# prstrive/GenS

Hardware: AMD Instinct MI355X
Metric: SDF ray-samples/sec at 480x640, 5-view, 3-scale volumes (higher is better)
Workload: dtype f32; 1 GPU; BASELINE config[1]: 5-view 480x640, volume_dims=[256, 128, 64], inference of 307200 rays x 128 samples per scene (K1 volume build + hierarchical sampling + SDF/blend MLPs + compositing); one scene per GPU; samples_per_ray=128, views=5, ray_chunk=30720, ray_chunk_set_by=ImplicitSurface.validate (default), cnn=out of scope (synthetic feature pyramid and regularised volumes), parallelism=single GPU

## Files before the change

gens_amd/csrc/k6b_sdf_bf16x3.hip:

```cpp
#include "common.h"

typedef float f32x16 __attribute__((ext_vector_type(16)));
typedef float f32x2v __attribute__((ext_vector_type(2)));
typedef float f32x4v __attribute__((ext_vector_type(4)));
typedef __bf16 bf16x2 __attribute__((ext_vector_type(2)));
typedef __bf16 bf16x8 __attribute__((ext_vector_type(8)));
typedef uint32_t u32x4 __attribute__((ext_vector_type(4)));

#define GB_WAVES 4
#define GB_PIECE 1024
#define GB_TERMS 3
#define GB_CH 8
#define GB_RING 4
#define GB_GT 2
#define GB_LPW (GB_CH / GB_WAVES)
#define GB_W_BYTES (GB_RING * GB_CH * GB_PIECE)
#define GB_D_BYTES (2 * 16 * 64 * 16)
#define GB_LDS_BYTES (GB_W_BYTES + GB_WAVES * GB_D_BYTES)
#define GB_JL_OFF 16384
#define GB_LOCK_OFF (GB_JL_OFF + 32 * 256)
#define GB_SLOT_BYTES (GB_LOCK_OFF + 256)
#define GB_SLOTS 2048
#define GB_C 144.26950408889634f

struct Split3Block {
    u32x4 p[GB_TERMS];
};

struct Split3Word {
    uint32_t w[GB_TERMS];
};
__device__ __forceinline__ uint32_t pk_bf16(float a, float b) {
    return __builtin_bit_cast(uint32_t, __builtin_convertvector((f32x2v){a, b}, bf16x2));
}
__device__ __forceinline__ Split3Word split3_pair(float a, float b) {
    Split3Word s;
#pragma unroll
    for (int k = 0; k < GB_TERMS; ++k) {
        const uint32_t w = pk_bf16(a, b);
        s.w[k] = w;
        if (k + 1 < GB_TERMS) {
            a -= __builtin_bit_cast(float, w << 16);
            b -= __builtin_bit_cast(float, w & 0xffff0000u);
        }
    }
    return s;
}
#define GB_PUT(BLK_, W_, A_, B_)                                            \
    {                                                                       \
        const Split3Word sw__ = split3_pair((A_), (B_));                    \
        _Pragma("unroll") for (int k__ = 0; k__ < GB_TERMS; ++k__) (BLK_).p[k__][(W_)] = sw__.w[k__]; \
    }

__device__ __forceinline__ float4 sample_volume4b(const float4* __restrict__ v, int Xd, int Yd, int Zd, const float x[3], bool live, float4& jx,
                                                  float4& jy, float4& jz) {
    float w0[3], w1[3];
    int i0[3];
    bool in0[3], in1[3];
    const int sz[3] = {Xd, Yd, Zd};
#pragma unroll
    for (int a = 0; a < 3; ++a) {
        const float pos = (x[a] + 1.0f) / 2.0f * (float)(sz[a] - 1);
        const float f = fminf(fmaxf(floorf(pos), -2.0f), (float)sz[a] + 1.0f);
        i0[a] = (int)f;
        w0[a] = (f + 1.0f) - pos;
        w1[a] = pos - f;
        in0[a] = i0[a] >= 0 && i0[a] < sz[a];
        in1[a] = i0[a] + 1 >= 0 && i0[a] + 1 < sz[a];
    }
    float4 acc = f4_zero();
    jx = f4_zero(); jy = f4_zero(); jz = f4_zero();
#pragma unroll
    for (int c = 0; c < 8; ++c) {
        const int a = c >> 2, b = (c >> 1) & 1, d = c & 1;
        const bool ok = live && (a ? in1[0] : in0[0]) && (b ? in1[1] : in0[1]) && (d ? in1[2] : in0[2]);
        const int cx = min(max(i0[0] + a, 0), Xd - 1), cy = min(max(i0[1] + b, 0), Yd - 1), cz = min(max(i0[2] + d, 0), Zd - 1);
        float4 t = v[((int64_t)cx * Yd + cy) * Zd + cz];
        if (!ok) t = f4_zero();
        const float wx = a ? w1[0] : w0[0], wy = b ? w1[1] : w0[1], wz = d ? w1[2] : w0[2];
        acc = f4_madd(acc, t, wx * wy * wz);
        jx = f4_madd(jx, t, (a ? 1.0f : -1.0f) * wy * wz);
        jy = f4_madd(jy, t, wx * (b ? 1.0f : -1.0f) * wz);
        jz = f4_madd(jz, t, wx * wy * (d ? 1.0f : -1.0f));
    }
    const float sx = (float)(Xd - 1) / 2.0f, sy = (float)(Yd - 1) / 2.0f, sz_ = (float)(Zd - 1) / 2.0f;
    jx.x *= sx; jx.y *= sx; jx.z *= sx; jx.w *= sx;
    jy.x *= sy; jy.y *= sy; jy.z *= sy; jy.w *= sy;
    jz.x *= sz_; jz.y *= sz_; jz.z *= sz_; jz.w *= sz_;
    return acc;
}

template <int NLEV>
struct GradShapeB {
    static constexpr int CF = 4 * NLEV;
    static constexpr int NCH = CF / 2;
    static constexpr int NC = (5 * NCH + 1 + 7) / 8;
    static constexpr int TC = (5 * NCH + 15) / 16;
    static constexpr int BLK = 4 * GB_TERMS;
    static constexpr int fwd(int l) { return l == 0 ? 0 : BLK * (2 + (l - 1) * (NC + 8) + (l > 3 ? 2 : 0)); }
    static constexpr int FWD_PIECES = fwd(5) + BLK * (NC + 8);
    static constexpr int rev_tiles(int l) { return 4 + TC + (l == 3 ? 1 : 0); }
    static constexpr int rev_blocks(int l) { return l == 2 ? 7 : 8; }
    static constexpr int rev(int l) {
        int p = FWD_PIECES;
        for (int k = 5; k > l; --k) p += GB_TERMS * rev_tiles(k) * rev_blocks(k);
        return p;
    }
    static constexpr int PIECES = rev(0) + 8 * GB_TERMS;
    static constexpr int NCHUNK = (PIECES + GB_CH - 1) / GB_CH;
    static constexpr int NCHUNK_FWD = (FWD_PIECES + GB_CH - 1) / GB_CH;
};

template <int NLEV, bool GRAD>
__global__ __launch_bounds__(64 * GB_WAVES, 1) void sdf_bf16x3_k(LevelSet vols, const char* __restrict__ pieces, const float* w_out, float b_last,
                                                                 float scale, float inv_scale, const float* __restrict__ pts,
                                                                 const int64_t* __restrict__ index, int64_t n_max, const int32_t* __restrict__ n_dev,
                                                                 float* __restrict__ sdf_out, float* __restrict__ grad_out,
                                                                 char* __restrict__ stash_all) {
    typedef GradShapeB<NLEV> S;
    constexpr int NCH = S::NCH, NC = S::NC, TC = S::TC, MID = NLEV / 2;
    constexpr int NCHUNK = GRAD ? S::NCHUNK : S::NCHUNK_FWD;
    extern __shared__ __attribute__((aligned(16))) char lds[];
    const int tid = threadIdx.x, lane = tid & 63;
    const int wave = __builtin_amdgcn_readfirstlane(tid >> 6);
    const int n_pt = lane & 31, half = lane >> 5;
    const int64_t n = n_dev ? min(n_max, (int64_t)n_dev[0]) : n_max;
    const int64_t m0 = (int64_t)blockIdx.x * (32 * GB_WAVES);
    if (m0 >= n) return;
    float4* const DS = (float4*)(lds + GB_W_BYTES + wave * GB_D_BYTES);

    const __amdgpu_buffer_rsrc_t prs = __builtin_amdgcn_make_buffer_rsrc((void*)pieces, 0, NCHUNK * GB_CH * GB_PIECE, 0x00020000);
    const uint32_t lane16 = (uint32_t)lane * 16u;
    auto stage = [&](int c) {
        char* dst = lds + (c % GB_RING) * (GB_CH * GB_PIECE);
#pragma unroll
        for (int p = 0; p < GB_LPW; ++p) {
            const int piece = wave + GB_WAVES * p;
            __builtin_amdgcn_raw_ptr_buffer_load_lds(prs, (__attribute__((address_space(3))) void*)(dst + piece * GB_PIECE), 16, lane16,
                                                     (uint32_t)(c * (GB_CH * GB_PIECE) + piece * GB_PIECE), 0, 0);
        }
    };
#pragma unroll
    for (int c = 0; c < GB_RING - 1; ++c) stage(c);

    uint32_t* lock = nullptr;
    uint32_t lock_seen = 0u;
    __amdgpu_buffer_rsrc_t stash;
    if constexpr (GRAD) {
        uint32_t hw_id, xcc_id;
        asm volatile("s_getreg_b32 %0, hwreg(HW_REG_HW_ID)" : "=s"(hw_id));
        asm volatile("s_getreg_b32 %0, hwreg(HW_REG_XCC_ID)" : "=s"(xcc_id));
        const uint32_t slot = ((((xcc_id & 7u) << 2 | ((hw_id >> 13) & 3u)) << 4 | ((hw_id >> 8) & 15u)) << 2) | (uint32_t)wave;
        char* const stash_slot = stash_all + (size_t)slot * GB_SLOT_BYTES;
        lock = (uint32_t*)(stash_slot + GB_LOCK_OFF);
        lock_seen = lane == 0 ? atomicCAS(lock, 0u, 1u) : 0u;
        stash = __builtin_amdgcn_make_buffer_rsrc((void*)stash_slot, 0, GB_LOCK_OFF, 0x00020000);
    }
    const uint32_t stash_lane = (uint32_t)lane * 16u, jl_lane = GB_JL_OFF + (uint32_t)lane * 4u;

    const int64_t row = m0 + 32 * wave + n_pt;
    const bool live = row < n;
    const int64_t src = live ? (index ? index[row] : row) : 0;
    float x[3] = {0.f, 0.f, 0.f};
    if (live) { x[0] = pts[3 * src]; x[1] = pts[3 * src + 1]; x[2] = pts[3 * src + 2]; }
    float nan_sum = 0.0f;

    Split3Block P[2];
    {
        float q[16];
#pragma unroll
        for (int k = 0; k < 16; ++k) q[k] = 0.0f;
#pragma unroll
        for (int a = 0; a < 3; ++a) {
            const float v = x[a] * scale;
            float s0, c0, s1, c1;
            hw_sincos(v * (half ? 4.0f : 1.0f), s0, c0);
            hw_sincos(v * (half ? 8.0f : 2.0f), s1, c1);
            if (half == 0) {
                q[a] = v; q[3 + a] = s0; q[6 + a] = c0; q[9 + a] = s1; q[12 + a] = c1;
            } else {
                q[a] = s0; q[3 + a] = c0; q[6 + a] = s1; q[9 + a] = c1;
            }
            nan_sum += x[a];
        }
        if (half == 0) q[15] = 1.0f;
#pragma unroll
        for (int k = 0; k < 16; k += 2) GB_PUT(P[k >> 3], (k & 7) >> 1, q[k], q[k + 1])
    }

    Split3Block C[NC];
    const float* wo = w_out + half * (64 + 16 * TC);
    float s_cond = 0.0f;
    float f[NCH];
    {
        float jl[3 * NCH];
#pragma unroll
        for (int j = 0; j <= MID; ++j) {
            const int l = j < MID ? (half ? MID + 1 + j : j) : MID;
            float4 jx, jy, jz;
            const float4 t = sample_volume4b((const float4*)vols.data[l], vols.dx[l], vols.dy[l], vols.dz[l], x, live, jx, jy, jz);
            float tv[4] = {t.x, t.y, t.z, t.w}, ax[4] = {jx.x, jx.y, jx.z, jx.w}, ay[4] = {jy.x, jy.y, jy.z, jy.w}, az[4] = {jz.x, jz.y, jz.z, jz.w};
            if (j == MID && half) {
                tv[0] = tv[2]; tv[1] = tv[3]; ax[0] = ax[2]; ax[1] = ax[3]; ay[0] = ay[2]; ay[1] = ay[3]; az[0] = az[2]; az[1] = az[3];
            }
#pragma unroll
            for (int c = 0; c < (j < MID ? 4 : 2); ++c) {
                const int ch = 4 * j + c;
                f[ch] = tv[c];
                jl[3 * ch] = ax[c]; jl[3 * ch + 1] = ay[c]; jl[3 * ch + 2] = az[c];
            }
        }
        if constexpr (GRAD) {
            if (lane == 0) gens_lock_slot(lock, lock_seen);
#pragma unroll
            for (int k = 0; k < 3 * NCH; ++k) __builtin_amdgcn_raw_buffer_store_b32(__builtin_bit_cast(uint32_t, jl[k]), stash, jl_lane + (uint32_t)k * 256u, 0, 0);
        }
        float e[8 * NC];
#pragma unroll
        for (int k = 5 * NCH; k < 8 * NC; ++k) e[k] = (k == 5 * NCH && half == 0) ? 1.0f : 0.0f;
#pragma unroll
        for (int j = 0; j < NCH; ++j) {
            e[5 * j] = f[j];
            hw_sincos(f[j], e[5 * j + 1], e[5 * j + 2]);
            hw_sincos(2.0f * f[j], e[5 * j + 3], e[5 * j + 4]);
            nan_sum += f[j];
#pragma unroll
            for (int q = 0; q < 5; ++q) s_cond = __builtin_fmaf(e[5 * j + q], wo[64 + 5 * j + q], s_cond);
        }
#pragma unroll
        for (int k = 0; k < 8 * NC; k += 2) GB_PUT(C[k >> 3], (k & 7) >> 1, e[k], e[k + 1])
    }

    f32x16 acc[4];
    Split3Block H[8];
    f32x16 D3[4], D4[4];
    f32x16 gc[TC], gp;
    u32x4 abuf[2][GB_TERMS * GB_GT];
    int par = 0;
    int dirty = GRAD ? 1 : 0;

#define GB_BOUNDARY(C_)                                                                                  \
    {                                                                                                    \
        const int c__ = (C_);                                                                            \
        const int later__ = (c__ + GB_RING - 2 < NCHUNK - 1 ? c__ + GB_RING - 2 : NCHUNK - 1) - c__;     \
        if (dirty || later__ <= 0) asm volatile("s_waitcnt vmcnt(0)" ::: "memory");                      \
        else if (later__ == 1) asm volatile("s_waitcnt vmcnt(%0)" ::"n"(GB_LPW) : "memory");             \
        else asm volatile("s_waitcnt vmcnt(%0)" ::"n"(2 * GB_LPW) : "memory");                           \
        dirty = 0;                                                                                       \
        __builtin_amdgcn_s_barrier();                                                                    \
        asm volatile("" ::: "memory");                                                                   \
        if (c__ + GB_RING - 1 < NCHUNK) stage(c__ + GB_RING - 1);                                        \
    }
#define GB_LOAD(SET_, P0_, CNT_)                                                                         \
    _Pragma("unroll") for (int j_ = 0; j_ < GB_TERMS * GB_GT; ++j_) if (j_ < (CNT_)) {                    \
        const int p_ = (P0_) + j_;                                                                       \
        if (p_ % GB_CH == 0) GB_BOUNDARY(p_ / GB_CH)                                                     \
        abuf[SET_][j_] = *((const u32x4*)(lds + ((p_ / GB_CH) % GB_RING) * (GB_CH * GB_PIECE) + (p_ % GB_CH) * GB_PIECE) + lane); \
    }
#define GB_MFMA(ACC_, A_, B_) ACC_ = __builtin_amdgcn_mfma_f32_32x32x16_bf16(__builtin_bit_cast(bf16x8, (A_)), __builtin_bit_cast(bf16x8, (B_)), ACC_, 0, 0, 0)
#define GB_RACC(T_) (*((T_) < 4 ? &acc[(T_) < 4 ? (T_) : 0] : (T_) < 4 + TC ? &gc[(T_) < 4 + TC && (T_) >= 4 ? (T_) - 4 : 0] : &gp))
#define GB_TERM(WA_, WB_, REV_, B_)                                                                      \
    _Pragma("unroll") for (int t_ = 0; t_ < GB_GT; ++t_) if (t_ < nt_) {                                 \
        if (REV_) GB_MFMA(GB_RACC(t0_ + t_), abuf[par][GB_TERMS * t_ + (WA_)], (B_)[i_].p[(WB_)]);       \
        else GB_MFMA(acc[(t0_ + t_) & 3], abuf[par][GB_TERMS * t_ + (WA_)], (B_)[i_].p[(WB_)]);          \
    }
#define GB_SEGMENT(P0_, CNT_, NT_, B_, REV_)                                                             \
    {                                                                                                    \
        constexpr int ng__ = ((NT_) + GB_GT - 1) / GB_GT;       \
        GB_LOAD(par, (P0_), GB_TERMS * ((NT_) < GB_GT ? (NT_) : GB_GT))                                  \
        _Pragma("unroll") for (int q_ = 0; q_ < (CNT_) * ng__; ++q_) {                                   \
            const int i_ = q_ / ng__, t0_ = (q_ % ng__) * GB_GT, nt_ = (NT_) - t0_ < GB_GT ? (NT_) - t0_ : GB_GT; \
            if (q_ + 1 < (CNT_) * ng__) {                                                                \
                const int i2_ = (q_ + 1) / ng__, t2_ = ((q_ + 1) % ng__) * GB_GT, n2_ = (NT_) - t2_ < GB_GT ? (NT_) - t2_ : GB_GT; \
                GB_LOAD(par ^ 1, (P0_) + GB_TERMS * ((NT_) * i2_ + t2_), GB_TERMS * n2_)                  \
            }                                                                                            \
            __builtin_amdgcn_sched_barrier(0);                                                           \
            GB_TERM(2, 0, REV_, B_) GB_TERM(1, 1, REV_, B_) GB_TERM(0, 2, REV_, B_)                      \
            GB_TERM(1, 0, REV_, B_) GB_TERM(0, 1, REV_, B_) GB_TERM(0, 0, REV_, B_)                      \
            __builtin_amdgcn_sched_barrier(0);                                                           \
            par ^= 1;                                                                                    \
        }                                                                                                \
    }
#define GB_ZERO()                                             \
    _Pragma("unroll") for (int t_ = 0; t_ < 4; ++t_)          \
        _Pragma("unroll") for (int r_ = 0; r_ < 16; ++r_) acc[t_][r_] = 0.0f;
#define GB_SOFTPLUS_TILE(T_, HT_, DT_)                                                                     \
    {                                                                                                      \
        f32x16 e__, u__, r__;                                                                              \
        _Pragma("unroll") for (int r_ = 0; r_ < 16; ++r_) e__[r_] = __builtin_amdgcn_exp2f(__builtin_amdgcn_fmed3f((T_)[r_], 126.0f, -3.0e38f)); \
        _Pragma("unroll") for (int r_ = 0; r_ < 16; ++r_) u__[r_] = 1.0f + e__[r_];                        \
        if (GRAD) { _Pragma("unroll") for (int r_ = 0; r_ < 16; ++r_) r__[r_] = __builtin_amdgcn_rcpf(u__[r_]); } \
        _Pragma("unroll") for (int r_ = 0; r_ < 16; ++r_) u__[r_] = __builtin_amdgcn_logf(u__[r_]);        \
        if (GRAD) { _Pragma("unroll") for (int r_ = 0; r_ < 16; ++r_) (DT_)[r_] = e__[r_] * r__[r_]; }     \
        _Pragma("unroll") for (int r_ = 0; r_ < 16; ++r_) (HT_)[r_] = __builtin_amdgcn_fmed3f((T_)[r_], u__[r_], 3.0e38f); \
    }
#define GB_SPLIT_TILE(T_, V_)                                                                              \
    _Pragma("unroll") for (int r_ = 0; r_ < 16; r_ += 2) GB_PUT(H[2 * (T_) + (r_ >> 3)], (r_ & 7) >> 1, (V_)[r_], (V_)[r_ + 1])

    float s_val = s_cond;
    GB_ZERO();
    GB_SEGMENT(S::fwd(0), 2, 4, P, false);
#pragma unroll
    for (int l = 0; l < 6; ++l) {
        if (l > 0) {
            GB_ZERO();
            GB_SEGMENT(S::fwd(l), NC, 4, C, false);
            if (l == 3) GB_SEGMENT(S::fwd(3) + S::BLK * NC, 2, 4, P, false);
            GB_SEGMENT(S::fwd(l) + S::BLK * (NC + (l == 3 ? 2 : 0)), 8, 4, H, false);
        }
#pragma unroll
        for (int t = 0; t < 4; ++t) {
            f32x16 h, d;
            if (l == 3) {
                GB_SOFTPLUS_TILE(acc[t], h, D3[t]);
            } else if (l == 4) {
                GB_SOFTPLUS_TILE(acc[t], h, D4[t]);
            } else {
                GB_SOFTPLUS_TILE(acc[t], h, d);
            }
            if constexpr (GRAD) {
                if (l < 2) {
#pragma unroll
                    for (int q = 0; q < 4; ++q) DS[(l * 16 + 4 * t + q) * 64 + lane] = make_float4(d[4 * q], d[4 * q + 1], d[4 * q + 2], d[4 * q + 3]);
                }
                if (l == 2) {
#pragma unroll
                    for (int q = 0; q < 4; ++q)
                        __builtin_amdgcn_raw_buffer_store_b128(__builtin_bit_cast(u32x4, (f32x4v){d[4 * q], d[4 * q + 1], d[4 * q + 2], d[4 * q + 3]}), stash,
                                                               stash_lane + (uint32_t)(4 * t + q) * 1024u, 0, 0);
                    dirty = 1;
                }
            }
            if (l < 5) {
                GB_SPLIT_TILE(t, h);
            } else {
                f32x16 g;
#pragma unroll
                for (int r = 0; r < 16; ++r) {
                    const float w = wo[16 * t + r];
                    s_val = __builtin_fmaf(h[r], w, s_val);
                    if (GRAD) g[r] = (w * GB_C) * d[r];
                }
                if constexpr (GRAD) GB_SPLIT_TILE(t, g);
            }
        }
    }
    s_val += 0.0f * nan_sum;
    s_val += __shfl_xor(s_val, 32, 64);

    if constexpr (!GRAD) {
        if (half == 0 && live) sdf_out[src] = (s_val + b_last) * inv_scale;
    } else {
#pragma unroll
        for (int c = 0; c < TC; ++c)
#pragma unroll
            for (int r = 0; r < 16; ++r) gc[c][r] = (16 * c + r < 5 * NCH) ? wo[64 + 16 * c + r] : 0.0f;
#pragma unroll
        for (int r = 0; r < 16; ++r) gp[r] = 0.0f;
#pragma unroll
        for (int l = 5; l >= 1; --l) {
            GB_ZERO();
            if (l == 3) {
#pragma unroll
                for (int t = 0; t < 4; ++t)
#pragma unroll
                    for (int q = 0; q < 4; ++q) {
                        const f32x4v v = __builtin_bit_cast(f32x4v, __builtin_amdgcn_raw_buffer_load_b128(stash, stash_lane + (uint32_t)(4 * t + q) * 1024u, 0, 0));
                        D4[t][4 * q] = v[0]; D4[t][4 * q + 1] = v[1]; D4[t][4 * q + 2] = v[2]; D4[t][4 * q + 3] = v[3];
                    }
            }
            if (l == 3) {
                GB_SEGMENT(S::rev(3), 8, 4 + TC + 1, H, true);
            } else if (l == 2) {
                GB_SEGMENT(S::rev(2), 7, 4 + TC, H, true);
            } else {
                GB_SEGMENT(S::rev(l), 8, 4 + TC, H, true);
            }
#pragma unroll
            for (int t = 0; t < 4; ++t) {
                f32x16 g;
#pragma unroll
                for (int q = 0; q < 4; ++q) {
                    float4 d;
                    if (l == 5) d = make_float4(D4[t][4 * q], D4[t][4 * q + 1], D4[t][4 * q + 2], D4[t][4 * q + 3]);
                    if (l == 4) d = make_float4(D3[t][4 * q], D3[t][4 * q + 1], D3[t][4 * q + 2], D3[t][4 * q + 3]);
                    if (l == 3) d = make_float4(D4[t][4 * q], D4[t][4 * q + 1], D4[t][4 * q + 2], D4[t][4 * q + 3]);
                    if (l == 2) d = DS[(16 + 4 * t + q) * 64 + lane];
                    if (l == 1) d = DS[(4 * t + q) * 64 + lane];
                    g[4 * q] = acc[t][4 * q] * d.x;
                    g[4 * q + 1] = acc[t][4 * q + 1] * d.y;
                    g[4 * q + 2] = acc[t][4 * q + 2] * d.z;
                    g[4 * q + 3] = acc[t][4 * q + 3] * d.w;
                }
                GB_SPLIT_TILE(t, g);
            }
        }
        {
            GB_ZERO();
            GB_LOAD(par, S::rev(0), GB_TERMS)
#pragma unroll
            for (int i = 0; i < 8; ++i) {
                if (i + 1 < 8) { GB_LOAD(par ^ 1, S::rev(0) + GB_TERMS * (i + 1), GB_TERMS) }
                __builtin_amdgcn_sched_barrier(0);
                GB_MFMA(acc[0], abuf[par][2], H[i].p[0]);
                GB_MFMA(acc[1], abuf[par][1], H[i].p[1]);
                GB_MFMA(acc[2], abuf[par][1], H[i].p[0]);
                GB_MFMA(acc[0], abuf[par][0], H[i].p[2]);
                GB_MFMA(acc[3], abuf[par][0], H[i].p[1]);
                GB_MFMA(gp, abuf[par][0], H[i].p[0]);
                __builtin_amdgcn_sched_barrier(0);
                par ^= 1;
            }
#pragma unroll
            for (int r = 0; r < 16; ++r) gp[r] += (acc[0][r] + acc[1][r]) + (acc[2][r] + acc[3][r]);
        }

        {
            float g[3];
#pragma unroll
            for (int a = 0; a < 3; ++a) asm volatile("" : "+v"(x[a]));
#pragma unroll
            for (int j = 0; j < NCH; ++j) asm volatile("" : "+v"(f[j]));
#pragma unroll
            for (int a = 0; a < 3; ++a) {
                const float v = x[a] * scale;
                float s0, c0, s1, c1;
                hw_sincos(v * (half ? 4.0f : 1.0f), s0, c0);
                hw_sincos(v * (half ? 8.0f : 2.0f), s1, c1);
                g[a] = half ? 4.0f * (gp[a] * c0 - gp[3 + a] * s0) + 8.0f * (gp[6 + a] * c1 - gp[9 + a] * s1)
                            : gp[a] + (gp[3 + a] * c0 - gp[6 + a] * s0) + 2.0f * (gp[9 + a] * c1 - gp[12 + a] * s1);
                g[a] *= scale;
            }
            {
                float acc_in = x[0] + x[1] + x[2];
#pragma unroll
                for (int j = 0; j < NCH; ++j) acc_in += f[j];
#pragma unroll
                for (int a = 0; a < 3; ++a) g[a] += 0.0f * acc_in;
            }
#pragma unroll
            for (int j = 0; j < NCH; ++j) {
                const int q = 5 * j;
                float s1, c1, s2, c2;
                hw_sincos(f[j], s1, c1);
                hw_sincos(2.0f * f[j], s2, c2);
                const float df = gc[q >> 4][q & 15] + gc[(q + 1) >> 4][(q + 1) & 15] * c1 - gc[(q + 2) >> 4][(q + 2) & 15] * s1 +
                                 2.0f * (gc[(q + 3) >> 4][(q + 3) & 15] * c2 - gc[(q + 4) >> 4][(q + 4) & 15] * s2);
#pragma unroll
                for (int a = 0; a < 3; ++a) {
                    const float jl = __builtin_bit_cast(float, __builtin_amdgcn_raw_buffer_load_b32(stash, jl_lane + (uint32_t)(3 * j + a) * 256u, 0, 0));
                    g[a] = __builtin_fmaf(df, jl, g[a]);
                }
            }
#pragma unroll
            for (int a = 0; a < 3; ++a) g[a] += __shfl_xor(g[a], 32, 64);
            if (half == 0 && live) {
                sdf_out[src] = (s_val + b_last) * inv_scale;
                grad_out[3 * src] = g[0] * inv_scale;
                grad_out[3 * src + 1] = g[1] * inv_scale;
                grad_out[3 * src + 2] = g[2] * inv_scale;
            }
        }
        if (lane == 0) atomicExch(lock, 0u);
    }
#undef GB_BOUNDARY
#undef GB_LOAD
#undef GB_MFMA
#undef GB_RACC
#undef GB_TERM
#undef GB_SEGMENT
#undef GB_ZERO
#undef GB_SOFTPLUS_TILE
#undef GB_SPLIT_TILE
}

int gens_fill_levels(const char* who, LevelSet* ls, const float* const* data, const int* dims, int n_levels);

extern "C" int gens_sdf_bf16x3_pieces(int n_levels) {
    return n_levels == 3 ? GradShapeB<3>::NCHUNK * GB_CH : n_levels == 5 ? GradShapeB<5>::NCHUNK * GB_CH : 0;
}

extern "C" int64_t gens_sdf_grad_f16_stash_bytes(void);

static int check_bf16x3_args(const char* who, int n_levels, const void* pieces, const float* w_out, float scale, const float* pts, int64_t n,
                             const float* sdf_out) {
    GENS_CHECK_ARG(n_levels == 3 || n_levels == 5, GENS_ELIMIT, "%s: built for 3 or 5 volume levels, got %d", who, n_levels);
    GENS_CHECK_ARG(pieces && w_out, GENS_EINVAL, "%s: null weight stream", who);
    GENS_CHECK_ARG(((uintptr_t)pieces & 15) == 0, GENS_EINVAL, "%s: the weight stream must be 16-byte aligned", who);
    GENS_CHECK_ARG(n >= 0 && (n == 0 || (pts && sdf_out)), GENS_EINVAL, "%s: null pts / output", who);
    GENS_CHECK_ARG(scale != 0.0f, GENS_EINVAL, "%s: scale must be non-zero", who);
    return 0;
}

extern "C" int gens_sdf_value_bf16x3(const float* const* vols_packed, const int* dims, int n_levels, const void* pieces, const float* w_out,
                                     float b_last, float scale, const float* pts, const int64_t* index, int64_t n, const int32_t* n_device,
                                     float* sdf_out, void* stream) {
    LevelSet vs;
    if (int e = gens_fill_levels("gens_sdf_value_bf16x3", &vs, vols_packed, dims, n_levels)) return e;
    if (int e = check_bf16x3_args("gens_sdf_value_bf16x3", n_levels, pieces, w_out, scale, pts, n, sdf_out)) return e;
    if (n == 0) return 0;
    const unsigned grid = gens_blocks(n, 32 * GB_WAVES);
    if (n_levels == 3)
        sdf_bf16x3_k<3, false><<<grid, 64 * GB_WAVES, GB_W_BYTES, (hipStream_t)stream>>>(vs, (const char*)pieces, w_out, b_last, scale, 1.0f / scale, pts,
                                                                                          index, n, n_device, sdf_out, nullptr, nullptr);
    else
        sdf_bf16x3_k<5, false><<<grid, 64 * GB_WAVES, GB_W_BYTES, (hipStream_t)stream>>>(vs, (const char*)pieces, w_out, b_last, scale, 1.0f / scale, pts,
                                                                                          index, n, n_device, sdf_out, nullptr, nullptr);
    return gens_launch_status("gens_sdf_value_bf16x3");
}

extern "C" int gens_sdf_grad_bf16x3(const float* const* vols_packed, const int* dims, int n_levels, const void* pieces, const float* w_out,
                                    float b_last, float scale, const float* pts, const int64_t* index, int64_t n, const int32_t* n_device,
                                    float* sdf_out, float* grad_out, void* stash, void* stream) {
    LevelSet vs;
    if (int e = gens_fill_levels("gens_sdf_grad_bf16x3", &vs, vols_packed, dims, n_levels)) return e;
    if (int e = check_bf16x3_args("gens_sdf_grad_bf16x3", n_levels, pieces, w_out, scale, pts, n, sdf_out)) return e;
    GENS_CHECK_ARG(n == 0 || grad_out, GENS_EINVAL, "gens_sdf_grad_bf16x3: null gradient output");
    GENS_CHECK_ARG(stash && ((uintptr_t)stash & 15) == 0, GENS_EINVAL,
                   "gens_sdf_grad_bf16x3: null or misaligned stash (gens_sdf_grad_f16_stash_bytes() bytes, zeroed once)");
    GENS_CHECK_ARG(gens_sdf_grad_f16_stash_bytes() == (int64_t)GB_SLOTS * GB_SLOT_BYTES, GENS_EINVAL, "gens_sdf_grad_bf16x3: stash layout differs from k6gh's");
    if (n == 0) return 0;
    static GensLdsOptIn lds3, lds5;
    if (int e = n_levels == 3 ? gens_lds_opt_in(lds3, (const void*)sdf_bf16x3_k<3, true>, GB_LDS_BYTES, "gens_sdf_grad_bf16x3")
                              : gens_lds_opt_in(lds5, (const void*)sdf_bf16x3_k<5, true>, GB_LDS_BYTES, "gens_sdf_grad_bf16x3"))
        return e;
    const unsigned grid = gens_blocks(n, 32 * GB_WAVES);
    if (n_levels == 3)
        sdf_bf16x3_k<3, true><<<grid, 64 * GB_WAVES, GB_LDS_BYTES, (hipStream_t)stream>>>(vs, (const char*)pieces, w_out, b_last, scale, 1.0f / scale, pts,
                                                                                           index, n, n_device, sdf_out, grad_out, (char*)stash);
    else
        sdf_bf16x3_k<5, true><<<grid, 64 * GB_WAVES, GB_LDS_BYTES, (hipStream_t)stream>>>(vs, (const char*)pieces, w_out, b_last, scale, 1.0f / scale, pts,
                                                                                           index, n, n_device, sdf_out, grad_out, (char*)stash);
    return gens_launch_status("gens_sdf_grad_bf16x3");
}
```

gens_amd/csrc/k7t_blend.hip:

```cpp
#include "k4_common.h"

typedef float f32x4 __attribute__((ext_vector_type(4)));

#define KT_NT 4
#define KT_XS 29

struct BlendTWeights {
    const float4* stream;
    const float* tab;
    float v2_last_b, u2_b, r3_b, s_abs;
    const float* sdev;
};
enum { KT_RD1_B = 0, KT_RD2_B, KT_B2_B, KT_V1_B, KT_V2_B, KT_U1_B, KT_R2_B, KT_V2_LAST, KT_U2, KT_R3, KT_TAB_ENTRIES };

__device__ __forceinline__ float elu1t(float x) { return __builtin_amdgcn_fmed3f(x, hw_exp(x) - 1.0f, 0.0f); }
template <int G>
__device__ __forceinline__ float group_sum(float v) {
    v += dpp_move<0xB1, 0xF>(v, v);
    if (G == 4) v += dpp_move<0x4E, 0xF>(v, v);
    return v;
}
template <int G>
__device__ __forceinline__ float group_min(float v) {
    v = fminf(v, dpp_move<0xB1, 0xF>(v, v));
    if (G == 4) v = fminf(v, dpp_move<0x4E, 0xF>(v, v));
    return v;
}
template <int G>
__device__ __forceinline__ float group_max(float v) {
    v = fmaxf(v, dpp_move<0xB1, 0xF>(v, v));
    if (G == 4) v = fmaxf(v, dpp_move<0x4E, 0xF>(v, v));
    return v;
}
__device__ __forceinline__ float lanes_q_sum(float v) {
    v += __shfl_xor(v, 16, 64);
    v += __shfl_xor(v, 32, 64);
    return v;
}

template <int NLEV, int S>
__global__ __launch_bounds__(64, 2) void blend_t_k(BlendTWeights W, MapSet fs, const float4* __restrict__ imgs, const float* __restrict__ w2c,
                                                   const float* __restrict__ intr, const float* __restrict__ c2w, const float* __restrict__ pts,
                                                   const int64_t* __restrict__ index, int64_t n_max, const int32_t* __restrict__ n_dev,
                                                   float* __restrict__ rgb_out, uint8_t* __restrict__ vis_out) {
    constexpr int F = 3 + 4 * NLEV;
    constexpr int XQ = NLEV + 1;
    constexpr int XT = (XQ + 3) / 4;
    constexpr int G = S == 2 ? 2 : 4;
    constexpr int PPT = 16 / G;
    constexpr int PPW = 64 / G;
    constexpr int NPT = PPW / 16;
    static_assert(S >= 2 && S <= 4, "two to four source views");
    static_assert(4 * XQ <= KT_XS, "feature tile too narrow");
    __shared__ float X[64 * KT_XS];
    __shared__ float RD[64 * 5];
    __shared__ float R[64];
    const int lane = threadIdx.x;
    const int np = lane & 15, q = lane >> 4;
    const int64_t n = n_dev ? min(n_max, (int64_t)n_dev[0]) : n_max;
    const int64_t first = (int64_t)blockIdx.x * PPW;
    if (first >= n) return;
    if (W.sdev) { W.v2_last_b = W.sdev[0]; W.u2_b = W.sdev[1]; W.r3_b = W.sdev[2]; W.s_abs = W.sdev[3]; }

    const float4* wp = W.stream;
    float4 wb[3];
    int par = 0;
    wb[0] = wp[lane];
    wb[1] = wp[lane + 64];
    wp += 128;

    {
        const int pl = lane / G, sv = (lane % G) + 1;
        const bool live = first + pl < n && sv <= S;
        const int64_t src = live ? (index ? index[first + pl] : first + pl) : 0;
        float x = 0.f, y = 0.f, z = 0.f;
        if (live) { x = pts[3 * src]; y = pts[3 * src + 1]; z = pts[3 * src + 2]; }
        bool inside = true;
        float* xr = X + lane * KT_XS;
        const int svc = sv <= S ? sv : S;
        const SrcBase pb = project_src_base(w2c + 16 * svc, intr + 16 * svc, x, y, z);
#pragma unroll
        for (int l = 0; l < NLEV; ++l) {
            const int h = fs.h[l], w = fs.w[l];
            const SrcProj p = project_src_level(pb, exp2f(-(float)l), h, w, fs.cw[l], fs.ch[l], fs.rcw[l], fs.rch[l]);
            inside = inside && p.inside;
            float4 f = f4_zero(), c = f4_zero();
            if (live) {
                const Taps2 t = bilinear_taps(p.ix, p.iy, h, w);
                f = sample_texel(fs.data[l] + (int64_t)svc * h * w, h, w, 1, 0, t);
                if (l == 0) c = sample_texel(imgs + (int64_t)svc * h * w, h, w, 1, 0, t);
            }
            xr[3 + 4 * l] = f.x; xr[4 + 4 * l] = f.y; xr[5 + 4 * l] = f.z; xr[6 + 4 * l] = f.w;
            if (l == 0) { xr[0] = c.x; xr[1] = c.y; xr[2] = c.z; }
        }
        xr[F] = 1.0f;
        float acc_in = x + y + z;
#pragma unroll
        for (int k = 0; k < F; ++k) acc_in += xr[k];
        R[lane] = ((live && inside) ? 1.0f : 0.0f) + 0.0f * acc_in;
        if (live && vis_out) vis_out[src * S + (sv - 1)] = inside ? 1 : 0;
        float rx = c2w[3] - x, ry = c2w[7] - y, rz = c2w[11] - z;
        const float rn = hw_rcp(__builtin_amdgcn_sqrtf(rx * rx + ry * ry + rz * rz) + 1e-6f);
        rx *= rn; ry *= rn; rz *= rn;
        const float* cs = c2w + 16 * svc;
        float sx = cs[3] - x, sy = cs[7] - y, sz = cs[11] - z;
        const float sn = hw_rcp(__builtin_amdgcn_sqrtf(sx * sx + sy * sy + sz * sz) + 1e-6f);
        sx *= sn; sy *= sn; sz *= sn;
        const float dx = rx - sx, dy = ry - sy, dz = rz - sz;
        const float dn = hw_rcp(fmaxf(__builtin_amdgcn_sqrtf(dx * dx + dy * dy + dz * dz), 1e-6f));
        float* rd = RD + lane * 5;
        rd[0] = live ? dx * dn : 0.0f;
        rd[1] = live ? dy * dn : 0.0f;
        rd[2] = live ? dz * dn : 0.0f;
        rd[3] = live ? rx * sx + ry * sy + rz * sz : 0.0f;
    }
    __syncthreads();

    float xq[KT_NT][XQ];
    float rgbc[KT_NT];
    float rdq[KT_NT], dotv[KT_NT], mask[KT_NT], rd3one[KT_NT], rdsh[KT_NT];
#pragma unroll
    for (int j = 0; j < KT_NT; ++j) {
        const int row = 16 * j + np;
#pragma unroll
        for (int kq = 0; kq < XQ; ++kq) xq[j][kq] = X[row * KT_XS + 4 * kq + q];
        rgbc[j] = xq[j][0];
        rdq[j] = RD[row * 5 + q];
        dotv[j] = RD[row * 5 + 3];
        mask[j] = R[row];
        rdsh[j] = q ? RD[row * 5 + q - 1] : 0.0f;
        rd3one[j] = q == 0 ? dotv[j] : (q == 1 ? 1.0f : 0.0f);
    }
    const float* tab = W.tab + q * 8;
#define KT_TAB(E, K) tab[(E) * 32 + (K)]

#define KT_GROUP(NT_, NQ_, ACC_, C0_, B_, Q0_)                                                           \
    {                                                                                                    \
        const float4 a_ = wb[par];                                                                       \
        wb[(par + 2) % 3] = wp[lane];                                                                    \
        wp += 64;                                                                                        \
        par = (par + 1) % 3;                                                                             \
        _Pragma("unroll") for (int j_ = 0; j_ < (NT_); ++j_) ACC_(j_) = __builtin_amdgcn_mfma_f32_16x16x4f32(a_.x, B_(j_, (Q0_)), C0_(j_), 0, 0, 0); \
        if ((NQ_) > 1) { _Pragma("unroll") for (int j_ = 0; j_ < (NT_); ++j_) ACC_(j_) = __builtin_amdgcn_mfma_f32_16x16x4f32(a_.y, B_(j_, (Q0_) + 1), ACC_(j_), 0, 0, 0); } \
        if ((NQ_) > 2) { _Pragma("unroll") for (int j_ = 0; j_ < (NT_); ++j_) ACC_(j_) = __builtin_amdgcn_mfma_f32_16x16x4f32(a_.z, B_(j_, (Q0_) + 2), ACC_(j_), 0, 0, 0); } \
        if ((NQ_) > 3) { _Pragma("unroll") for (int j_ = 0; j_ < (NT_); ++j_) ACC_(j_) = __builtin_amdgcn_mfma_f32_16x16x4f32(a_.w, B_(j_, (Q0_) + 3), ACC_(j_), 0, 0, 0); } \
    }
#define KT_PRODUCT(NT_, MT_, NQ_, ACC2_, B_)                                                             \
    _Pragma("unroll") for (int T_ = 0; T_ < (MT_); ++T_)                                                 \
        _Pragma("unroll") for (int g_ = 0; g_ < ((NQ_) + 3) / 4; ++g_) {                                 \
            if (g_ == 0) KT_GROUP(NT_, ((NQ_) < 4 ? (NQ_) : 4), ACC_T_, INIT_T_, B_, 0)                  \
            else KT_GROUP(NT_, ((NQ_) - 4 * g_ < 4 ? (NQ_) - 4 * g_ : 4), ACC_T_, ACC_T_, B_, 4 * g_)   \
        }

    f32x4 D[KT_NT];
    {
        const f32x4 b = {KT_TAB(KT_RD1_B, 0), KT_TAB(KT_RD1_B, 1), KT_TAB(KT_RD1_B, 2), KT_TAB(KT_RD1_B, 3)};
#define ACC_T_(j) D[j]
#define INIT_T_(j) b
#define B_RD(j, k) rdq[j]
        KT_GROUP(KT_NT, 1, ACC_T_, INIT_T_, B_RD, 0)
#undef ACC_T_
#undef INIT_T_
#pragma unroll
        for (int j = 0; j < KT_NT; ++j)
#pragma unroll
            for (int i = 0; i < 4; ++i) D[j][i] = elu1t(D[j][i]);
    }
    {
        f32x4 E[XT][KT_NT], bias[XT];
#pragma unroll
        for (int T = 0; T < XT; ++T)
            bias[T] = (f32x4){KT_TAB(KT_RD2_B, 4 * T), KT_TAB(KT_RD2_B, 4 * T + 1), KT_TAB(KT_RD2_B, 4 * T + 2), KT_TAB(KT_RD2_B, 4 * T + 3)};
#define ACC_T_(j) E[T_][j]
#define INIT_T_(j) bias[T_]
#define B_D(j, k) D[j][k]
        KT_PRODUCT(KT_NT, XT, 4, E, B_D)
#undef ACC_T_
#undef INIT_T_
#pragma unroll
        for (int j = 0; j < KT_NT; ++j)
#pragma unroll
            for (int kq = 0; kq < XQ; ++kq) xq[j][kq] += elu1t(E[kq >> 2][j][kq & 3]);
    }

    float wn[KT_NT];
    float pm[NPT][XQ], pv[NPT][XQ];
    const bool dead = S == 3 && (np & 3) == 3;
    {
        const int src = (G * (np % PPT) + 16 * q) * 4;
#pragma unroll
        for (int t = 0; t < NPT; ++t)
#pragma unroll
            for (int kq = 0; kq < XQ; ++kq) { pm[t][kq] = 0.0f; pv[t][kq] = 0.0f; }
#pragma unroll
        for (int j = 0; j < KT_NT; ++j) {
            const float e = hw_exp(W.s_abs * (dotv[j] - 1.0f));
            const float mn = group_min<G>(dead ? __builtin_inff() : e);
            const float wr = dead ? 0.0f : (e - mn) * mask[j];
            wn[j] = wr / (group_sum<G>(wr) + 1e-8f);
#pragma unroll
            for (int kq = 0; kq < XQ; ++kq) {
                const float mean = group_sum<G>(wn[j] * xq[j][kq]);
                const float d = xq[j][kq] - mean;
                const float var = group_sum<G>(wn[j] * (d * d));
                const float tm = __builtin_bit_cast(float, __builtin_amdgcn_ds_bpermute(src, __builtin_bit_cast(int, mean)));
                const float tv = __builtin_bit_cast(float, __builtin_amdgcn_ds_bpermute(src, __builtin_bit_cast(int, var)));
#pragma unroll
                for (int t = 0; t < NPT; ++t) {
                    const bool sel = (16 * t + np) / PPT == j;
                    pm[t][kq] = sel ? tm : pm[t][kq];
                    pv[t][kq] = sel ? tv : pv[t][kq];
                }
            }
        }
    }

    f32x4 H1[4][KT_NT];
    {
        f32x4 P[NPT][4];
        const f32x4 zero4 = {0.f, 0.f, 0.f, 0.f};
#define INIT_T_(j) zero4
#define ACC_T_(j) P[j][T_]
#define B_PM(j, k) ((k) < XQ ? pm[j][(k) < XQ ? (k) : 0] : pv[j][(k) < XQ ? 0 : (k) - XQ])
        KT_PRODUCT(NPT, 4, 2 * XQ, P, B_PM)
#undef ACC_T_
#undef INIT_T_
#pragma unroll
        for (int j = 0; j < KT_NT; ++j) {
            const int src = (((PPT * j) & 15) + np / G + 16 * q) * 4;
#pragma unroll
            for (int T = 0; T < 4; ++T)
#pragma unroll
                for (int i = 0; i < 4; ++i) {
                    float v = P[(PPT * j) >> 4][T][i];
                    asm volatile("" : "+v"(v));
                    H1[T][j][i] = __builtin_bit_cast(float, __builtin_amdgcn_ds_bpermute(src, __builtin_bit_cast(int, v)));
                }
        }
#define ACC_T_(j) H1[T_][j]
#define INIT_T_(j) H1[T_][j]
#define B_X(j, k) xq[j][k]
        KT_PRODUCT(KT_NT, 4, XQ, H1, B_X)
#undef ACC_T_
#undef INIT_T_
#pragma unroll
        for (int T = 0; T < 4; ++T)
#pragma unroll
            for (int j = 0; j < KT_NT; ++j)
#pragma unroll
                for (int i = 0; i < 4; ++i) H1[T][j][i] = elu1t(H1[T][j][i]);
    }
    f32x4 XH[2][KT_NT];
    {
        f32x4 bias[2];
#pragma unroll
        for (int T = 0; T < 2; ++T)
            bias[T] = (f32x4){KT_TAB(KT_B2_B, 4 * T), KT_TAB(KT_B2_B, 4 * T + 1), KT_TAB(KT_B2_B, 4 * T + 2), KT_TAB(KT_B2_B, 4 * T + 3)};
#define ACC_T_(j) XH[T_][j]
#define INIT_T_(j) bias[T_]
#define B_H1(j, k) H1[(k) >> 2][j][(k) & 3]
        KT_PRODUCT(KT_NT, 2, 16, XH, B_H1)
#undef ACC_T_
#undef INIT_T_
#pragma unroll
        for (int T = 0; T < 2; ++T)
#pragma unroll
            for (int j = 0; j < KT_NT; ++j)
#pragma unroll
                for (int i = 0; i < 4; ++i) XH[T][j][i] = elu1t(XH[T][j][i]);
    }

    f32x4 G1[2][KT_NT];
#define B_XS(j, k) xs[j][k]
#define KT_LAYER32(ENTRY, SCALE)                                                                                      \
    {                                                                                                                 \
        float xs[KT_NT][8];                                                                                           \
        _Pragma("unroll") for (int j = 0; j < KT_NT; ++j)                                                             \
            _Pragma("unroll") for (int k = 0; k < 8; ++k) xs[j][k] = XH[k >> 2][j][k & 3] * SCALE[j];                 \
        f32x4 bias[2];                                                                                                \
        _Pragma("unroll") for (int T = 0; T < 2; ++T)                                                                 \
            bias[T] = (f32x4){KT_TAB(ENTRY, 4 * T), KT_TAB(ENTRY, 4 * T + 1), KT_TAB(ENTRY, 4 * T + 2), KT_TAB(ENTRY, 4 * T + 3)}; \
        KT_PRODUCT(KT_NT, 2, 8, G1, B_XS)                                                                             \
        _Pragma("unroll") for (int T = 0; T < 2; ++T)                                                                 \
            _Pragma("unroll") for (int j = 0; j < KT_NT; ++j)                                                         \
                _Pragma("unroll") for (int i = 0; i < 4; ++i) G1[T][j][i] = elu1t(G1[T][j][i]);                       \
    }
#define KT_DOT32(ENTRY, OUT)                                                                                          \
    _Pragma("unroll") for (int j = 0; j < KT_NT; ++j) {                                                               \
        float s_ = 0.0f;                                                                                              \
        _Pragma("unroll") for (int k = 0; k < 8; ++k) s_ = __builtin_fmaf(G1[k >> 2][j][k & 3], KT_TAB(ENTRY, k), s_); \
        OUT[j] = lanes_q_sum(s_);                                                                                     \
    }

    float vis[KT_NT];
#define ACC_T_(j) G1[T_][j]
#define INIT_T_(j) bias[T_]
    KT_LAYER32(KT_V1_B, wn)
    KT_DOT32(KT_V2_LAST, vis)
#undef ACC_T_
#undef INIT_T_
    {
        f32x4 V2[2][KT_NT], bias[2];
#pragma unroll
        for (int T = 0; T < 2; ++T)
            bias[T] = (f32x4){KT_TAB(KT_V2_B, 4 * T), KT_TAB(KT_V2_B, 4 * T + 1), KT_TAB(KT_V2_B, 4 * T + 2), KT_TAB(KT_V2_B, 4 * T + 3)};
#define ACC_T_(j) V2[T_][j]
#define INIT_T_(j) bias[T_]
#define B_G1(j, k) G1[(k) >> 2][j][(k) & 3]
        KT_PRODUCT(KT_NT, 2, 8, V2, B_G1)
#undef ACC_T_
#undef INIT_T_
#pragma unroll
        for (int T = 0; T < 2; ++T)
#pragma unroll
            for (int j = 0; j < KT_NT; ++j)
#pragma unroll
                for (int i = 0; i < 4; ++i) XH[T][j][i] += elu1t(V2[T][j][i]);
    }
#pragma unroll
    for (int j = 0; j < KT_NT; ++j) vis[j] = hw_sigmoid(elu1t(vis[j] + W.v2_last_b)) * mask[j];

    float vis2[KT_NT];
#define ACC_T_(j) G1[T_][j]
#define INIT_T_(j) bias[T_]
    KT_LAYER32(KT_U1_B, vis)
    KT_DOT32(KT_U2, vis2)
#undef ACC_T_
#undef INIT_T_
#pragma unroll
    for (int j = 0; j < KT_NT; ++j) vis2[j] = hw_sigmoid(vis2[j] + W.u2_b) * mask[j];

    float score[KT_NT];
    {
        f32x4 C1[KT_NT];
        const f32x4 zero4 = {0.f, 0.f, 0.f, 0.f};
#define INIT_T_(j) zero4
#define ACC_T_(j) C1[j]
#define B_R1(j, k) ((k) < 8 ? XH[((k) < 8 ? (k) : 0) >> 2][j][(k) & 3] : (k) == 8 ? (q == 0 ? vis2[j] : rdsh[j]) : rd3one[j])
        KT_PRODUCT(KT_NT, 1, 10, C1, B_R1)
#undef ACC_T_
#undef INIT_T_
#pragma unroll
        for (int j = 0; j < KT_NT; ++j)
#pragma unroll
            for (int i = 0; i < 4; ++i) C1[j][i] = elu1t(C1[j][i]);
        f32x4 C2[KT_NT];
        const f32x4 b2 = {KT_TAB(KT_R2_B, 0), KT_TAB(KT_R2_B, 1), KT_TAB(KT_R2_B, 2), KT_TAB(KT_R2_B, 3)};
#define ACC_T_(j) C2[j]
#define INIT_T_(j) b2
#define B_C1(j, k) C1[j][k]
        KT_PRODUCT(KT_NT, 1, 4, C2, B_C1)
#undef ACC_T_
#undef INIT_T_
#pragma unroll
        for (int j = 0; j < KT_NT; ++j) {
            const float s = elu1t(C2[j][0]) * KT_TAB(KT_R3, 0) + elu1t(C2[j][1]) * KT_TAB(KT_R3, 1);
            score[j] = (mask[j] == 0.0f ? -1e9f : lanes_q_sum(s) + W.r3_b) + 0.0f * mask[j];
            if (dead) score[j] = -__builtin_inff();
        }
    }

#pragma unroll
    for (int j = 0; j < KT_NT; ++j) {
        const float mx = group_max<G>(score[j]);
        const float e = hw_exp(score[j] - mx);
        const float den = group_sum<G>(e);
        const float col = group_sum<G>(rgbc[j] * e) / den;
        const int64_t pt = first + PPT * j + np / G;
        if ((np % G) == 0 && q < 3 && pt < n) {
            const int64_t dst = index ? index[pt] : pt;
            rgb_out[3 * dst + q] = col;
        }
    }
#undef KT_TAB
#undef KT_GROUP
#undef KT_PRODUCT
#undef KT_LAYER32
#undef KT_DOT32
}

int gens_fill_maps(const char* who, MapSet* ms, const float* const* feats, const int* hw, int n_levels);

extern "C" int gens_blend_views_t_groups(int n_levels) {
    if (n_levels < 1 || n_levels > 5) return 0;
    const int xq = n_levels + 1, xt = (xq + 3) / 4;
    return 1 + xt + 4 * ((2 * xq + 3) / 4) + 4 * ((xq + 3) / 4) + 2 * 4 + 2 * 2 + 2 * 2 + 2 * 2 + 3 + 1;
}
extern "C" int gens_blend_views4_groups(int n_levels) { return gens_blend_views_t_groups(n_levels); }

struct BlendTWeights;
static int blend_t_run(int n_levels, int nv, const BlendTWeights& W, const MapSet& fs, const float* imgs, const float* w2c, const float* intr,
                       const float* c2w, const float* pts, const int64_t* index, int64_t n, const int32_t* n_device, float* rgb_out,
                       uint8_t* vis_out, void* stream);

template <int S>
static void blend_t_launch(int n_levels, unsigned grid, hipStream_t st, const BlendTWeights& W, const MapSet& fs, const float* imgs, const float* w2c,
                           const float* intr, const float* c2w, const float* pts, const int64_t* index, int64_t n, const int32_t* n_device,
                           float* rgb_out, uint8_t* vis_out) {
#define BLEND_LAUNCH(NL) blend_t_k<NL, S><<<grid, 64, 0, st>>>(W, fs, (const float4*)imgs, w2c, intr, c2w, pts, index, n, n_device, rgb_out, vis_out)
    switch (n_levels) {
        case 1: BLEND_LAUNCH(1); break;
        case 2: BLEND_LAUNCH(2); break;
        case 3: BLEND_LAUNCH(3); break;
        case 4: BLEND_LAUNCH(4); break;
        default: BLEND_LAUNCH(5); break;
    }
#undef BLEND_LAUNCH
}

extern "C" int gens_blend_views_t(const float* const* feats, const int* hw, int n_levels, const float* imgs, const float* w2c, const float* intr,
                                  const float* c2w, int nv, const float* wstream, const float* tab, const float* scalars, const float* pts,
                                  const int64_t* index, int64_t n, const int32_t* n_device, float* rgb_out, uint8_t* vis_out, void* stream) {
    MapSet fs;
    GENS_CHECK_ARG(feats && wstream && tab && scalars, GENS_EINVAL, "gens_blend_views_t: null table");
    if (int e = gens_fill_maps("gens_blend_views_t", &fs, feats, hw, n_levels)) return e;
    GENS_CHECK_ARG(n_levels <= 5, GENS_ELIMIT, "gens_blend_views_t: at most 5 feature levels (d_feature <= 20), got %d", n_levels);
    GENS_CHECK_ARG(nv >= 3 && nv <= 5, GENS_ELIMIT, "gens_blend_views_t: built for two to four source views (nv = 3..5), got nv=%d (use gens_blend_views)", nv);
    GENS_CHECK_ARG(imgs && w2c && intr && c2w, GENS_EINVAL, "gens_blend_views_t: null camera / image pointer");
    GENS_CHECK_ARG(((uintptr_t)wstream & 15) == 0, GENS_EINVAL, "gens_blend_views_t: the weight stream must be 16-byte aligned");
    GENS_CHECK_ARG(n >= 0 && (n == 0 || (pts && rgb_out)), GENS_EINVAL, "gens_blend_views_t: null pts / output");
    if (n == 0) return 0;
    BlendTWeights W;
    W.stream = (const float4*)wstream;
    W.tab = tab;
    W.v2_last_b = scalars[0]; W.u2_b = scalars[1]; W.r3_b = scalars[2]; W.s_abs = scalars[3];
    W.sdev = nullptr;
    return blend_t_run(n_levels, nv, W, fs, imgs, w2c, intr, c2w, pts, index, n, n_device, rgb_out, vis_out, stream);
}

static int blend_t_run(int n_levels, int nv, const BlendTWeights& W, const MapSet& fs, const float* imgs, const float* w2c, const float* intr,
                       const float* c2w, const float* pts, const int64_t* index, int64_t n, const int32_t* n_device, float* rgb_out,
                       uint8_t* vis_out, void* stream) {
    hipStream_t st = (hipStream_t)stream;
    if (nv == 3) blend_t_launch<2>(n_levels, gens_blocks(n, 32), st, W, fs, imgs, w2c, intr, c2w, pts, index, n, n_device, rgb_out, vis_out);
    else if (nv == 4) blend_t_launch<3>(n_levels, gens_blocks(n, 16), st, W, fs, imgs, w2c, intr, c2w, pts, index, n, n_device, rgb_out, vis_out);
    else blend_t_launch<4>(n_levels, gens_blocks(n, 16), st, W, fs, imgs, w2c, intr, c2w, pts, index, n, n_device, rgb_out, vis_out);
    return gens_launch_status("gens_blend_views_t");
}

extern "C" int gens_blend_views4(const float* const* feats, const int* hw, int n_levels, const float* imgs, const float* w2c, const float* intr,
                                 const float* c2w, int nv, const float* wstream, const float* tab, const float* scalars, const float* pts,
                                 const int64_t* index, int64_t n, const int32_t* n_device, float* rgb_out, uint8_t* vis_out, void* stream) {
    GENS_CHECK_ARG(nv == 5, GENS_ELIMIT, "gens_blend_views4: built for four source views (nv = 5), got nv=%d (use gens_blend_views_t / gens_blend_views)", nv);
    return gens_blend_views_t(feats, hw, n_levels, imgs, w2c, intr, c2w, nv, wstream, tab, scalars, pts, index, n, n_device, rgb_out, vis_out, stream);
}

struct BlendPackT {
    const float* p[23];
    int f;
    float4* stream;
    float* tab;
    float* scalars;
    int n_groups;
};

__device__ __forceinline__ float bpt_entry(const BlendPackT& A, int prod, int row, int slot, int xq) {
    const int f = A.f;
    int wi, O, I, col;
    bool has_bias = false;
    switch (prod) {
        case 0: wi = 0; O = 16; I = 4; col = slot < 4 ? slot : -2; break;
        case 1: wi = 2; O = f; I = 16; col = slot < 16 ? slot : -2; break;
        case 2: wi = 4; O = 64; I = 3 * f;
            col = slot < 4 * xq ? (slot < f ? slot : -2) : (slot - 4 * xq < f ? f + slot - 4 * xq : -2); break;
        case 3: wi = 4; O = 64; I = 3 * f; has_bias = true; col = slot < f ? 2 * f + slot : (slot == f ? -1 : -2); break;
        case 4: wi = 6; O = 32; I = 64; col = slot < 64 ? slot : -2; break;
        case 5: wi = 8; O = 32; I = 32; col = slot < 32 ? slot : -2; break;
        case 6: wi = 10; O = 32; I = 32; col = slot < 32 ? slot : -2; break;
        case 7: wi = 12; O = 32; I = 32; col = slot < 32 ? slot : -2; break;
        case 8: wi = 16; O = 16; I = 37; has_bias = true; col = slot < 37 ? slot : (slot == 37 ? -1 : -2); break;
        default: wi = 18; O = 8; I = 16; col = slot < 16 ? slot : -2; break;
    }
    if (row >= O || col == -2) return 0.0f;
    if (col == -1) return has_bias ? A.p[wi + 1][row] : 0.0f;
    return A.p[wi][(int64_t)row * I + col];
}

__global__ __launch_bounds__(256) void blend_pack_t_k(BlendPackT A) {
    const int f = A.f, xq = (f + 1) / 4, xt = (xq + 3) / 4;
    const int nq[10] = {1, 4, 2 * xq, xq, 16, 8, 8, 8, 10, 4};
    const int mt[10] = {1, xt, 4, 4, 2, 2, 2, 2, 1, 1};
    const int gid = blockIdx.x * 256 + threadIdx.x;
    const int n_stream = (A.n_groups + 2) * 64;
    if (gid < n_stream) {
        const int grp = gid >> 6, lane = gid & 63;
        float4 v = f4_zero();
        if (grp < A.n_groups) {
            int prod = 0, g0 = 0;
            for (; prod < 10; ++prod) {
                const int gp = mt[prod] * ((nq[prod] + 3) / 4);
                if (grp < g0 + gp) break;
                g0 += gp;
            }
            const int gq = (nq[prod] + 3) / 4, t = (grp - g0) / gq, g = (grp - g0) % gq;
            const int m = lane & 15, qk = lane >> 4;
            const int row = 16 * t + 4 * (m & 3) + (m >> 2);
            float e[4];
#pragma unroll
            for (int j = 0; j < 4; ++j) {
                const int kq = 4 * g + j;
                e[j] = kq < nq[prod] ? bpt_entry(A, prod, row, 4 * kq + qk, xq) : 0.0f;
            }
            v = make_float4(e[0], e[1], e[2], e[3]);
        }
        A.stream[gid] = v;
        return;
    }
    const int k = gid - n_stream;
    if (k < 10 * 32) {
        const int entry = k >> 5, q = (k >> 3) & 3, c = k & 7;
        float v = 0.0f;
        if (entry < 7) {
            const int bi[7] = {1, 3, 7, 9, 11, 13, 19}, len[7] = {16, f, 32, 32, 32, 32, 8}, tiles[7] = {1, xt, 2, 2, 2, 2, 1};
            const int T = c >> 2, i = c & 3, src = 16 * T + 4 * i + q;
            if (T < tiles[entry] && src < len[entry]) v = A.p[bi[entry]][src];
        } else {
            const int src = 4 * c + q;
            if (entry == 7) v = A.p[10][32 * 32 + src];
            else if (entry == 8) v = A.p[14][src];
            else v = src < 8 ? A.p[20][src] : 0.0f;
        }
        A.tab[k] = v;
    } else if (k == 10 * 32) {
        A.scalars[0] = A.p[11][32];
        A.scalars[1] = A.p[15][0];
        A.scalars[2] = A.p[21][0];
        A.scalars[3] = fabsf(A.p[22][0]);
    }
}

extern "C" int gens_blend_pack_t(const float* const* weights, int n_levels, float* wstream, float* tab, float* scalars_dev, void* stream) {
    GENS_CHECK_ARG(weights && wstream && tab && scalars_dev, GENS_EINVAL, "gens_blend_pack_t: null pointer");
    GENS_CHECK_ARG(n_levels >= 1 && n_levels <= 5, GENS_ELIMIT, "gens_blend_pack_t: 1..5 feature levels, got %d", n_levels);
    GENS_CHECK_ARG(((uintptr_t)wstream & 15) == 0, GENS_EINVAL, "gens_blend_pack_t: the weight stream must be 16-byte aligned");
    BlendPackT A;
    for (int k = 0; k < 23; ++k) {
        GENS_CHECK_ARG(weights[k], GENS_EINVAL, "gens_blend_pack_t: weight %d is null", k);
        A.p[k] = weights[k];
    }
    A.f = 3 + 4 * n_levels;
    A.stream = (float4*)wstream;
    A.tab = tab;
    A.scalars = scalars_dev;
    A.n_groups = gens_blend_views_t_groups(n_levels);
    const int work = (A.n_groups + 2) * 64 + 10 * 32 + 1;
    blend_pack_t_k<<<gens_blocks(work, 256), 256, 0, (hipStream_t)stream>>>(A);
    return gens_launch_status("gens_blend_pack_t");
}

extern "C" int gens_blend_views_t_dev(const float* const* feats, const int* hw, int n_levels, const float* imgs, const float* w2c, const float* intr,
                                      const float* c2w, int nv, const float* wstream, const float* tab, const float* scalars_dev, const float* pts,
                                      const int64_t* index, int64_t n, const int32_t* n_device, float* rgb_out, uint8_t* vis_out, void* stream) {
    MapSet fs;
    GENS_CHECK_ARG(feats && wstream && tab && scalars_dev, GENS_EINVAL, "gens_blend_views_t_dev: null table");
    if (int e = gens_fill_maps("gens_blend_views_t_dev", &fs, feats, hw, n_levels)) return e;
    GENS_CHECK_ARG(n_levels <= 5, GENS_ELIMIT, "gens_blend_views_t_dev: at most 5 feature levels (d_feature <= 20), got %d", n_levels);
    GENS_CHECK_ARG(nv >= 3 && nv <= 5, GENS_ELIMIT, "gens_blend_views_t_dev: built for two to four source views (nv = 3..5), got nv=%d", nv);
    GENS_CHECK_ARG(imgs && w2c && intr && c2w, GENS_EINVAL, "gens_blend_views_t_dev: null camera / image pointer");
    GENS_CHECK_ARG(((uintptr_t)wstream & 15) == 0, GENS_EINVAL, "gens_blend_views_t_dev: the weight stream must be 16-byte aligned");
    GENS_CHECK_ARG(n >= 0 && (n == 0 || (pts && rgb_out)), GENS_EINVAL, "gens_blend_views_t_dev: null pts / output");
    if (n == 0) return 0;
    BlendTWeights W;
    W.stream = (const float4*)wstream;
    W.tab = tab;
    W.v2_last_b = W.u2_b = W.r3_b = W.s_abs = 0.0f;
    W.sdev = scalars_dev;
    return blend_t_run(n_levels, nv, W, fs, imgs, w2c, intr, c2w, pts, index, n, n_device, rgb_out, vis_out, stream);
}
```

gens_amd/lib.py:

```python
import ctypes as C
import os

import torch

_HERE = os.path.dirname(os.path.abspath(__file__))
LIB_PATH = os.environ.get("GENS_HIP_LIB", os.path.join(_HERE, "csrc", "libgens_hip.so"))

MAX_LEVELS = 8
MAX_VIEWS = 16
LAYOUT_PLANAR = 0
LAYOUT_PACKED = 1

_p = C.c_void_p
_i = C.c_int
_l = C.c_int64
_f = C.c_float
_d = C.c_double
_pp = C.POINTER(C.c_void_p)
_ip = C.POINTER(C.c_int)
_fp = C.POINTER(C.c_float)


class CompositeIn(C.Structure):
    _fields_ = [(n, _p) for n in ("rays_o", "rays_d", "z", "sdf", "grad", "color", "smooth", "voxel_mask", "src_vis", "inv_s", "z_max")] + [
        ("n_rays", _l), ("n", _i), ("n_src", _i), ("sample_dist", _f), ("cos_anneal", _f), ("rot", _f * 9), ("rot_dev", _p), ("cos_anneal_dev", _p)]


class LossArgs(C.Structure):
    _fields_ = [("color", _p), ("target", _p), ("valid", _p), ("b", _l), ("sparse", _p), ("n_sparse", _l), ("sparse_scale", _f), ("pseudo", _p),
                ("n_pseudo", _l), ("ncc", _p), ("mid_in", _p), ("depth", _p), ("pseudo_depth_t", _p), ("depth_t", _p), ("ge", _p), ("se", _p), ("tv", _p)] + [
        (n, _f) for n in ("w_color", "w_igr", "w_sparse", "w_mfc", "w_smooth", "w_tv", "w_pseudo_sdf", "w_pseudo_depth")] + [
        (n, _p) for n in ("out", "g", "g_color", "g_sparse", "g_pseudo", "g_ncc", "g_depth", "g_scalars")]


class CompositeOut(C.Structure):
    _fields_ = [(n, _p) for n in ("color", "normal", "depth", "wsum", "wmax", "mid_in", "sdf_depth", "z_cross", "eik_num", "eik_den",
                                  "smooth_vec", "valid", "cross_idx", "weights", "inside", "pts_cross")]


class CompositeGrad(C.Structure):
    _fields_ = [(n, _p) for n in ("g_color", "g_normal", "g_depth", "g_weights", "g_wsum", "g_eik_num", "g_smooth_vec", "g_z_cross",
                                  "weights", "cross_idx", "smooth_vec", "g_sdf", "g_grad", "g_col", "g_smooth", "g_inv_s", "g_gradient_error",
                                  "g_smooth_error", "finish")]


class MeshGridArgs(C.Structure):
    _fields_ = [(n, _p) for n in ("vertices", "triangles", "cell_start", "cell_faces")] + [("n_faces", _l)] + [
        (n, _f) for n in ("lo_x", "lo_y", "lo_z", "cell")] + [(n, _i) for n in ("nx", "ny", "nz")]


class PointGridArgs(C.Structure):
    _fields_ = [(n, _p) for n in ("points", "sorted", "cell_start", "cell_points")] + [("n", _l)] + [
        (n, _d) for n in ("lo_x", "lo_y", "lo_z", "cell")] + [(n, _i) for n in ("nx", "ny", "nz")]


SIGNATURES = {
    "gens_pack_nchw": [_p, _p, _i, _i, _i, _i, _p],
    "gens_unpack_nhwc": [_p, _p, _i, _i, _i, _i, _p],
    "gens_pack_volume": [_p, _p, _i, _i, _i, _p],
    "gens_volume_build_fwd": [_p, _p, _p, _f, _i, _i, _i, _i, _i, _p, _p, _p],
    "gens_volume_build_bwd": [_p, _p, _p, _f, _i, _i, _i, _i, _p, _p, _p],
    "gens_selftest_division": [_p, _p],
    "gens_volume_build_levels": [_pp, _ip, _ip, _i, _p, _pp, _i, _i, _pp, _pp, _pp, _p],
    "gens_volume_build_levels_bits": [_pp, _ip, _ip, _i, _p, _pp, _i, _i, _pp, _pp, _pp, _pp, _p],
    "gens_volume_build_bwd_levels": [_pp, _ip, _ip, _i, _p, _pp, _i, _pp, _pp, _pp, _pp, _p, _l, _p],
    "gens_gemm_tn_slabs": [_l, _i, _i],
    "gens_gemm_tn": [_p, _p, _l, _i, _i, _p, _p, _p],
    "gens_conv3d_gather": [_p, _p, _p, _i, _i, _ip, _i, _p, _p],
    "gens_conv3d_scatter2": [_p, _p, _i, _i, _ip, _p, _p],
    "gens_conv3d_wgrad_parts": [_i, _i, _ip],
    "gens_conv3d_wgrad_parts_strided": [_i, _i, _ip, _i],
    "gens_conv3d_wgrad": [_p, _p, _i, _i, _ip, _i, _p, _p],
    "gens_instnorm_blocks": [_i, _l],
    "gens_instnorm_stats": [_p, _i, _l, _p, _p],
    "gens_instnorm_finish": [_p, _i, _l, C.c_double, _i, _p, _p],
    "gens_instnorm_relu_fwd": [_p, _p, _i, _l, _p, _p],
    "gens_instnorm_relu_add_fwd": [_p, _p, _p, _i, _l, _p, _p],
    "gens_instnorm_relu_bwd_stats": [_p, _p, _p, _i, _l, _p, _p],
    "gens_instnorm_relu_bwd": [_p, _p, _p, _p, _i, _l, _p, _p],
    "gens_lookup_volume_fwd": [_pp, _ip, _i, _i, _p, _l, _p, _p],
    "gens_lookup_volume_bwd": [_pp, _ip, _i, _i, _p, _p, _l, _pp, _p, _p],
    "gens_lookup_volume_bwd_bricks": [_pp, _ip, _i, _i, _p, _p, _l, _pp, _p, _p, _l, _p],
    "gens_lookup_volume_bwd2": [_pp, _ip, _i, _i, _p, _p, _p, _pp, _l, _p, _pp, _p, _p],
    "gens_lookup_volume_bwd2_bricks": [_pp, _ip, _i, _i, _p, _p, _p, _pp, _l, _p, _pp, _p, _p, _l, _p],
    "gens_lookup_mask_nearest": [_pp, _ip, _i, _p, _l, _p, _p, _p],
    "gens_ray_points": [_p, _p, _p, _l, _i, _i, _f, _pp, _ip, _i, _i, _p, _p, _p],
    "gens_pack_mask_bits": [_p, _l, _p, _p],
    "gens_lookup_feature_fwd": [_pp, _ip, _i, _p, _p, _p, _p, _i, _p, _l, _p, _p, _p, _p],
    "gens_lookup_feature_bwd": [_ip, _i, _p, _p, _i, _p, _p, _l, _pp, _p, _p],
    "gens_upsample": [_p, _p, _p, _p, _l, _i, _i, _f, _pp, _ip, _i, _i, _p, _p, _p, _p, _p],
    "gens_merge_samples": [_p, _p, _p, _p, _p, _p, _l, _i, _i, _p, _p, _p, _p],
    "gens_merge_upsample": [_p, _p, _p, _p, _p, _p, _p, _p, _l, _i, _i, _i, _f, _f, _pp, _ip, _i, _i, _i, _p, _p, _p, _p, _p, _p, _p],
    "gens_composite_fwd": [C.POINTER(CompositeIn), C.POINTER(CompositeOut), _p],
    "gens_composite_bwd": [C.POINTER(CompositeIn), C.POINTER(CompositeGrad), _p],
    "gens_patch_sample_fwd": [_p, _i, _i, _i, _p, _l, _p, _p],
    "gens_patch_sample_bwd": [_p, _i, _i, _i, _p, _p, _l, _p, _p],
    "gens_upsample2d_into": [_p, _i, _i, _i, _i, _p, _i, _i, _i, _i, _p],
    "gens_upsample2d_cat": [_pp, _ip, _i, _i, _p, _i, _i, _i, _p],
    "gens_select_views": [_pp, _pp, _ip, _ip, _i, _p, _i, _p],
    "gens_tv_fwd": [_p, _p, _i, _i, _i, _p, _p],
    "gens_tv_bwd": [_p, _p, _i, _i, _i, _f, _p, _p],
    "gens_tv_bwd_scaled": [_p, _p, _i, _i, _i, _f, _p, _p, _p],
    "gens_lattice_points": [_fp, _fp, _i, _l, _l, _p, _p],
    "gens_blend_views": [_pp, _ip, _i, _p, _p, _p, _p, _i, _pp, _fp, _p, _p, _l, _p, _p, _p, _p],
    "gens_blend_views4": [_pp, _ip, _i, _p, _p, _p, _p, _i, _p, _p, _fp, _p, _p, _l, _p, _p, _p, _p],
    "gens_blend_views4_groups": [_i],
    "gens_blend_views_t": [_pp, _ip, _i, _p, _p, _p, _p, _i, _p, _p, _fp, _p, _p, _l, _p, _p, _p, _p],
    "gens_blend_views_t_groups": [_i],
    "gens_blend_pack_t": [_pp, _i, _p, _p, _p, _p],
    "gens_blend_views_t_dev": [_pp, _ip, _i, _p, _p, _p, _p, _i, _p, _p, _p, _p, _p, _l, _p, _p, _p, _p],
    "gens_compact_valid": [_p, _l, _p, _p, _p, _p],
    "gens_sdf_value": [_pp, _ip, _i, _p, _p, _f, _f, _p, _p, _l, _p, _p, _p],
    "gens_sdf_value_groups": [_i],
    "gens_sdf_grad": [_pp, _ip, _i, _p, _p, _f, _f, _p, _p, _l, _p, _p, _p, _p, _p],
    "gens_sdf_grad_groups": [_i],
    "gens_sdf_grad_f16": [_pp, _ip, _i, _p, _p, _f, _f, _f, _p, _p, _l, _p, _p, _p, _p, _p, _p],
    "gens_sdf_grad_f16_pieces": [_i],
    "gens_sdf_value_f16": [_pp, _ip, _i, _p, _p, _f, _f, _p, _p, _l, _p, _p, _p, _p],
    "gens_sdf_value_f16_units": [_i],
    "gens_sdf_value_bf16x3": [_pp, _ip, _i, _p, _p, _f, _f, _p, _p, _l, _p, _p, _p],
    "gens_sdf_grad_bf16x3": [_pp, _ip, _i, _p, _p, _f, _f, _p, _p, _l, _p, _p, _p, _p, _p],
    "gens_sdf_bf16x3_pieces": [_i],
    "gens_lncc_fwd": [_p, _p, _l, _i, _i, _i, _p, _p, _p],
    "gens_lncc_bwd": [_p, _p, _p, _p, _l, _i, _i, _i, _p, _p, _p],
    "gens_mc_classify": [_p, _i, _i, _i, _f, _p, _p, _p, _p, _p, _p],
    "gens_mc_emit": [_p, _i, _i, _i, _f, _p, _i, _p, _p, _p, _p, _p, _p, _p, _p],
    "gens_sdf_mlp": [_pp, _ip, _i, _pp, _pp, _p, _p, _f, _f, _p, _p, _l, _p, _p, _p, _p],
    "gens_sdf_mlp_dev": [_pp, _ip, _i, _pp, _pp, _p, _p, _f, _p, _p, _l, _p, _p, _p, _p],
    "gens_blend_train_fwd": [_pp, _ip, _i, _p, _p, _p, _p, _i, _pp, _p, _p, _l, _p, _p, _p, _p],
    "gens_blend_train_bwd": [_pp, _ip, _i, _p, _p, _p, _p, _i, _pp, _p, _p, _l, _p, _p, _pp, _pp, _p, _p, _p],
    "gens_blend_train_bwd_acc": [_pp, _ip, _i, _p, _p, _p, _p, _i, _pp, _p, _p, _l, _p, _p, _p, _p, _p, _p, _p],
    "gens_blend_train_bwd_t": [_pp, _ip, _i, _p, _p, _p, _p, _i, _pp, _p, _p, _l, _p, _p, _p, _p, _p, _p, _p],
    "gens_blend_train_bwd_t_dump": [_pp, _ip, _i, _p, _p, _p, _p, _i, _pp, _p, _p, _l, _p, _p, _p, _p, _p, _p, _pp, _pp, _p],
    "gens_lookup_feature_bwd_idx": [_ip, _i, _p, _p, _i, _p, _p, _p, _l, _p, _pp, _p, _p],
    "gens_gemm_tn_batch_live": [_i, _pp, _ip, _pp, _ip, _ip, _ip, _l, _p, _i, _i, _p, _p, _p],
    "gens_sdf_train_pack": [_pp, _pp, _i, _pp, _pp, _p],
    "gens_sdf_train_pack_wn": [_pp, _pp, _pp, _i, _pp, _pp, _pp, _p, _p, _p],
    "gens_sdf_train_wgrad": [_pp, _pp, _i, _p, _p, _pp, _pp, _pp, _p],
    "gens_sdf_train_fwd": [_pp, _ip, _i, _pp, _pp, _p, _p, _p, _p, _l, _p, _p, _p, _p, _p, _p],
    "gens_sdf_train_bwd": [_pp, _ip, _i, _pp, _pp, _p, _p, _p, _l, _p, _p, _p, _p, _p, _p, _p, _p, _p, _p, _p, _p, _p, _p],
    "gens_gemm_tn_batch": [_i, _pp, _ip, _pp, _ip, _ip, _ip, _l, _p, _p, _p],
    "gens_sdf_train_scatter": [_ip, _i, _p, _p, _p, _p, _p, _p, _p, _l, _p, _pp, _p],
    "gens_scene_setup": [_p, _p, _i, _p, _p],
    "gens_coarse_z": [_p, _p, _i, _p, _p, _l, _i, _p, _p],
    "gens_sdf_grad_stash_reset": [_p, _p],
    "gens_depthwise_conv2d_fwd": [_p, _p, _i, _i, _i, _i, _i, _i, _p, _p],
    "gens_depthwise_conv2d_dgrad": [_p, _p, _i, _i, _i, _i, _i, _i, _p, _p],
    "gens_depthwise_conv2d_wgrad_parts": [_i, _i, _i, _i, _i, _i],
    "gens_depthwise_conv2d_wgrad": [_p, _p, _i, _i, _i, _i, _i, _i, _p, _p],
    "gens_batchnorm2d_train_fwd": [_p, _p, _p, _i, _i, _i, _f, _f, _i, _p, _p, _p, _p, _p, _p, _p],
    "gens_batchnorm2d_train_bwd": [_p, _p, _p, _p, _p, _i, _i, _i, _i, _p, _p, _p, _p, _p],
    "gens_grid_sample_fwd": [_p, _p, _i, _i, _i, _ip, _l, _i, _i, _p, _p],
    "gens_grid_sample_bwd": [_p, _p, _p, _i, _i, _i, _ip, _l, _i, _i, _p, _p, _p],
    "gens_grid_sample_bwd2": [_p, _p, _p, _p, _p, _i, _i, _i, _ip, _l, _i, _i, _p, _p, _p, _p],
    "gens_sdf_grad_f16_stash_reset": [_p, _p],
    "gens_blend_train_wgrad": [_p, _p, _i, _p, _i, _pp, _p],
    "gens_loss_fwd": [_p, _p],
    "gens_loss_bwd": [_p, _p],
    "gens_composite_finish_fwd": [_p, _p, _p, _l, _p, _p],
    "gens_composite_finish_bwd": [_p, _l, _p, _p, _p, _p, _p, _l, _l, _p],
    "gens_patch_warp_fwd": [_p, _p, _p, _p, _l, _p, _p, _p, _i, _p, _i, _i, _i, _i, _p, _p, _p],
    "gens_patch_warp_bwd": [_p, _p, _p, _p, _l, _p, _p, _p, _i, _p, _i, _i, _i, _i, _p, _p, _p],
    "gens_pack_maps": [_pp, _pp, _ip, _i, _p],
    "gens_unpack_maps": [_pp, _pp, _ip, _i, _p],
    "gens_compact_points": [_p, _l, _l, _l, _p, _p, _p, _p, _p, _p, _p, _i, _p, _l, _p, _p, _p, _p],
    "gens_tv_levels_blocks": [_ip, _i],
    "gens_tv_levels_fwd": [_pp, _pp, _ip, _i, _p, _p, _p],
    "gens_tv_levels_bwd": [_pp, _pp, _ip, _i, _p, _p, _pp, _p],
    "gens_mesh_grid_count": [C.POINTER(MeshGridArgs), _p, _p],
    "gens_mesh_grid_fill": [C.POINTER(MeshGridArgs), _p, _p],
    "gens_ray_first_hit": [C.POINTER(MeshGridArgs), _p, _p, _l, _p, _p, _p],
    "gens_view_rays_hit_faces": [C.POINTER(MeshGridArgs), _p, _p, _i, _i, _i, _i, _i, _f, _p, _p, _p],
    "gens_face_cc_hook": [_p, _l, _p, _l, _p],
    "gens_face_cc_compress": [_p, _l, _p, _p],
    "gens_mesh_sample_count": [_p, _l, _p, _l, _d, _p, _p],
    "gens_mesh_sample_emit": [_p, _l, _p, _l, _d, _p, _l, _p, _p],
    "gens_point_grid_count": [C.POINTER(PointGridArgs), _p, _p],
    "gens_point_grid_fill": [C.POINTER(PointGridArgs), _p, _p],
    "gens_radius_downsample_round": [C.POINTER(PointGridArgs), _p, _d, _p, _p, _p, _p],
    "gens_nearest_point": [C.POINTER(PointGridArgs), _p, _l, _d, _p, _p, _p],
    "gens_dilate_u8": [_p, _p, _i, _i, _i, _i, _i, _i, _i, _ip, _p],
    "gens_vertex_mask_votes": [_p, _l, _p, _p, _i, _i, _i, _p, _p],
    "gens_view_rays_hit_counts": [C.POINTER(MeshGridArgs), _p, _p, _i, _i, _i, _f, _p, _p, _p],
    "gens_filter_masks": [_p, _f, _pp, _pp, _pp, _ip, _i, _p, _p, _p],
    "gens_filter_band": [_p, _f, _i, _p, _p, _p],
    "gens_filter_levels": [_pp, _pp, _pp, _ip, _i, _p, _p, _p],
    "gens_components_scratch_bytes": [_i, _i, _i],
    "gens_largest_component": [_p, _i, _i, _i, _i, _p, _p, _p, _p],
    "gens_unpack_mask_bits": [_p, _l, _p, _p],
    "gens_sparse_coarse_points": [_fp, _fp, _i, _i, _l, _l, _p, _p],
    "gens_sparse_classify": [_p, _i, _i, _f, _f, _p, _p],
    "gens_sparse_brick_points": [_fp, _fp, _i, _i, _p, _l, _l, _l, _p, _p],
    "gens_sparse_fill": [_p, _i, _i, _p, _p],
    "gens_sparse_scatter": [_p, _i, _i, _p, _l, _l, _l, _p, _p],
    "gens_sparse_leaks": [_p, _i, _i, _p, _f, _p, _p],
}

_lib = None


def load():
    global _lib
    if _lib is not None:
        return _lib
    if not os.path.exists(LIB_PATH):
        raise RuntimeError(f"{LIB_PATH} is missing: build it with `make -C gens_amd/csrc` (or __graft_entry__.build()); "
                           "gens_amd has no CPU / PyTorch fallback for the hot path")
    lib = C.CDLL(LIB_PATH)
    lib.gens_last_error.restype = C.c_char_p
    lib.gens_last_error.argtypes = []
    lib.gens_abi_version.restype = _i
    lib.gens_abi_version.argtypes = []
    lib.gens_tv_blocks.restype = _i
    lib.gens_tv_blocks.argtypes = [_l]
    lib.gens_volume_build_bwd_levels_scratch_bytes.restype = _l
    lib.gens_volume_build_bwd_levels_scratch_bytes.argtypes = [_ip, _ip, _i, _i]
    lib.gens_sdf_train_stash_bytes.restype = _l
    lib.gens_sdf_grad_stash_bytes.restype = _l
    lib.gens_sdf_grad_stash_bytes.argtypes = []
    lib.gens_sdf_grad_f16_stash_bytes.restype = _l
    lib.gens_sdf_grad_f16_stash_bytes.argtypes = []
    lib.gens_sdf_train_stash_bytes.argtypes = [_l, _i]
    lib.gens_blend_train_rows.restype = _l
    lib.gens_blend_train_rows.argtypes = [_l, _i]
    lib.gens_blend_train_acc_parts.restype = _i
    lib.gens_blend_train_acc_parts.argtypes = [_l, _i]
    lib.gens_blend_train_acc_floats.restype = _i
    lib.gens_blend_train_acc_floats.argtypes = [_i]
    lib.gens_blend_train_t_parts.restype = _i
    lib.gens_blend_train_t_parts.argtypes = [_l, _i]
    lib.gens_lookup_scatter_bricks_scratch_bytes.restype = _l
    lib.gens_lookup_scatter_bricks_scratch_bytes.argtypes = [_l]
    lib.gens_gemm_tn_batch_workspace.restype = _l
    lib.gens_gemm_tn_batch_workspace.argtypes = [_i, _ip, _ip, _l]
    lib.gens_scene_cams_floats.restype = _l
    lib.gens_scene_cams_floats.argtypes = [_i]
    lib.gens_batchnorm2d_scratch_doubles.restype = _l
    lib.gens_batchnorm2d_scratch_doubles.argtypes = [_i, _i, _i]
    lib.gens_compact_points_scratch.restype = _l
    lib.gens_compact_points_scratch.argtypes = [_l]
    for name, args in SIGNATURES.items():
        fn = getattr(lib, name)
        fn.restype = _i
        fn.argtypes = args
    lib.gens_components_scratch_bytes.restype = _l
    _lib = lib
    return lib


_profile = None


_profile_only = None


def profile_begin(only=None):
    global _profile, _profile_only
    _profile = []
    _profile_only = set(only) if only else None


def profile_end(raw=False, per_launch=False):
    global _profile
    rec, _profile = _profile or [], None
    torch.cuda.synchronize()
    if raw:
        return [(name, s.elapsed_time(e), nbytes, flops) for name, s, e, nbytes, flops, _live in rec]
    out, each = {}, {}
    for name, s, e, nbytes, flops, live in rec:
        d = out.setdefault(name, {"launches": 0, "ms": 0.0, "bytes": 0, "flops": 0})
        frac = 1.0
        if live is not None:
            frac = min(1.0, float(live[0].item()) / max(1, live[1]))
        ms = s.elapsed_time(e)
        d["launches"] += 1
        d["ms"] += ms
        d["bytes"] += int(nbytes * frac)
        d["flops"] += int(flops * frac)
        each.setdefault(name, []).append(ms)
    return (out, each) if per_launch else out


def call(name, *args, nbytes=0, flops=0, live=None, label=None):
    lib = load()
    key = label or name
    if _profile is not None and (_profile_only is None or key in _profile_only):
        s, e = torch.cuda.Event(enable_timing=True), torch.cuda.Event(enable_timing=True)
        s.record()
        rc = getattr(lib, name)(*args)
        e.record()
        _profile.append((key, s, e, int(nbytes), int(flops), (live[0].clone(), live[1]) if live is not None else None))
    else:
        rc = getattr(lib, name)(*args)
    if rc != 0:
        raise RuntimeError(f"{name} failed (rc={rc}): {lib.gens_last_error().decode()}")


def stream():
    return C.c_void_p(torch.cuda.current_stream().cuda_stream)


def ptr(t, dtype=torch.float32, align=None):
    if t is None:
        return None
    if not t.is_cuda:
        raise RuntimeError("gens_amd kernels need device tensors (no CPU path)")
    if t.dtype != dtype:
        raise RuntimeError(f"expected {dtype}, got {t.dtype}")
    if not t.is_contiguous():
        raise RuntimeError("tensor must be contiguous")
    if align and t.data_ptr() % align != 0 and t.numel() > 0:
        raise RuntimeError(f"tensor storage is not {align}-byte aligned (offset view, data_ptr % {align} = {t.data_ptr() % align}): pass a .clone()")
    return C.c_void_p(t.data_ptr())


def ptr_table(tensors, dtype=torch.float32, align=None):
    if tensors is None:
        return None
    arr = (C.c_void_p * len(tensors))()
    for k, t in enumerate(tensors):
        arr[k] = None if t is None else ptr(t, dtype, align).value
    return C.cast(arr, _pp)


def int_table(values):
    flat = [int(v) for v in values]
    return (C.c_int * len(flat))(*flat)
```

gens_amd/ops/base.py:

```python
import ctypes as C
import os
import math

import torch

from .. import lib as L

_f32 = torch.float32


class KernelChoice:

    def __init__(self, env=os.environ):
        f32_mfma = "transposed" if env.get("GENS_SDF_F32_MFMA") else "bf16x3"
        self.sdf_value = "rowmajor" if env.get("GENS_SDF_VALUE_ROWMAJOR") else f32_mfma
        self.sdf_grad = "rowmajor" if env.get("GENS_SDF_GRAD_ROWMAJOR") else f32_mfma
        self.sdf_grad_f16 = not env.get("GENS_SDF_GRAD_F32_ONLY")
        self.blend = "rowmajor" if env.get("GENS_BLEND_ROWMAJOR") else "transposed"
        self.blend_train_fwd = "rowmajor" if env.get("GENS_BLEND_TRAIN_ROWMAJOR") else "transposed"
        self.blend_train_wgrad = "rows" if env.get("GENS_K18_OPERAND_ROWS") else "inside"
        self.blend_train_bwd = "rowmajor" if env.get("GENS_BLEND_TRAIN_BWD_ROWMAJOR") or env.get("GENS_K18_OPERAND_ROWS") else "transposed"
        self.k1_bwd = "window" if env.get("GENS_K1_BWD_WINDOW") else "auto"
        self.tex_cache = not env.get("GENS_NO_TEX_CACHE")
        self.select_views = not env.get("GENS_NO_SELECT_VIEWS")
        self.k2_bricks_min = int(env.get("GENS_K2_BRICKS_MIN", "196608"))


kernels = KernelChoice()


def _c(t):
    return t if t.is_contiguous() else t.contiguous()


_SDF_GRAD_STASH = {}


def sdf_grad_stash(device):
    key = torch.device(device).index if torch.device(device).index is not None else torch.cuda.current_device()
    buf = _SDF_GRAD_STASH.get(key)
    if buf is None:
        buf = _SDF_GRAD_STASH[key] = torch.zeros(L.load().gens_sdf_grad_stash_bytes(), device=torch.device("cuda", key), dtype=torch.uint8)
    return buf


def reset_sdf_grad_stashes():
    for key, buf in _SDF_GRAD_STASH.items():
        with torch.cuda.device(key):
            L.call("gens_sdf_grad_stash_reset", L.ptr(buf, torch.uint8), L.stream())
    for key, buf in _SDF_GRAD_F16_STASH.items():
        with torch.cuda.device(key):
            L.call("gens_sdf_grad_f16_stash_reset", L.ptr(buf, torch.uint8), L.stream())


_SDF_GRAD_F16_STASH = {}


def sdf_grad_f16_stash(device):
    key = torch.device(device).index if torch.device(device).index is not None else torch.cuda.current_device()
    buf = _SDF_GRAD_F16_STASH.get(key)
    if buf is None:
        buf = _SDF_GRAD_F16_STASH[key] = torch.zeros(L.load().gens_sdf_grad_f16_stash_bytes(), device=torch.device("cuda", key), dtype=torch.uint8)
    return buf


def aligned16(t):
    t = _c(t)
    return t if t.data_ptr() % 16 == 0 else t.clone()


def _dev_f32(t, device):
    return _c(t.to(device=device, dtype=_f32))


def inv(a):
    return torch.linalg.inv_ex(a).inverse


class _PackNCHW(torch.autograd.Function):
    @staticmethod
    def forward(ctx, x):
        n, c, h, w = x.shape
        ctx.shape = (n, c, h, w)
        out = torch.empty(n, h, w, 4 * ((c + 3) // 4), device=x.device, dtype=_f32)
        L.call("gens_pack_nchw", L.ptr(_c(x)), L.ptr(out), n, c, h, w, L.stream())
        return out

    @staticmethod
    def backward(ctx, g):
        n, c, h, w = ctx.shape
        out = torch.empty(n, c, h, w, device=g.device, dtype=_f32)
        L.call("gens_unpack_nhwc", L.ptr(_c(g)), L.ptr(out), n, c, h, w, L.stream())
        return out


def pack_nchw(x):
    return _PackNCHW.apply(x)


class _PackMaps(torch.autograd.Function):

    @staticmethod
    def forward(ctx, *xs):
        xs = [_c(x) for x in xs]
        outs = [torch.empty(x.shape[0], x.shape[2], x.shape[3], 4 * ((x.shape[1] + 3) // 4), device=x.device, dtype=_f32) for x in xs]
        nchw = [d for x in xs for d in x.shape]
        L.call("gens_pack_maps", L.ptr_table(xs), L.ptr_table(outs, align=16), L.int_table(nchw), len(xs), L.stream())
        ctx.shapes = [tuple(x.shape) for x in xs]
        ctx.set_materialize_grads(False)
        ctx.mark_non_differentiable(*[o for k, o in enumerate(outs) if not ctx.needs_input_grad[k]])
        return tuple(outs)

    @staticmethod
    def backward(ctx, *gs):
        live = [k for k, g in enumerate(gs) if g is not None and ctx.needs_input_grad[k]]
        res = [None] * len(gs)
        if live:
            srcs = [aligned16(gs[k]) for k in live]
            dsts = [torch.empty(ctx.shapes[k], device=srcs[0].device, dtype=_f32) for k in live]
            nchw = [d for k in live for d in ctx.shapes[k]]
            L.call("gens_unpack_maps", L.ptr_table(srcs, align=16), L.ptr_table(dsts), L.int_table(nchw), len(live), L.stream())
            for k, d in zip(live, dsts):
                res[k] = d
        return tuple(res)


def pack_maps(maps):
    maps = [m if m.dtype == _f32 else m.to(_f32) for m in maps]
    out, todo = [None] * len(maps), []
    grad_mode = torch.is_grad_enabled()
    for k, m in enumerate(maps):
        hit = getattr(m, "_gens_tex", None) if kernels.tex_cache else None
        if hit is not None and hit[0] == m._version and hit[1] == (grad_mode and m.requires_grad) and hit[2].device == m.device:
            out[k] = hit[2]
        else:
            todo.append(k)
    for s in range(0, len(todo), 8):
        part = todo[s:s + 8]
        texs = _PackMaps.apply(*[maps[k] for k in part])
        for k, t in zip(part, texs):
            out[k] = t
            try:
                maps[k]._gens_tex = (maps[k]._version, grad_mode and maps[k].requires_grad, t)
            except (AttributeError, RuntimeError):
                pass
    return out


class SceneCams:
    _last = None

    def __init__(self, intrs, c2ws):
        dev = c2ws.device
        self.nv = int(c2ws.shape[0])
        self.c2w, self.intr = _dev_f32(c2ws.detach(), dev), _dev_f32(intrs.detach(), dev)
        self.buf = torch.empty(L.load().gens_scene_cams_floats(self.nv), device=dev, dtype=_f32)
        L.call("gens_scene_setup", L.ptr(self.c2w), L.ptr(self.intr), self.nv, L.ptr(self.buf), L.stream())
        nv, o = self.nv, self.nv * 16
        self.w2c = self.buf[:o].view(nv, 4, 4)
        self.ks = [self.buf[o + l * nv * 16:o + (l + 1) * nv * 16].view(nv, 4, 4) for l in range(L.MAX_LEVELS)]
        o += L.MAX_LEVELS * nv * 16
        self.rot_inv = self.buf[o:o + 9]
        self.kinv_ref = self.buf[o + 12:o + 21].view(3, 3)
        self.status = self.buf[o + 24:o + 25].view(torch.int32)

    @staticmethod
    def of(intrs, c2ws):
        key = (intrs, c2ws, intrs._version, c2ws._version)
        last = SceneCams._last
        if last is not None and last[0][0] is intrs and last[0][1] is c2ws and last[0][2:] == key[2:]:
            return last[1]
        cams = SceneCams(intrs, c2ws)
        SceneCams._last = (key, cams)
        return cams

    def check(self):
        if int(self.status.item()) != 0:
            raise RuntimeError("linalg.inv: a camera pose or intrinsics matrix of the scene is singular (gens_scene_setup)")


def pack_volume(v):
    v = v.detach()
    if v.dim() == 5:
        v = v[0]
    assert v.shape[0] == 4, "only 4-channel volume levels are supported"
    _, x, y, z = v.shape
    out = torch.empty(x, y, z, 4, device=v.device, dtype=_f32)
    L.call("gens_pack_volume", L.ptr(_c(v)), L.ptr(out), x, y, z, L.stream())
    return out


class VolumeSet:

    def __init__(self, tensors, layout):
        self.layout = layout
        self.tensors = [aligned16(t) if layout == L.LAYOUT_PACKED else _c(t) for t in tensors]
        if layout == L.LAYOUT_PACKED:
            dims = [tuple(t.shape[:3]) for t in self.tensors]
        else:
            for t in self.tensors:
                assert t.shape[-4] == 4, "only 4-channel volume levels are supported (confs/gens.conf:63-67)"
            dims = [tuple(t.shape[-3:]) for t in self.tensors]
        self.dims = dims
        self.n = len(self.tensors)
        assert 1 <= self.n <= L.MAX_LEVELS
        self.table = L.ptr_table(self.tensors)
        self.dim_table = L.int_table([d for dd in dims for d in dd])

    @staticmethod
    def packed(volumes):
        return VolumeSet([pack_volume(v) for v in volumes], L.LAYOUT_PACKED)

    @staticmethod
    def masks(mask_volumes):
        vs = VolumeSet.__new__(VolumeSet)
        vs.layout = L.LAYOUT_PLANAR
        vs.tensors = [_c(m.detach().reshape(m.shape[-3:])) for m in mask_volumes]
        vs.sources = list(mask_volumes)
        vs.dims = [tuple(t.shape) for t in vs.tensors]
        vs.n = len(vs.tensors)
        vs.table = L.ptr_table(vs.tensors)
        vs.dim_table = L.int_table([d for dd in vs.dims for d in dd])
        vs._bits = None
        return vs

    def bit_table(self):
        if getattr(self, "_bits", None) is None:
            words = []
            for t, src in zip(self.tensors, getattr(self, "sources", self.tensors)):
                hit = getattr(src, "_gens_bits", None)
                if hit is not None and hit[0] == src._version and hit[1].device == t.device:
                    words.append(hit[1])
                    continue
                n = t.numel()
                w = torch.empty((n + 31) // 32, device=t.device, dtype=torch.int32)
                L.call("gens_pack_mask_bits", L.ptr(t), n, L.ptr(w, torch.int32), L.stream())
                words.append(w)
                try:
                    src._gens_bits = (src._version, w)
                except (AttributeError, RuntimeError):
                    pass
            self._bits = (words, L.ptr_table(words, torch.int32))
        return self._bits[1]


__all__ = [n_ for n_ in dir() if not n_.startswith("__")]
```

gens_amd/ops/blend.py:

```python
from .base import *
from .sdf import _pack_b16, _pack_b_groups, _poison

def _pad32(b):
    out = torch.zeros(32 * ((b.numel() + 31) // 32), device=b.device, dtype=_f32)
    out[:b.numel()] = b.reshape(-1)
    return out


def _pack_blend_t(layers, n_feat):
    f = n_feat
    xq = (f + 1) // 4
    dev = layers["rd1"][0].device
    lane = torch.arange(64, device=dev)
    m, qk = lane & 15, lane >> 4
    row_in_tile = 4 * (m & 3) + (m >> 2)

    def product(w, slots, m_tiles, bias=None):
        o = w.shape[0]
        aug = torch.cat([w, (bias if bias is not None else torch.zeros(o, device=dev))[:, None], torch.zeros(o, 1, device=dev)], 1)
        aug = torch.cat([aug, torch.zeros(16 * m_tiles - o, aug.shape[1], device=dev)], 0) if 16 * m_tiles > o else aug
        cols = torch.tensor([c if c >= 0 else (w.shape[1] if c == -1 else w.shape[1] + 1) for c in slots], device=dev)
        nq = (len(slots) + 3) // 4
        cols = torch.cat([cols, torch.full((4 * nq - len(slots),), w.shape[1] + 1, device=dev)])
        groups = []
        for t in range(m_tiles):
            rows = 16 * t + row_in_tile
            for g in range((nq + 3) // 4):
                frag = torch.zeros(64, 4, device=dev, dtype=_f32)
                for j in range(4):
                    kq = 4 * g + j
                    if kq < nq:
                        frag[:, j] = aug[rows, cols[4 * kq + qk]]
                groups.append(frag)
        return groups

    rd1, rd2, b1, b2, v1, v2, u1, u2, r1, r2, r3 = (layers[k] for k in ("rd1", "rd2", "b1", "b2", "v1", "v2", "u1", "u2", "r1", "r2", "r3"))
    xt = (xq + 3) // 4
    g = []
    g += product(rd1[0], [0, 1, 2, 3], 1)
    g += product(rd2[0], list(range(16)), xt)
    pad = [-2] * (4 * xq - f)
    g += product(b1[0], list(range(f)) + pad + list(range(f, 2 * f)) + pad, 4)
    g += product(b1[0], list(range(2 * f, 3 * f)) + [-1], 4, b1[1])
    g += product(b2[0], list(range(64)), 2)
    g += product(v1[0], list(range(32)), 2)
    g += product(v2[0][:32], list(range(32)), 2)
    g += product(u1[0], list(range(32)), 2)
    g += product(r1[0], list(range(36)) + [36, -1, -2, -2], 1, r1[1])
    g += product(r2[0], list(range(16)), 1)
    stream = torch.stack(g + [torch.zeros(64, 4, device=dev, dtype=_f32)] * 2).contiguous()

    def acc_bias(b, m_tiles):
        full = torch.zeros(32, device=dev, dtype=_f32)
        full[:min(b.shape[0], 16 * m_tiles)] = b[:16 * m_tiles]
        out = torch.zeros(4, 8, device=dev, dtype=_f32)
        for q in range(4):
            for t in range(m_tiles):
                for i in range(4):
                    out[q, 4 * t + i] = full[16 * t + 4 * i + q]
        return out

    def dot_row(w):
        full = torch.zeros(32, device=dev, dtype=_f32)
        full[:w.shape[0]] = w
        return full.reshape(8, 4).t().contiguous()

    tab = torch.stack([acc_bias(rd1[1], 1), acc_bias(rd2[1], xt), acc_bias(b2[1], 2), acc_bias(v1[1], 2), acc_bias(v2[1][:32], 2),
                       acc_bias(u1[1], 2), acc_bias(r2[1], 1), dot_row(v2[0][32]), dot_row(u2[0][0]), dot_row(r3[0][0])]).contiguous()
    return stream, tab


class BlendPlan:

    @staticmethod
    def supported(net):
        return bool(getattr(net, "anti_alias_pooling", False)) and net.base_fc[0].weight.shape[0] == 64 and net.rgb_fc[0].weight.shape[1] == 37

    @staticmethod
    def version(net):
        return tuple(p._version for p in net.parameters()) + tuple(p.data_ptr() for p in net.parameters())

    def __init__(self, net):
        assert BlendPlan.supported(net)
        g = lambda m: (m.weight.detach().to(_f32), m.bias.detach().to(_f32))
        with torch.no_grad():
            rd1, rd2 = g(net.ray_dir_fc[0]), g(net.ray_dir_fc[2])
            b1, b2 = g(net.base_fc[0]), g(net.base_fc[2])
            v1, v2 = g(net.vis_fc[0]), g(net.vis_fc[2])
            u1, u2 = g(net.vis_fc2[0]), g(net.vis_fc2[2])
            r1, r2, r3 = g(net.rgb_fc[0]), g(net.rgb_fc[2]), g(net.rgb_fc[4])
            self.n_feat = rd2[0].shape[0]
            P = _pack_b_groups
            N = _pack_b16
            self.tensors = [N(rd1[0], [(0, 2)]), _pad32(rd1[1]), P(rd2[0]), _pad32(rd2[1]), P(b1[0]), _pad32(b1[1]), P(b2[0]), _pad32(b2[1]),
                            P(v1[0]), _pad32(v1[1]), P(v2[0][:32]), _pad32(v2[1][:32]), _c(v2[0][32].clone()),
                            P(u1[0]), _pad32(u1[1]), _c(u2[0][0].clone()),
                            N(r1[0], [(0, 4), (16, 4), (32, 2)]), _pad32(r1[1]), N(r2[0], [(0, 4)]), _pad32(r2[1]), _c(r3[0][0].clone())]
            self.scalars = (C.c_float * 4)(float(v2[1][32]), float(u2[1][0]), float(r3[1][0]), float(net.s.detach().abs()))
            self.finite = bool(torch.stack([torch.isfinite(p.detach()).all() for p in net.parameters()]).all())
            self.t_stream, self.t_tab = _pack_blend_t(dict(rd1=rd1, rd2=rd2, b1=b1, b2=b2, v1=v1, v2=v2, u1=u1, u2=u2, r1=r1, r2=r2, r3=r3),
                                                      self.n_feat)
            assert self.t_stream.shape[0] == L.load().gens_blend_views_t_groups((self.n_feat - 3) // 4) + 2
        self.table = L.ptr_table(self.tensors)
        self.key = BlendPlan.version(net)


def blend_views(plan, views, pts, index=None, rgb_out=None, vis_out=None, count=None):
    pts = _c(pts.detach().reshape(-1, 3).to(_f32))
    n = pts.shape[0] if index is None else index.shape[0]
    s = views.nv - 1
    nl = len(views.feat_tex)
    assert plan.n_feat == 3 + 4 * nl, "colour network width does not match the feature pyramid"
    if rgb_out is None:
        rgb_out = torch.zeros(pts.shape[0], 3, device=pts.device, dtype=_f32)
    if vis_out is None:
        vis_out = torch.zeros(pts.shape[0], s, device=pts.device, dtype=torch.uint8)
    idx = None if index is None else _c(index.to(torch.int64))
    hw = [d for f in views.feat_tex for d in f.shape[1:3]]
    feats = [aligned16(f.detach()) for f in views.feat_tex]
    f = plan.n_feat
    flops = 2 * s * (4 * 16 + 16 * f + 3 * f * 64 + 64 * 32 + 32 * 32 + 32 * 33 + 32 * 32 + 32 + 37 * 16 + 16 * 8 + 8)
    nbytes = n * (12 + 12 + s + (8 if idx is not None else 0))
    if 2 <= s <= 4 and kernels.blend == "transposed":
        L.call("gens_blend_views_t", L.ptr_table(feats, align=16), L.int_table(hw), nl, L.ptr(aligned16(views.imgs_tex.detach()), align=16),
               L.ptr(views.w2c), L.ptr(views.intr), L.ptr(views.c2w), views.nv, L.ptr(plan.t_stream), L.ptr(plan.t_tab), plan.scalars, L.ptr(pts),
               L.ptr(idx, torch.int64), n, L.ptr(count, torch.int32), L.ptr(rgb_out), L.ptr(vis_out, torch.uint8), L.stream(),
               live=None if count is None else (count, n), nbytes=nbytes, flops=n * flops, label="gens_blend_views")
        if not plan.finite:
            _poison(idx, count, rgb_out)
        return rgb_out, vis_out
    L.call("gens_blend_views", L.ptr_table(feats, align=16), L.int_table(hw), nl, L.ptr(aligned16(views.imgs_tex.detach()), align=16), L.ptr(views.w2c), L.ptr(views.intr),
           L.ptr(views.c2w), views.nv, plan.table, plan.scalars, L.ptr(pts), L.ptr(idx, torch.int64), n, L.ptr(count, torch.int32),
           L.ptr(rgb_out), L.ptr(vis_out, torch.uint8), L.stream(), live=None if count is None else (count, n), nbytes=nbytes, flops=n * flops)
    if not plan.finite:
        _poison(idx, count, rgb_out)
    return rgb_out, vis_out


def blend_params(net):
    mods = [net.ray_dir_fc[0], net.ray_dir_fc[2], net.base_fc[0], net.base_fc[2], net.vis_fc[0], net.vis_fc[2], net.vis_fc2[0], net.vis_fc2[2],
            net.rgb_fc[0], net.rgb_fc[2], net.rgb_fc[4]]
    out = []
    for m in mods:
        out += [m.weight, m.bias]
    return out + [net.s]


class _BlendTrain(torch.autograd.Function):

    @staticmethod
    def forward(ctx, pts, views, sel, *tensors):
        params, imgs_tex, feat_tex = tensors[:23], tensors[23], tensors[24:]
        n, s, nl = (pts.shape[0] if sel is None else sel.n_ray), views.nv - 1, len(feat_tex)
        dev = pts.device
        idx, cnt = (None, None) if sel is None else (sel.idx, sel.counts[1:2])
        w = [_c(p.detach().to(_f32)).reshape(-1) if p.dim() == 0 else _c(p.detach().to(_f32)) for p in params]
        feats = [aligned16(f.detach()) for f in feat_tex]
        imgs = aligned16(imgs_tex.detach())
        hw = [d for f in feats for d in f.shape[1:3]]
        if sel is None:
            rgb = torch.empty(n, 3, device=dev, dtype=_f32)
            vis = torch.empty(n, s, device=dev, dtype=torch.uint8)
        else:
            rgb, vis = sel.rgb, sel.vis
        f = 3 + 4 * nl
        flops = 2 * s * (4 * 16 + 16 * f + 3 * f * 64 + 64 * 32 + 32 * 32 + 32 * 33 + 32 * 32 + 32 + 37 * 16 + 16 * 8 + 8)
        ctx.args = (L.ptr_table(feats, align=16), L.int_table(hw), nl, L.ptr(imgs, align=16), L.ptr(views.w2c), L.ptr(views.intr), L.ptr(views.c2w),
                    views.nv, L.ptr_table(w), L.ptr(pts), L.ptr(idx, torch.int64), n, L.ptr(cnt, torch.int32))
        ctx.keep = (feats, imgs, w, views, pts, hw, idx, cnt)
        ctx.meta = (n, s, nl, f, flops, [p.shape for p in params], [t.shape for t in feat_tex], imgs_tex.shape)
        ctx.live = None if cnt is None else (cnt, n)
        if 2 <= s <= 4 and kernels.blend_train_fwd == "transposed":
            groups = L.load().gens_blend_views_t_groups(nl)
            wstream = torch.empty((groups + 2) * 64 * 4, device=dev, dtype=_f32)
            tab, sc = torch.empty(320, device=dev, dtype=_f32), torch.empty(4, device=dev, dtype=_f32)
            L.call("gens_blend_pack_t", L.ptr_table(w), nl, L.ptr(wstream, align=16), L.ptr(tab), L.ptr(sc), L.stream())
            L.call("gens_blend_views_t_dev", ctx.args[0], ctx.args[1], nl, ctx.args[3], ctx.args[4], ctx.args[5], ctx.args[6], views.nv, L.ptr(wstream),
                   L.ptr(tab), L.ptr(sc), L.ptr(pts), L.ptr(idx, torch.int64), n, L.ptr(cnt, torch.int32), L.ptr(rgb), L.ptr(vis, torch.uint8), L.stream(),
                   nbytes=n * (24 + s), flops=n * flops, live=ctx.live, label="gens_blend_train_fwd")
        else:
            L.call("gens_blend_train_fwd", *ctx.args, L.ptr(rgb), L.ptr(vis, torch.uint8), L.stream(), nbytes=n * (24 + s), flops=n * flops, live=ctx.live)
        ctx.mark_non_differentiable(vis)
        return rgb, vis

    @staticmethod
    @torch.autograd.function.once_differentiable
    def backward(ctx, g_rgb, _g_vis):
        n, s, nl, f, flops, pshapes, fshapes, ishape = ctx.meta
        feats, imgs, w, views, pts, hw, idx, cnt = ctx.keep
        dev = pts.device
        rows = L.load().gens_blend_train_rows(n, views.nv)
        ins = [4, 16, 3 * f, 64, 32, 32, 32, 32, 37, 16, 8]
        outs = [16, f, 64, 32, 32, 33, 32, 1, 16, 8, 1]
        e = lambda *shape: torch.empty(*shape, device=dev, dtype=_f32)
        ev = lambda x: (x + 1) // 2 * 2
        want_maps = any(ctx.needs_input_grad[3 + 23:])
        g_feat = e(n, s, f) if want_maps else None
        true_flops = (2 * flops + 2 * s * sum(m * (k + 1) for m, k in zip(outs, ins))) * n
        kernels.blend_bwd_round5_count_ratio = (3 * flops + 2 * s * sum(m * (k + 1) for m, k in zip(outs, ins))) * n / max(true_flops, 1)
        if 2 <= s <= 4 and kernels.blend_train_bwd == "transposed" and kernels.blend_train_wgrad == "inside" and n > 0:
            lib = L.load()
            csz = lib.gens_blend_train_acc_floats(nl)
            n_parts = lib.gens_blend_train_t_parts(n, views.nv)
            parts, cc, s_part = e(n_parts, csz), e(csz), e(n_parts)
            L.call("gens_blend_train_bwd_t", *ctx.args, L.ptr(_c(g_rgb.to(_f32))), L.ptr(g_feat), L.ptr(s_part), L.ptr(parts), L.ptr(cc), L.stream(),
                   nbytes=4 * n * (3 + s * f), flops=true_flops, live=ctx.live, label="gens_blend_train_bwd")
            return _BlendTrain._finish(ctx, cc, s_part, g_feat, w, f, nl, pshapes, fshapes, ishape, want_maps, views, pts, hw, idx, cnt, n, dev)
        s_part = e(rows // 32) if n else torch.zeros(rows // 32, device=dev, dtype=_f32)
        if kernels.blend_train_wgrad == "inside":
            lib = L.load()
            csz = lib.gens_blend_train_acc_floats(nl)
            assert csz == sum(ev(m) * ev(k + 1) for m, k in zip(outs, ins))
            parts = e(lib.gens_blend_train_acc_parts(n, views.nv), csz)
            cc = torch.zeros(csz, device=dev, dtype=_f32) if n == 0 else e(csz)
            L.call("gens_blend_train_bwd_acc", *ctx.args, L.ptr(_c(g_rgb.to(_f32))), L.ptr(g_feat), L.ptr(s_part), L.ptr(parts), L.ptr(cc), L.stream(),
                   nbytes=4 * n * (3 + s * f), flops=true_flops, live=ctx.live, label="gens_blend_train_bwd")
            return _BlendTrain._finish(ctx, cc, s_part, g_feat, w, f, nl, pshapes, fshapes, ishape, want_maps, views, pts, hw, idx, cnt, n, dev)
        r_ops = [e(rows, ev(k + 1)) for k in ins]
        l_ops = [e(rows, ev(m)) for m in outs]
        L.call("gens_blend_train_bwd", *ctx.args, L.ptr(_c(g_rgb.to(_f32))), L.ptr_table(r_ops), L.ptr_table(l_ops), L.ptr(g_feat), L.ptr(s_part),
               L.stream(), nbytes=4 * rows * (sum(ins) + 11 + sum(outs)), flops=2 * n * flops, live=ctx.live)
        ms, ns = [ev(m) for m in outs], [ev(k + 1) for k in ins]
        mi, ni = L.int_table(ms), L.int_table(ns)
        ws = e(L.load().gens_gemm_tn_batch_workspace(11, mi, ni, rows))
        cc = e(sum(m * k for m, k in zip(ms, ns)))
        if cnt is None:
            L.call("gens_gemm_tn_batch", 11, L.ptr_table(l_ops), mi, L.ptr_table(r_ops), ni, mi, ni, rows, L.ptr(ws), L.ptr(cc), L.stream(),
                   nbytes=4 * rows * (sum(ms) + sum(ns)), flops=2 * rows * sum(m * k for m, k in zip(ms, ns)))
        else:
            L.call("gens_gemm_tn_batch_live", 11, L.ptr_table(l_ops), mi, L.ptr_table(r_ops), ni, mi, ni, rows, L.ptr(cnt, torch.int32), 32 // s, 32,
                   L.ptr(ws), L.ptr(cc), L.stream(), nbytes=4 * rows * (sum(ms) + sum(ns)), flops=2 * rows * sum(m * k for m, k in zip(ms, ns)),
                   live=ctx.live, label="gens_gemm_tn_batch")
        return _BlendTrain._finish(ctx, cc, s_part, g_feat, w, f, nl, pshapes, fshapes, ishape, want_maps, views, pts, hw, idx, cnt, n, dev)

    @staticmethod
    def _finish(ctx, cc, s_part, g_feat, w, f, nl, pshapes, fshapes, ishape, want_maps, views, pts, hw, idx, cnt, n, dev):
        e = lambda *shape: torch.empty(*shape, device=dev, dtype=_f32)
        sizes = [math.prod(sh) if len(sh) else 1 for sh in pshapes]
        flat = e(sum(sizes))
        grads, off = [], 0
        for sh, sz in zip(pshapes, sizes):
            grads.append(flat[off:off + sz].view(sh))
            off += sz
        L.call("gens_blend_train_wgrad", L.ptr(cc), L.ptr(s_part), s_part.numel(), L.ptr(w[22]), f, L.ptr_table([g_.reshape(-1) for g_ in grads]), L.stream())
        g_imgs, g_feats = None, [None] * nl
        if want_maps:
            want_img = ctx.needs_input_grad[3 + 23]
            want_feat = any(ctx.needs_input_grad[3 + 24:])
            g_feats_t = [torch.zeros(sh, device=dev, dtype=_f32) for sh in fshapes] if want_feat else None
            g_imgs = torch.zeros(ishape, device=dev, dtype=_f32) if want_img else None
            L.call("gens_lookup_feature_bwd_idx", L.int_table(hw), nl, L.ptr(views.w2c), L.ptr(views.intr), views.nv, L.ptr(pts), L.ptr(g_feat),
                   L.ptr(idx, torch.int64), n, L.ptr(cnt, torch.int32), L.ptr_table(g_feats_t), L.ptr(g_imgs), L.stream(), label="gens_lookup_feature_bwd")
            if want_feat:
                g_feats = g_feats_t
        return (None, None, None, *grads, g_imgs, *g_feats)


def blend_train(net, views, pts, sel=None):
    pts = _c(pts.detach().reshape(-1, 3).to(_f32))
    rgb, vis = _BlendTrain.apply(pts, views, sel, *blend_params(net), views.imgs_tex, *views.feat_tex)
    return rgb, (vis if sel is not None else vis.bool())


class StepPoints:

    def __init__(self, pts_all, valid_all, n_ray, n_always, n_src, z=None, variance=None):
        dev = pts_all.device
        self.pts = pts_all
        self.n, self.n_ray, self.n_always = int(pts_all.shape[0]), int(n_ray), int(n_always)
        n = self.n
        self.idx = torch.empty(n, device=dev, dtype=torch.int64)
        self.counts = torch.empty(3, device=dev, dtype=torch.int32)
        self.y, self.g, self.s = (torch.empty(n, k, device=dev, dtype=_f32) for k in (1, 3, 3))
        self.rgb = torch.empty(self.n_ray, 3, device=dev, dtype=_f32)
        self.vis = torch.empty(self.n_ray, n_src, device=dev, dtype=torch.uint8)
        self.scalars = torch.empty(4, device=dev, dtype=_f32)
        zc = None if z is None else _c(z.detach())
        scratch = torch.empty(L.load().gens_compact_points_scratch(n), device=dev, dtype=torch.int32)
        L.call("gens_compact_points", L.ptr(_c(valid_all), torch.uint8), self.n_ray, self.n_always, n, L.ptr(self.idx, torch.int64),
               L.ptr(self.counts, torch.int32), L.ptr(self.y), L.ptr(self.g), L.ptr(self.s), L.ptr(self.rgb), L.ptr(self.vis, torch.uint8), n_src,
               L.ptr(zc), 0 if zc is None else zc.numel(), L.ptr(None if variance is None else _c(variance.detach().reshape(1))), L.ptr(self.scalars),
               L.ptr(scratch, torch.int32), L.stream(), nbytes=n * 9)


__all__ = [n_ for n_ in dir() if not n_.startswith("__")]
```

include/gens_hip.h:

```cpp
#ifndef GENS_HIP_H
#define GENS_HIP_H

#include <stdint.h>

#ifdef __cplusplus
extern "C" {
#endif

#define GENS_MAX_LEVELS 8
#define GENS_MAX_VIEWS 16

#define GENS_EINVAL (-1)
#define GENS_ELIMIT (-2)

#define GENS_LAYOUT_PLANAR 0
#define GENS_LAYOUT_PACKED 1

const char* gens_last_error(void);
int gens_abi_version(void);


int gens_pack_nchw(const float* src, float* dst, int n, int c, int h, int w, void* stream);
int gens_unpack_nhwc(const float* src, float* dst, int n, int c, int h, int w, void* stream);
int gens_pack_volume(const float* src, float* dst, int x, int y, int z, void* stream);

int gens_volume_build_fwd(const float* feat, const float* w2c, const float* intr, float intr_scale, int nv, int h,
                          int w, int d, int min_vis_view, float* volume, float* mask, void* stream);
int gens_volume_build_bwd(const float* feat, const float* w2c, const float* intr, float intr_scale, int nv, int h,
                          int w, int d, const float* g_volume, float* g_feat, void* stream);
int gens_volume_build_levels(const float* const* feat, const int* hw, const int* dims, int n_levels, const float* w2c,
                             const float* const* intr, int nv, int min_vis_view, float* const* volumes, float* const* masks,
                             uint8_t* const* counts, void* stream);
int gens_volume_build_levels_bits(const float* const* feat, const int* hw, const int* dims, int n_levels, const float* w2c,
                                  const float* const* intr, int nv, int min_vis_view, float* const* volumes, float* const* masks,
                                  uint8_t* const* counts, uint32_t* const* mask_bits, void* stream);
int64_t gens_volume_build_bwd_levels_scratch_bytes(const int* hw, const int* dims, int n_levels, int nv);
int gens_volume_build_bwd_levels(const float* const* feat, const int* hw, const int* dims, int n_levels, const float* w2c,
                                 const float* const* intr, int nv, const float* const* volumes, const uint8_t* const* counts,
                                 const float* const* g_volumes, float* const* g_feat, void* scratch, int64_t scratch_bytes, void* stream);
int gens_selftest_division(unsigned long long* counts, void* stream);

int gens_lookup_volume_fwd(const float* const* vols, const int* dims, int n_levels, int layout, const float* pts,
                           int64_t n, float* out, void* stream);
int gens_lookup_volume_bwd(const float* const* vols, const int* dims, int n_levels, int layout, const float* pts,
                           const float* g_out, int64_t n, float* const* g_vols, float* g_pts, void* stream);
int gens_lookup_volume_bwd2(const float* const* vols, const int* dims, int n_levels, int layout, const float* pts,
                            const float* g_out, const float* gg_pts, const float* const* gg_vols, int64_t n,
                            float* gg_out, float* const* g_vols2, float* g_pts2, void* stream);
int64_t gens_lookup_scatter_bricks_scratch_bytes(int64_t n);
int gens_lookup_volume_bwd_bricks(const float* const* vols, const int* dims, int n_levels, int layout, const float* pts,
                                  const float* g_out, int64_t n, float* const* g_vols, float* g_pts, void* scratch,
                                  int64_t scratch_bytes, void* stream);
int gens_lookup_volume_bwd2_bricks(const float* const* vols, const int* dims, int n_levels, int layout, const float* pts,
                                   const float* g_out, const float* gg_pts, const float* const* gg_vols, int64_t n,
                                   float* gg_out, float* const* g_vols2, float* g_pts2, void* scratch, int64_t scratch_bytes,
                                   void* stream);

int gens_lookup_mask_nearest(const float* const* masks, const int* dims, int n_levels, const float* pts, int64_t n,
                             uint8_t* valid, float* vals, void* stream);
int gens_ray_points(const float* rays_o, const float* rays_d, const float* z, int64_t n_rays, int n_samples, int mid,
                    float sample_dist, const float* const* masks, const int* dims, int n_levels, int mask_bits,
                    float* pts, uint8_t* valid, void* stream);
int gens_pack_mask_bits(const float* mask, int64_t n, uint32_t* bits, void* stream);

int gens_compact_valid(const uint8_t* valid, int64_t n, int64_t* idx, int32_t* count, int32_t* scratch, void* stream);

int gens_lookup_feature_fwd(const float* const* feats, const int* hw, int n_levels, const float* imgs,
                            const float* w2c, const float* intr, const float* c2w, int nv, const float* pts,
                            int64_t n, float* out, float* ray_diff, uint8_t* vis, void* stream);
int gens_lookup_feature_bwd(const int* hw, int n_levels, const float* w2c, const float* intr, int nv,
                            const float* pts, const float* g_out, int64_t n, float* const* g_feats, float* g_imgs,
                            void* stream);
int gens_lookup_feature_bwd_idx(const int* hw, int n_levels, const float* w2c, const float* intr, int nv,
                                const float* pts, const float* g_out, const int64_t* index, int64_t n, const int32_t* n_device,
                                float* const* g_feats, float* g_imgs, void* stream);

int gens_upsample(const float* rays_o, const float* rays_d, const float* z, const float* sdf, int64_t n_rays, int n,
                  int n_new, float inv_s, const float* const* masks, const int* dims, int n_levels, int mask_bits,
                  const uint8_t* valid_in, float* z_new, float* pts_new, uint8_t* valid_new, void* stream);
int gens_merge_samples(const float* z, const float* sdf, const float* z_new, const float* sdf_new, const uint8_t* valid,
                       const uint8_t* valid_new, int64_t n_rays, int n, int n_new, float* z_out, float* sdf_out,
                       uint8_t* valid_out, void* stream);
int gens_merge_upsample(const float* rays_o, const float* rays_d, const float* z, const float* sdf, const uint8_t* valid,
                        const float* z_add, const float* sdf_add, const uint8_t* valid_add, int64_t n_rays, int n, int n_add, int n_new,
                        float inv_s, float sample_dist, const float* const* masks, const int* dims, int n_levels, int mask_bits, int mode,
                        float* z_out, float* sdf_out, uint8_t* valid_out, float* z_new, float* pts_out, uint8_t* valid_new, void* stream);

typedef struct {
    const float *rays_o, *rays_d, *z, *sdf, *grad, *color, *smooth;
    const uint8_t *voxel_mask, *src_vis;
    const float *inv_s, *z_max;
    int64_t n_rays;
    int n, n_src;
    float sample_dist, cos_anneal;
    float rot[9];
    const float* rot_dev;
    const float* cos_anneal_dev;
} gens_composite_in;

typedef struct {
    float *color, *normal, *depth, *wsum, *wmax, *mid_in, *sdf_depth, *z_cross, *eik_num, *eik_den, *smooth_vec;
    uint8_t* valid;
    int32_t* cross_idx;
    float *weights, *inside;
    float* pts_cross;
} gens_composite_out;

typedef struct {
    const float *g_color, *g_normal, *g_depth, *g_weights, *g_wsum, *g_eik_num, *g_smooth_vec, *g_z_cross;
    const float* weights;
    const int32_t* cross_idx;
    const float* smooth_vec;
    float *g_sdf, *g_grad, *g_col, *g_smooth, *g_inv_s;
    const float *g_gradient_error, *g_smooth_error, *finish;
} gens_composite_grad;

int gens_composite_fwd(const gens_composite_in* in, const gens_composite_out* out, void* stream);
int gens_composite_bwd(const gens_composite_in* in, const gens_composite_grad* g, void* stream);
int gens_composite_finish_fwd(const float* eik_num, const float* eik_den, const float* smooth_vec, int64_t n_rays, float* finish, void* stream);
int gens_composite_finish_bwd(const float* g_inv_s, int64_t n_rays, const float* scalars, float* g_variance, float* g_sdf, float* g_grad,
                              float* g_smooth, int64_t n_ray_pts, int64_t n_all, void* stream);

int gens_sdf_mlp(const float* const* vols_packed, const int* dims, int n_levels, const float* const* wf,
                 const float* const* wb, const float* w_last, const float* w_last_scaled, float b_last, float scale,
                 const float* pts, const int64_t* index, int64_t n, const int32_t* n_device, float* sdf_out, float* grad_out,
                 void* stream);

int gens_sdf_mlp_dev(const float* const* vols_packed, const int* dims, int n_levels, const float* const* wf,
                     const float* const* wb, const float* w_last, const float* b_last_dev, float scale,
                     const float* pts, const int64_t* index, int64_t n, const int32_t* n_device, float* sdf_out, float* grad_out,
                     void* stream);

int gens_sdf_value(const float* const* vols_packed, const int* dims, int n_levels, const float* wstream, const float* w_out,
                   float b_last, float scale, const float* pts, const int64_t* index, int64_t n, const int32_t* n_device,
                   float* sdf_out, void* stream);
int gens_sdf_value_groups(int n_levels);

int gens_sdf_grad(const float* const* vols_packed, const int* dims, int n_levels, const float* wstream, const float* w_out,
                  float b_last, float scale, const float* pts, const int64_t* index, int64_t n, const int32_t* n_device,
                  float* sdf_out, float* grad_out, void* stash, void* stream);
int64_t gens_sdf_grad_stash_bytes(void);
int gens_sdf_grad_stash_reset(void* stash, void* stream);
int gens_sdf_grad_groups(int n_levels);

int gens_sdf_value_f16(const float* const* vols_packed, const int* dims, int n_levels, const void* units, const float* w_out,
                       float b_last, float scale, const float* pts, const int64_t* index, int64_t n, const int32_t* n_device,
                       float* sdf_out, int* overflow_flag, void* stream);
int gens_sdf_value_f16_units(int n_levels);

int gens_sdf_grad_f16(const float* const* vols_packed, const int* dims, int n_levels, const void* pieces, const float* w_out,
                      float b_last, float scale, float g_scale, const float* pts, const int64_t* index, int64_t n,
                      const int32_t* n_device, float* sdf_out, float* grad_out, void* stash, int* overflow_flag, void* stream);
int64_t gens_sdf_grad_f16_stash_bytes(void);
int gens_sdf_grad_f16_stash_reset(void* stash, void* stream);
int gens_sdf_grad_f16_pieces(int n_levels);

int gens_sdf_value_bf16x3(const float* const* vols_packed, const int* dims, int n_levels, const void* pieces, const float* w_out,
                          float b_last, float scale, const float* pts, const int64_t* index, int64_t n, const int32_t* n_device,
                          float* sdf_out, void* stream);
int gens_sdf_grad_bf16x3(const float* const* vols_packed, const int* dims, int n_levels, const void* pieces, const float* w_out,
                         float b_last, float scale, const float* pts, const int64_t* index, int64_t n, const int32_t* n_device,
                         float* sdf_out, float* grad_out, void* stash, void* stream);
int gens_sdf_bf16x3_pieces(int n_levels);

int gens_depthwise_conv2d_fwd(const float* in, const float* weight, int n, int c, int h, int w, int k, int stride, float* out, void* stream);
int gens_depthwise_conv2d_dgrad(const float* grad_out, const float* weight, int n, int c, int h, int w, int k, int stride, float* grad_in,
                                void* stream);
int gens_depthwise_conv2d_wgrad_parts(int n, int c, int h, int w, int k, int stride);
int gens_depthwise_conv2d_wgrad(const float* in, const float* grad_out, int n, int c, int h, int w, int k, int stride, float* partial,
                                void* stream);

int64_t gens_batchnorm2d_scratch_doubles(int n, int c, int hw);
int gens_batchnorm2d_train_fwd(const float* x, const float* gamma, const float* beta, int n, int c, int hw, float eps, float momentum, int relu,
                               float* y, float* mean_rstd, float* running_mean, float* running_var, int64_t* num_batches_tracked,
                               double* scratch, void* stream);
int gens_batchnorm2d_train_bwd(const float* x, const float* grad_y, const float* mean_rstd, const float* gamma, const float* beta, int n, int c,
                               int hw, int relu, float* grad_x, float* grad_gamma, float* grad_beta, double* scratch, void* stream);

int gens_grid_sample_fwd(const float* input, const float* grid, int ndim, int n, int c, const int* in_size, int64_t n_out,
                         int padding_mode, int align_corners, float* out, void* stream);
int gens_grid_sample_bwd(const float* grad_out, const float* input, const float* grid, int ndim, int n, int c, const int* in_size,
                         int64_t n_out, int padding_mode, int align_corners, float* grad_input, float* grad_grid, void* stream);
int gens_grid_sample_bwd2(const float* gg_input, const float* gg_grid, const float* grad_out, const float* input, const float* grid,
                          int ndim, int n, int c, const int* in_size, int64_t n_out, int padding_mode, int align_corners,
                          float* gg_out, float* grad_input, float* grad_grid, void* stream);

int gens_sdf_train_pack_wn(const float* const* v, const float* const* g, const float* const* b, int n_levels, float* const* scale,
                           float* const* wf, float* const* wb, float* w_last, float* b_last, void* stream);
int gens_sdf_train_wgrad(const float* const* v, const float* const* g, int n_levels, const float* cc, const float* w6_sum,
                         float* const* dv, float* const* dg, float* const* db, void* stream);
int64_t gens_sdf_train_stash_bytes(int64_t n, int backward);
int gens_sdf_train_pack(const float* const* w, const float* const* b, int n_levels, float* const* wf, float* const* wb, void* stream);
int gens_sdf_train_fwd(const float* const* vols_packed, const int* dims, int n_levels, const float* const* wf,
                       const float* const* wb, const float* w_last, const float* b_last, const float* pts, const int64_t* index,
                       int64_t n, const int32_t* n_device, void* stash, float* y_out, float* g_out, float* s_out, void* stream);
int gens_sdf_train_bwd(const float* const* vols_packed, const int* dims, int n_levels, const float* const* wf,
                       const float* const* wb, const float* w_last, const float* pts, const int64_t* index, int64_t n,
                       const int32_t* n_device, const float* y_bar, const float* g_bar, const float* s_bar, void* stash, float* lop,
                       float* rh, float* re, float* r0, float* f_hat, float* mu_f, float* lam_f, float* w6_part, void* stream);
int gens_sdf_train_scatter(const int* dims, int n_levels, const float* pts, const float* g_bar, const float* s_bar,
                           const float* f_hat, const float* mu_f, const float* lam_f, const int64_t* index, int64_t n,
                           const int32_t* n_device, float* const* g_vols, void* stream);

int gens_blend_views(const float* const* feats, const int* hw, int n_levels, const float* imgs, const float* w2c,
                     const float* intr, const float* c2w, int nv, const float* const* weights, const float* scalars,
                     const float* pts, const int64_t* index, int64_t n, const int32_t* n_device, float* rgb_out, uint8_t* vis_out,
                     void* stream);

int gens_blend_views_t(const float* const* feats, const int* hw, int n_levels, const float* imgs, const float* w2c, const float* intr,
                       const float* c2w, int nv, const float* wstream, const float* tab, const float* scalars, const float* pts,
                       const int64_t* index, int64_t n, const int32_t* n_device, float* rgb_out, uint8_t* vis_out, void* stream);
int gens_blend_views_t_groups(int n_levels);
int gens_blend_pack_t(const float* const* weights, int n_levels, float* wstream, float* tab, float* scalars_dev, void* stream);
int gens_blend_views_t_dev(const float* const* feats, const int* hw, int n_levels, const float* imgs, const float* w2c, const float* intr,
                           const float* c2w, int nv, const float* wstream, const float* tab, const float* scalars_dev, const float* pts,
                           const int64_t* index, int64_t n, const int32_t* n_device, float* rgb_out, uint8_t* vis_out, void* stream);
int gens_blend_views4(const float* const* feats, const int* hw, int n_levels, const float* imgs, const float* w2c, const float* intr,
                      const float* c2w, int nv, const float* wstream, const float* tab, const float* scalars, const float* pts,
                      const int64_t* index, int64_t n, const int32_t* n_device, float* rgb_out, uint8_t* vis_out, void* stream);
int gens_blend_views4_groups(int n_levels);

int64_t gens_blend_train_rows(int64_t n, int nv);
int gens_blend_train_fwd(const float* const* feats, const int* hw, int n_levels, const float* imgs, const float* w2c, const float* intr,
                         const float* c2w, int nv, const float* const* weights, const float* pts, const int64_t* index, int64_t n,
                         const int32_t* n_device, float* rgb_out, uint8_t* vis_out, void* stream);
int gens_blend_train_bwd(const float* const* feats, const int* hw, int n_levels, const float* imgs, const float* w2c, const float* intr,
                         const float* c2w, int nv, const float* const* weights, const float* pts, const int64_t* index, int64_t n,
                         const int32_t* n_device, const float* g_rgb, float* const* r_ops, float* const* l_ops, float* g_feat,
                         float* s_part, void* stream);
int gens_blend_train_acc_parts(int64_t n, int nv);
int gens_blend_train_acc_floats(int n_levels);
int gens_blend_train_bwd_acc(const float* const* feats, const int* hw, int n_levels, const float* imgs, const float* w2c, const float* intr,
                             const float* c2w, int nv, const float* const* weights, const float* pts, const int64_t* index, int64_t n,
                             const int32_t* n_device, const float* g_rgb, float* g_feat, float* s_part, float* parts, float* cc, void* stream);
int gens_blend_train_t_parts(int64_t n, int nv);
int gens_blend_train_bwd_t(const float* const* feats, const int* hw, int n_levels, const float* imgs, const float* w2c, const float* intr,
                           const float* c2w, int nv, const float* const* weights, const float* pts, const int64_t* index, int64_t n,
                           const int32_t* n_device, const float* g_rgb, float* g_feat, float* s_part, float* parts, float* cc, void* stream);
int gens_blend_train_bwd_t_dump(const float* const* feats, const int* hw, int n_levels, const float* imgs, const float* w2c, const float* intr,
                                const float* c2w, int nv, const float* const* weights, const float* pts, const int64_t* index, int64_t n,
                                const int32_t* n_device, const float* g_rgb, float* g_feat, float* s_part, float* parts, float* cc,
                                float* const* r_ops, float* const* l_ops, void* stream);

int gens_patch_sample_fwd(const float* image, int h, int w, int c, const float* xy, int64_t p, float* out,
                          void* stream);
int gens_patch_sample_bwd(const float* image, int h, int w, int c, const float* xy, const float* g_out, int64_t p,
                          float* g_xy, void* stream);
int gens_upsample2d_into(const float* src, int n, int c, int hs, int ws, float* dst, int h, int w, int c_pad_dst,
                         int c_off, void* stream);
int gens_upsample2d_cat(const float* const* srcs, const int* chw, int n_maps, int n, float* dst, int h, int w, int c_pad_dst,
                        void* stream);

int gens_lncc_fwd(const float* ref, const float* src, int64_t n_rays, int n_src, int n_patch, int n_ch, float* ncc, int32_t* sel,
                  void* stream);
int gens_lncc_bwd(const float* ref, const float* src, const float* g_ncc, const int32_t* sel, int64_t n_rays, int n_src, int n_patch,
                  int n_ch, float* g_ref, float* g_src, void* stream);

int gens_mc_classify(const float* u, int x, int y, int z, float iso, const uint8_t* tri_count, uint8_t* vmask,
                     uint8_t* vcount, uint8_t* cases, uint8_t* tcount, void* stream);
int gens_mc_emit(const float* u, int x, int y, int z, float iso, const int8_t* tri_table, int table_stride,
                 const uint8_t* vmask, const int32_t* voff, const uint8_t* cases, const uint8_t* tcount, const int32_t* toff,
                 double* vertices, int32_t* triangles, void* stream);

int gens_tv_blocks(int64_t n_voxels);
int gens_tv_fwd(const float* vol, const float* mask, int x, int y, int z, float* partial, void* stream);
int gens_tv_bwd(const float* vol, const float* mask, int x, int y, int z, float coef, float* g_vol, void* stream);
int gens_tv_bwd_scaled(const float* vol, const float* mask, int x, int y, int z, float coef, const float* coef_dev, float* g_vol,
                       void* stream);

int gens_lattice_points(const float* bmin3_host, const float* bmax3_host, int res, int64_t first, int64_t count,
                        float* pts, void* stream);

typedef struct {
    const double* vertices;
    const int32_t* triangles;
    const int32_t* cell_start;
    int32_t* cell_faces;
    int64_t n_faces;
    float lo_x, lo_y, lo_z, cell;
    int nx, ny, nz;
} gens_mesh_grid;
int gens_mesh_grid_count(const gens_mesh_grid* grid, int32_t* counts, void* stream);
int gens_mesh_grid_fill(const gens_mesh_grid* grid, int32_t* cursor, void* stream);
int gens_ray_first_hit(const gens_mesh_grid* grid, const float* rays_o, const float* rays_d, int64_t n_rays, int32_t* face, float* t,
                       void* stream);
int gens_view_rays_hit_faces(const gens_mesh_grid* grid, const float* masks, const float* cams, int nv, int h, int w, int hu, int wu,
                             float inv_scale, uint8_t* flags, int32_t* any_miss, void* stream);
int gens_face_cc_hook(const int32_t* pairs, int64_t n_pairs, int32_t* parent, int64_t n_faces, void* stream);
int gens_face_cc_compress(const int32_t* parent, int64_t n_faces, int32_t* label, void* stream);

typedef struct {
    const double* points;
    double* sorted;
    const int32_t* cell_start;
    int32_t* cell_points;
    int64_t n;
    double lo_x, lo_y, lo_z, cell;
    int nx, ny, nz;
} gens_point_grid;
int gens_mesh_sample_count(const double* vertices, int64_t n_vertices, const int32_t* triangles, int64_t n_triangles, double density,
                           int64_t* counts, void* stream);
int gens_mesh_sample_emit(const double* vertices, int64_t n_vertices, const int32_t* triangles, int64_t n_triangles, double density,
                          const int64_t* offsets, int64_t total, double* out, void* stream);
int gens_point_grid_count(const gens_point_grid* grid, int32_t* counts, void* stream);
int gens_point_grid_fill(const gens_point_grid* grid, int32_t* cursor, void* stream);
int gens_radius_downsample_round(const gens_point_grid* grid, const int32_t* rank, double radius, const uint8_t* state_in, uint8_t* state_out,
                                 int32_t* undecided, void* stream);
int gens_nearest_point(const gens_point_grid* grid, const double* queries, int64_t n_queries, double max_dist, double* dist, int32_t* index,
                       void* stream);

int gens_dilate_u8(const uint8_t* in, uint8_t* out, int n, int h, int w, int c, int channels, int kw, int kh, const int* half_spans_host,
                   void* stream);
int gens_vertex_mask_votes(const double* points, int64_t n_points, const float* proj, const uint8_t* masks, int nv, int h, int w,
                           int32_t* votes, void* stream);
int gens_view_rays_hit_counts(const gens_mesh_grid* grid, const uint8_t* masks, const float* cams, int nv, int h, int w, float dep_min,
                              uint8_t* flags, int32_t* any_miss, void* stream);

int gens_filter_masks(const float* u, float thresh, const float* const* masks_in, float* const* masks_out, uint32_t* const* bits_out,
                      const int* dims, int n_levels, uint32_t* band_words, int64_t* counts, void* stream);
int gens_filter_band(const float* u, float thresh, int d0, uint32_t* band_words, int64_t* counts, void* stream);
int gens_filter_levels(const float* const* masks_in, float* const* masks_out, uint32_t* const* bits_out, const int* dims, int n_levels,
                       const uint32_t* band_words, int64_t* counts, void* stream);

int64_t gens_components_scratch_bytes(int nx, int ny, int nz);
int gens_largest_component(const uint32_t* bits_in, int nx, int ny, int nz, int connectivity, uint32_t* bits_out, void* scratch,
                           int64_t* results, void* stream);
int gens_unpack_mask_bits(const uint32_t* bits, int64_t n, float* mask, void* stream);

int gens_sparse_coarse_points(const float* bmin3_host, const float* bmax3_host, int res, int brick, int64_t first, int64_t count, float* pts,
                              void* stream);
int gens_sparse_classify(const float* uc, int res, int brick, float t, float margin, uint8_t* flags, void* stream);
int gens_sparse_brick_points(const float* bmin3_host, const float* bmax3_host, int res, int brick, const int64_t* list, int64_t n_list,
                             int64_t first, int64_t count, float* pts, void* stream);
int gens_sparse_fill(const float* uc, int res, int brick, float* u, void* stream);
int gens_sparse_scatter(const float* sdf, int res, int brick, const int64_t* list, int64_t n_list, int64_t first, int64_t count, float* u,
                        void* stream);
int gens_sparse_leaks(const float* u, int res, int brick, const uint8_t* flags, float t, int64_t* leaks, void* stream);

int gens_gemm_tn_slabs(int64_t k, int m, int n);
int gens_gemm_tn(const float* a, const float* b, int64_t k, int m, int n, float* workspace, float* c, void* stream);
int64_t gens_gemm_tn_batch_workspace(int count, const int* m, const int* n, int64_t k);
int gens_gemm_tn_batch(int count, const float* const* a, const int* lda, const float* const* b, const int* ldb, const int* m,
                       const int* n, int64_t k, float* workspace, float* c, void* stream);
int gens_gemm_tn_batch_live(int count, const float* const* a, const int* lda, const float* const* b, const int* ldb, const int* m,
                            const int* n, int64_t k, const int32_t* k_live, int k_div, int k_rows, float* workspace, float* c,
                            void* stream);

int gens_conv3d_gather(const float* q, const float* w, const float* bias, int cp, int cq, const int* dims_p, int stride,
                       float* p, void* stream);
int gens_conv3d_scatter2(const float* p, const float* w, int cp, int cq, const int* dims_p, float* q, void* stream);
int gens_conv3d_wgrad_parts(int cp, int cq, const int* dims_p);
int gens_conv3d_wgrad_parts_strided(int cp, int cq, const int* dims_p, int stride);
int gens_conv3d_wgrad(const float* p, const float* q, int cp, int cq, const int* dims_p, int stride, float* workspace, void* stream);

int gens_instnorm_blocks(int c, int64_t n);
int gens_instnorm_stats(const float* x, int c, int64_t n, double* partials, void* stream);
int gens_instnorm_finish(const double* partials, int c, int64_t n, double eps, int mode, float* out, void* stream);
int gens_instnorm_relu_fwd(const float* x, const float* mean_rstd, int c, int64_t n, float* y, void* stream);
int gens_instnorm_relu_add_fwd(const float* x, const float* mean_rstd, const float* skip, int c, int64_t n, float* y, void* stream);
int gens_instnorm_relu_bwd_stats(const float* x, const float* gy, const float* mean_rstd, int c, int64_t n, double* partials, void* stream);
int gens_instnorm_relu_bwd(const float* x, const float* gy, const float* mean_rstd, const float* g_means, int c, int64_t n, float* gx,
                           void* stream);

int gens_patch_warp_fwd(const float* rays_o, const float* rays_d, const float* z, const float* g0, int64_t n_rays, const float* c2ws,
                        const float* intrs, const float* kinv_ref, int nv, const float* tex, int h, int w, int c, int patch, float* ref,
                        float* sampled, void* stream);
int gens_patch_warp_bwd(const float* rays_o, const float* rays_d, const float* z, const float* g0, int64_t n_rays, const float* c2ws,
                        const float* intrs, const float* kinv_ref, int nv, const float* tex, int h, int w, int c, int patch,
                        const float* g_sampled, float* g_z, void* stream);
typedef struct {
    const float *color, *target;
    const uint8_t* valid;
    int64_t b;
    const float* sparse;
    int64_t n_sparse;
    float sparse_scale;
    const float* pseudo;
    int64_t n_pseudo;
    const float *ncc, *mid_in;
    const float *depth, *pseudo_depth_t, *depth_t;
    const float *ge, *se, *tv;
    float w_color, w_igr, w_sparse, w_mfc, w_smooth, w_tv, w_pseudo_sdf, w_pseudo_depth;
    float* out;
    const float* g;
    float *g_color, *g_sparse, *g_pseudo, *g_ncc, *g_depth, *g_scalars;
} gens_loss_args;
int gens_loss_fwd(const gens_loss_args* args, void* stream);
int gens_loss_bwd(const gens_loss_args* args, void* stream);
int gens_coarse_z(const float* near, const float* far, int per_ray, const float* steps, const float* t_rand, int64_t n_rays, int n, float* z,
                  void* stream);
int gens_blend_train_wgrad(const float* cc, const float* s_part, int n_part, const float* s, int n_feat, float* const* grads, void* stream);
int64_t gens_scene_cams_floats(int nv);
int gens_scene_setup(const float* c2ws, const float* intrs, int nv, float* cams, void* stream);
int gens_pack_maps(const float* const* src, float* const* dst, const int* nchw, int n_maps, void* stream);
int gens_unpack_maps(const float* const* src, float* const* dst, const int* nchw, int n_maps, void* stream);
int gens_select_views(const float* const* src, float* const* dst, const int* floats_per_view, const int* views_in_src, int n_maps,
                      const int64_t* index, int n_sel, void* stream);
int64_t gens_compact_points_scratch(int64_t n);
int gens_compact_points(const uint8_t* valid, int64_t n_ray_pts, int64_t n_always, int64_t n, int64_t* idx, int32_t* counts,
                        float* y_fill, float* g_fill, float* s_fill, float* rgb_fill, uint8_t* vis_fill, int n_src, const float* z,
                        int64_t nz, const float* variance, float* scalars, int32_t* scratch, void* stream);
int gens_tv_levels_blocks(const int* dims, int n_levels);
int gens_tv_levels_fwd(const float* const* vols, const float* const* masks, const int* dims, int n_levels, float* partial, float* out,
                       void* stream);
int gens_tv_levels_bwd(const float* const* vols, const float* const* masks, const int* dims, int n_levels, const float* out,
                       const float* g, float* const* g_vols, void* stream);

#ifdef __cplusplus
}
#endif
#endif
```

Before: 237.8 million ray-samples/s.

## Add bf16x3 split-precision MFMA blend kernel alongside fp32 transposed path

```diff
diff --git a/gens_amd/csrc/k6b_sdf_bf16x3.hip b/gens_amd/csrc/k6b_sdf_bf16x3.hip
--- a/gens_amd/csrc/k6b_sdf_bf16x3.hip
+++ b/gens_amd/csrc/k6b_sdf_bf16x3.hip
@@ -1,15 +1,12 @@
 #include "common.h"
+#include "split3.h"
 
 typedef float f32x16 __attribute__((ext_vector_type(16)));
-typedef float f32x2v __attribute__((ext_vector_type(2)));
 typedef float f32x4v __attribute__((ext_vector_type(4)));
-typedef __bf16 bf16x2 __attribute__((ext_vector_type(2)));
-typedef __bf16 bf16x8 __attribute__((ext_vector_type(8)));
-typedef uint32_t u32x4 __attribute__((ext_vector_type(4)));
 
 #define GB_WAVES 4
 #define GB_PIECE 1024
-#define GB_TERMS 3
+#define GB_TERMS SPLIT3_TERMS
 #define GB_CH 8
 #define GB_RING 4
 #define GB_GT 2
@@ -23,29 +20,6 @@
 #define GB_SLOTS 2048
 #define GB_C 144.26950408889634f
 
-struct Split3Block {
-    u32x4 p[GB_TERMS];
-};
-
-struct Split3Word {
-    uint32_t w[GB_TERMS];
-};
-__device__ __forceinline__ uint32_t pk_bf16(float a, float b) {
-    return __builtin_bit_cast(uint32_t, __builtin_convertvector((f32x2v){a, b}, bf16x2));
-}
-__device__ __forceinline__ Split3Word split3_pair(float a, float b) {
-    Split3Word s;
-#pragma unroll
-    for (int k = 0; k < GB_TERMS; ++k) {
-        const uint32_t w = pk_bf16(a, b);
-        s.w[k] = w;
-        if (k + 1 < GB_TERMS) {
-            a -= __builtin_bit_cast(float, w << 16);
-            b -= __builtin_bit_cast(float, w & 0xffff0000u);
-        }
-    }
-    return s;
-}
 #define GB_PUT(BLK_, W_, A_, B_)                                            \
     {                                                                       \
         const Split3Word sw__ = split3_pair((A_), (B_));                    \
diff --git a/gens_amd/csrc/k7b_blend_bf16x3.hip b/gens_amd/csrc/k7b_blend_bf16x3.hip
--- /dev/null
+++ b/gens_amd/csrc/k7b_blend_bf16x3.hip
@@ -0,0 +1,418 @@
+#include "k7t_rows.h"
+#include "split3.h"
+
+struct BlendBWeights {
+    const u32x4* stream;
+    const float* tab;
+    float v2_last_b, u2_b, r3_b, s_abs;
+};
+
+__device__ __forceinline__ f32x2v elu2b(f32x2v x) {
+    const f32x2v t = x * 1.44269504088896340736f;
+    const f32x2v e = (f32x2v){__builtin_amdgcn_exp2f(t[0]), __builtin_amdgcn_exp2f(t[1])} - 1.0f;
+    return (f32x2v){__builtin_amdgcn_fmed3f(x[0], e[0], 0.0f), __builtin_amdgcn_fmed3f(x[1], e[1], 0.0f)};
+}
+__device__ __forceinline__ f32x4 elu4b(f32x4 x) {
+    const f32x2v lo = elu2b((f32x2v){x[0], x[1]}), hi = elu2b((f32x2v){x[2], x[3]});
+    return (f32x4){lo[0], lo[1], hi[0], hi[1]};
+}
+
+template <int NLEV, int S>
+__global__ __launch_bounds__(64, 2) void blend_b_k(BlendBWeights W, MapSet fs, const float4* __restrict__ imgs, const float* __restrict__ w2c,
+                                                   const float* __restrict__ intr, const float* __restrict__ c2w, const float* __restrict__ pts,
+                                                   const int64_t* __restrict__ index, int64_t n_max, const int32_t* __restrict__ n_dev,
+                                                   float* __restrict__ rgb_out, uint8_t* __restrict__ vis_out) {
+    constexpr int XQ = NLEV + 1;
+    constexpr int XT = (XQ + 3) / 4;
+    constexpr int NB_MV = (2 * XQ + 7) / 8;
+    constexpr int G = S == 2 ? 2 : 4;
+    constexpr int PPT = 16 / G;
+    constexpr int PPW = 64 / G;
+    constexpr int NPT = PPW / 16;
+    static_assert(S >= 2 && S <= 4, "two to four source views");
+    static_assert(4 * XQ <= KT_XS && XQ <= 8, "feature tile too narrow");
+    __shared__ float X[64 * KT_XS];
+    __shared__ float RD[64 * 5];
+    __shared__ float R[64];
+    const int lane = threadIdx.x;
+    const int np = lane & 15, q = lane >> 4;
+    const int64_t n = n_dev ? min(n_max, (int64_t)n_dev[0]) : n_max;
+    const int64_t first = (int64_t)blockIdx.x * PPW;
+    if (first >= n) return;
+
+    const u32x4* wp = W.stream;
+    u32x4 wb[3][3];
+    int par = 0;
+#pragma unroll
+    for (int g = 0; g < 2; ++g)
+#pragma unroll
+        for (int k = 0; k < 3; ++k) wb[g][k] = wp[lane + 64 * (3 * g + k)];
+    wp += 384;
+
+    blend_gather_row<NLEV, S>(fs, imgs, w2c, intr, c2w, pts, index, first, n, vis_out, lane, X, RD, R);
+    __syncthreads();
+
+    float xq[KT_NT][XQ];
+    float rgbc[KT_NT];
+    float rdq[KT_NT], dotv[KT_NT], mask[KT_NT], rd3one[KT_NT], rdsh[KT_NT];
+#pragma unroll
+    for (int j = 0; j < KT_NT; ++j) {
+        const int row = 16 * j + np;
+#pragma unroll
+        for (int kq = 0; kq < XQ; ++kq) xq[j][kq] = X[row * KT_XS + 4 * kq + q];
+        rgbc[j] = xq[j][0];
+        rdq[j] = RD[row * 5 + q];
+        dotv[j] = RD[row * 5 + 3];
+        mask[j] = R[row];
+        rdsh[j] = q ? RD[row * 5 + q - 1] : 0.0f;
+        rd3one[j] = q == 0 ? dotv[j] : (q == 1 ? 1.0f : 0.0f);
+    }
+    const float* tab = W.tab + q * 8;
+#define KB_TAB(E, K) tab[(E) * 32 + (K)]
+#define KB_BIAS(E, T) ((f32x4){KB_TAB(E, 4 * (T)), KB_TAB(E, 4 * (T) + 1), KB_TAB(E, 4 * (T) + 2), KB_TAB(E, 4 * (T) + 3)})
+
+#define KB_NEXT()                                                                                        \
+    const u32x4 a0_ = wb[par][0], a1_ = wb[par][1], a2_ = wb[par][2];                                    \
+    _Pragma("unroll") for (int k_ = 0; k_ < 3; ++k_) wb[(par + 2) % 3][k_] = wp[lane + 64 * k_];          \
+    wp += 192;                                                                                           \
+    par = (par + 1) % 3;
+#define KB_MFMA(A_, B_, C_) __builtin_amdgcn_mfma_f32_16x16x32_bf16(__builtin_bit_cast(bf16x8, (A_)), __builtin_bit_cast(bf16x8, (B_)), (C_), 0, 0, 0)
+#define KB_GROUP(NT_, ACC_, C0_, B_, BLK_)                                                               \
+    {                                                                                                    \
+        KB_NEXT()                                                                                        \
+        _Pragma("unroll") for (int j_ = 0; j_ < (NT_); ++j_) ACC_(j_) = KB_MFMA(a2_, B_(j_, (BLK_)).p[0], C0_(j_));  \
+        _Pragma("unroll") for (int j_ = 0; j_ < (NT_); ++j_) ACC_(j_) = KB_MFMA(a1_, B_(j_, (BLK_)).p[1], ACC_(j_)); \
+        _Pragma("unroll") for (int j_ = 0; j_ < (NT_); ++j_) ACC_(j_) = KB_MFMA(a0_, B_(j_, (BLK_)).p[2], ACC_(j_)); \
+        _Pragma("unroll") for (int j_ = 0; j_ < (NT_); ++j_) ACC_(j_) = KB_MFMA(a1_, B_(j_, (BLK_)).p[0], ACC_(j_)); \
+        _Pragma("unroll") for (int j_ = 0; j_ < (NT_); ++j_) ACC_(j_) = KB_MFMA(a0_, B_(j_, (BLK_)).p[1], ACC_(j_)); \
+        _Pragma("unroll") for (int j_ = 0; j_ < (NT_); ++j_) ACC_(j_) = KB_MFMA(a0_, B_(j_, (BLK_)).p[0], ACC_(j_)); \
+    }
+#define KB_PRODUCT(NT_, MT_, NB_, B_)                                                                    \
+    _Pragma("unroll") for (int T_ = 0; T_ < (MT_); ++T_)                                                 \
+        _Pragma("unroll") for (int b_ = 0; b_ < (NB_); ++b_) {                                           \
+            if (b_ == 0) KB_GROUP(NT_, ACC_T_, INIT_T_, B_, 0)                                           \
+            else KB_GROUP(NT_, ACC_T_, ACC_T_, B_, b_)                                                   \
+        }
+#define KB_F32(A_, NQ_, ACC_, C0_, B_)                                                                   \
+    {                                                                                                    \
+        const f32x4 af_ = __builtin_bit_cast(f32x4, (A_));                                               \
+        _Pragma("unroll") for (int k_ = 0; k_ < (NQ_); ++k_)                                             \
+            _Pragma("unroll") for (int j_ = 0; j_ < KT_NT; ++j_)                                         \
+                ACC_(j_) = k_ == 0 ? __builtin_amdgcn_mfma_f32_16x16x4f32(af_[0], B_(j_, 0), C0_(j_), 0, 0, 0)          \
+                                   : __builtin_amdgcn_mfma_f32_16x16x4f32(af_[k_], B_(j_, k_), ACC_(j_), 0, 0, 0);      \
+    }
+#define KB_SPLIT8(BLK_, V_)                                                                              \
+    _Pragma("unroll") for (int w_ = 0; w_ < 4; ++w_) {                                                   \
+        const Split3Word sw_ = split3_pair<true>(V_(2 * w_), V_(2 * w_ + 1));                                  \
+        _Pragma("unroll") for (int k_ = 0; k_ < SPLIT3_TERMS; ++k_) (BLK_).p[k_][w_] = sw_.w[k_];        \
+    }
+
+    {
+        KB_NEXT()
+        f32x4 D[KT_NT];
+        const f32x4 b = KB_BIAS(KT_RD1_B, 0);
+#define ACC_D_(j) D[j]
+#define INIT_B_(j) b
+#define B_RD(j, k) rdq[j]
+        KB_F32(a0_, 1, ACC_D_, INIT_B_, B_RD)
+#undef INIT_B_
+#pragma unroll
+        for (int j = 0; j < KT_NT; ++j) D[j] = elu4b(D[j]);
+        f32x4 E[XT][KT_NT];
+#define B_D(j, k) D[j][k]
+#pragma unroll
+        for (int T = 0; T < XT; ++T) {
+            const f32x4 bias = KB_BIAS(KT_RD2_B, T);
+#define ACC_E_(j) E[T][j]
+#define INIT_B_(j) bias
+            KB_F32((T == 0 ? a1_ : a2_), 4, ACC_E_, INIT_B_, B_D)
+#undef ACC_E_
+#undef INIT_B_
+        }
+#undef ACC_D_
+#pragma unroll
+        for (int j = 0; j < KT_NT; ++j) {
+#pragma unroll
+            for (int T = 0; T < XT; ++T) E[T][j] = elu4b(E[T][j]);
+#pragma unroll
+            for (int kq = 0; kq < XQ; ++kq) xq[j][kq] += E[kq >> 2][j][kq & 3];
+        }
+    }
+
+    float wn[KT_NT];
+    Split3Block pmv[NPT][NB_MV];
+    const bool dead = S == 3 && (np & 3) == 3;
+    {
+        float pc[NPT][8 * NB_MV];
+        const int src = (G * (np % PPT) + 16 * q) * 4;
+#pragma unroll
+        for (int t = 0; t < NPT; ++t)
+#pragma unroll
+            for (int k = 0; k < 8 * NB_MV; ++k) pc[t][k] = 0.0f;
+#pragma unroll
+        for (int j = 0; j < KT_NT; ++j) {
+            const float e = hw_exp(W.s_abs * (dotv[j] - 1.0f));
+            const float mn = group_min<G>(dead ? __builtin_inff() : e);
+            const float wr = dead ? 0.0f : (e - mn) * mask[j];
+            wn[j] = wr / (group_sum<G>(wr) + 1e-8f);
+#pragma unroll
+            for (int kq = 0; kq < XQ; ++kq) {
+                const float mean = group_sum<G>(wn[j] * xq[j][kq]);
+                const float d = xq[j][kq] - mean;
+                const float var = group_sum<G>(wn[j] * (d * d));
+                const float tm = __builtin_bit_cast(float, __builtin_amdgcn_ds_bpermute(src, __builtin_bit_cast(int, mean)));
+                const float tv = __builtin_bit_cast(float, __builtin_amdgcn_ds_bpermute(src, __builtin_bit_cast(int, var)));
+#pragma unroll
+                for (int t = 0; t < NPT; ++t) {
+                    const bool sel = (16 * t + np) / PPT == j;
+                    pc[t][kq] = sel ? tm : pc[t][kq];
+                    pc[t][XQ + kq] = sel ? tv : pc[t][XQ + kq];
+                }
+            }
+        }
+#pragma unroll
+        for (int t = 0; t < NPT; ++t)
+#pragma unroll
+            for (int b = 0; b < NB_MV; ++b) {
+#define V_PC(k) pc[t][8 * b + (k)]
+                KB_SPLIT8(pmv[t][b], V_PC)
+#undef V_PC
+            }
+    }
+
+    Split3Block hb[KT_NT][2];
+    {
+        f32x4 H1[4][KT_NT];
+        {
+            f32x4 P[NPT][4];
+            const f32x4 zero4 = {0.f, 0.f, 0.f, 0.f};
+#define INIT_T_(j) zero4
+#define ACC_T_(j) P[j][T_]
+#define B_PMV(j, b) pmv[j][b]
+            KB_PRODUCT(NPT, 4, NB_MV, B_PMV)
+#undef ACC_T_
+#undef INIT_T_
+#pragma unroll
+            for (int j = 0; j < KT_NT; ++j) {
+                const int src = (((PPT * j) & 15) + np / G + 16 * q) * 4;
+#pragma unroll
+                for (int T = 0; T < 4; ++T)
+#pragma unroll
+                    for (int i = 0; i < 4; ++i) {
+                        float v = P[(PPT * j) >> 4][T][i];
+                        asm volatile("" : "+v"(v));
+                        H1[T][j][i] = __builtin_bit_cast(float, __builtin_amdgcn_ds_bpermute(src, __builtin_bit_cast(int, v)));
+                    }
+            }
+        }
+        Split3Block xb[KT_NT];
+#pragma unroll
+        for (int j = 0; j < KT_NT; ++j) {
+#define V_X(k) ((k) < XQ ? xq[j][(k) < XQ ? (k) : 0] : 0.0f)
+            KB_SPLIT8(xb[j], V_X)
+#undef V_X
+        }
+#define ACC_T_(j) H1[T_][j]
+#define INIT_T_(j) H1[T_][j]
+#define B_XB(j, b) xb[j]
+        KB_PRODUCT(KT_NT, 4, 1, B_XB)
+#undef ACC_T_
+#undef INIT_T_
+#pragma unroll
+        for (int j = 0; j < KT_NT; ++j)
+#pragma unroll
+            for (int b = 0; b < 2; ++b) {
+                H1[2 * b][j] = elu4b(H1[2 * b][j]);
+                H1[2 * b + 1][j] = elu4b(H1[2 * b + 1][j]);
+#define V_H1(k) H1[2 * b + ((k) >> 2)][j][(k) & 3]
+                KB_SPLIT8(hb[j][b], V_H1)
+#undef V_H1
+            }
+    }
+#define B_HB(j, b) hb[j][b]
+    f32x4 XH[2][KT_NT];
+    {
+#define ACC_T_(j) XH[T_][j]
+#define INIT_T_(j) KB_BIAS(KT_B2_B, T_)
+        KB_PRODUCT(KT_NT, 2, 2, B_HB)
+#undef ACC_T_
+#undef INIT_T_
+#pragma unroll
+        for (int T = 0; T < 2; ++T)
+#pragma unroll
+            for (int j = 0; j < KT_NT; ++j) XH[T][j] = elu4b(XH[T][j]);
+    }
+
+    f32x4 G1[2][KT_NT];
+#define KB_DOT32(ENTRY, OUT)                                                                                          \
+    _Pragma("unroll") for (int j = 0; j < KT_NT; ++j) {                                                               \
+        float s_ = 0.0f;                                                                                              \
+        _Pragma("unroll") for (int k = 0; k < 8; ++k) s_ = __builtin_fmaf(G1[k >> 2][j][k & 3], KB_TAB(ENTRY, k), s_); \
+        OUT[j] = lanes_q_sum(s_);                                                                                     \
+    }
+
+    float vis[KT_NT];
+#pragma unroll
+    for (int j = 0; j < KT_NT; ++j) {
+#define V_XS(k) (XH[(k) >> 2][j][(k) & 3] * wn[j])
+        KB_SPLIT8(hb[j][0], V_XS)
+#undef V_XS
+    }
+#define ACC_T_(j) G1[T_][j]
+#define INIT_T_(j) KB_BIAS(KT_V1_B, T_)
+    KB_PRODUCT(KT_NT, 2, 1, B_HB)
+#undef INIT_T_
+#undef ACC_T_
+#pragma unroll
+    for (int T = 0; T < 2; ++T)
+#pragma unroll
+        for (int j = 0; j < KT_NT; ++j) G1[T][j] = elu4b(G1[T][j]);
+    KB_DOT32(KT_V2_LAST, vis)
+    {
+        f32x4 V2[2][KT_NT];
+#pragma unroll
+        for (int j = 0; j < KT_NT; ++j) {
+#define V_G1(k) G1[(k) >> 2][j][(k) & 3]
+            KB_SPLIT8(hb[j][0], V_G1)
+#undef V_G1
+        }
+#define ACC_T_(j) V2[T_][j]
+#define INIT_T_(j) KB_BIAS(KT_V2_B, T_)
+        KB_PRODUCT(KT_NT, 2, 1, B_HB)
+#undef ACC_T_
+#undef INIT_T_
+#pragma unroll
+        for (int T = 0; T < 2; ++T)
+#pragma unroll
+            for (int j = 0; j < KT_NT; ++j) XH[T][j] += elu4b(V2[T][j]);
+    }
+#pragma unroll
+    for (int j = 0; j < KT_NT; ++j) vis[j] = hw_sigmoid(elu1t(vis[j] + W.v2_last_b)) * mask[j];
+
+    float vis2[KT_NT];
+    const f32x4 zero4 = {0.f, 0.f, 0.f, 0.f};
+#pragma unroll
+    for (int j = 0; j < KT_NT; ++j) {
+#define V_XH(k) XH[(k) >> 2][j][(k) & 3]
+        KB_SPLIT8(hb[j][0], V_XH)
+#undef V_XH
+    }
+#define ACC_T_(j) G1[T_][j]
+#define INIT_T_(j) zero4
+    KB_PRODUCT(KT_NT, 2, 1, B_HB)
+#undef INIT_T_
+#undef ACC_T_
+#pragma unroll
+    for (int T = 0; T < 2; ++T) {
+        const f32x4 bias = KB_BIAS(KT_U1_B, T);
+#pragma unroll
+        for (int j = 0; j < KT_NT; ++j) {
+#pragma unroll
+            for (int i = 0; i < 4; ++i) G1[T][j][i] = __builtin_fmaf(G1[T][j][i], vis[j], bias[i]);
+            G1[T][j] = elu4b(G1[T][j]);
+        }
+    }
+    KB_DOT32(KT_U2, vis2)
+#pragma unroll
+    for (int j = 0; j < KT_NT; ++j) vis2[j] = hw_sigmoid(vis2[j] + W.u2_b) * mask[j];
+
+    float score[KT_NT];
+    {
+        f32x4 C1[KT_NT], C2[KT_NT];
+#define INIT_T_(j) zero4
+#define ACC_T_(j) C1[j]
+        KB_PRODUCT(KT_NT, 1, 1, B_HB)
+#undef INIT_T_
+        {
+            KB_NEXT()
+            (void)a2_;
+#define B_R1(j, k) ((k) == 0 ? (q == 0 ? vis2[j] : rdsh[j]) : rd3one[j])
+            KB_F32(a0_, 2, ACC_T_, ACC_T_, B_R1)
+#undef ACC_T_
+#pragma unroll
+            for (int j = 0; j < KT_NT; ++j) C1[j] = elu4b(C1[j]);
+            const f32x4 b2 = KB_BIAS(KT_R2_B, 0);
+#define ACC_T_(j) C2[j]
+#define INIT_T_(j) b2
+#define B_C1(j, k) C1[j][k]
+            KB_F32(a1_, 4, ACC_T_, INIT_T_, B_C1)
+#undef ACC_T_
+#undef INIT_T_
+        }
+#pragma unroll
+        for (int j = 0; j < KT_NT; ++j) {
+            const f32x2v c2 = elu2b((f32x2v){C2[j][0], C2[j][1]});
+            const float s = c2[0] * KB_TAB(KT_R3, 0) + c2[1] * KB_TAB(KT_R3, 1);
+            score[j] = (mask[j] == 0.0f ? -1e9f : lanes_q_sum(s) + W.r3_b) + 0.0f * mask[j];
+            if (dead) score[j] = -__builtin_inff();
+        }
+    }
+
+#pragma unroll
+    for (int j = 0; j < KT_NT; ++j) {
+        const float mx = group_max<G>(score[j]);
+        const float e = hw_exp(score[j] - mx);
+        const float den = group_sum<G>(e);
+        const float col = group_sum<G>(rgbc[j] * e) / den;
+        const int64_t pt = first + PPT * j + np / G;
+        if ((np % G) == 0 && q < 3 && pt < n) {
+            const int64_t dst = index ? index[pt] : pt;
+            rgb_out[3 * dst + q] = col;
+        }
+    }
+#undef KB_TAB
+#undef KB_BIAS
+#undef KB_NEXT
+#undef KB_MFMA
+#undef KB_GROUP
+#undef KB_PRODUCT
+#undef KB_F32
+#undef KB_SPLIT8
+#undef KB_DOT32
+}
+
+int gens_fill_maps(const char* who, MapSet* ms, const float* const* feats, const int* hw, int n_levels);
+
+extern "C" int gens_blend_bf16x3_groups(int n_levels) {
+    if (n_levels < 1 || n_levels > 5) return 0;
+    const int xq = n_levels + 1;
+    return 1 + 4 * ((2 * xq + 7) / 8) + 4 + 2 * 2 + 2 + 2 + 2 + 1 + 1;
+}
+
+template <int S>
+static void blend_b_launch(int n_levels, unsigned grid, hipStream_t st, const BlendBWeights& W, const MapSet& fs, const float* imgs, const float* w2c,
+                           const float* intr, const float* c2w, const float* pts, const int64_t* index, int64_t n, const int32_t* n_device,
+                           float* rgb_out, uint8_t* vis_out) {
+#define BLEND_LAUNCH(NL) blend_b_k<NL, S><<<grid, 64, 0, st>>>(W, fs, (const float4*)imgs, w2c, intr, c2w, pts, index, n, n_device, rgb_out, vis_out)
+    switch (n_levels) {
+        case 1: BLEND_LAUNCH(1); break;
+        case 2: BLEND_LAUNCH(2); break;
+        case 3: BLEND_LAUNCH(3); break;
+        case 4: BLEND_LAUNCH(4); break;
+        default: BLEND_LAUNCH(5); break;
+    }
+#undef BLEND_LAUNCH
+}
+
+extern "C" int gens_blend_views_bf16x3(const float* const* feats, const int* hw, int n_levels, const float* imgs, const float* w2c, const float* intr,
+                                       const float* c2w, int nv, const void* wstream, const float* tab, const float* scalars, const float* pts,
+                                       const int64_t* index, int64_t n, const int32_t* n_device, float* rgb_out, uint8_t* vis_out, void* stream) {
+    MapSet fs;
+    GENS_CHECK_ARG(feats && wstream && tab && scalars, GENS_EINVAL, "gens_blend_views_bf16x3: null table");
+    if (int e = gens_fill_maps("gens_blend_views_bf16x3", &fs, feats, hw, n_levels)) return e;
+    GENS_CHECK_ARG(n_levels <= 5, GENS_ELIMIT, "gens_blend_views_bf16x3: at most 5 feature levels (d_feature <= 20), got %d", n_levels);
+    GENS_CHECK_ARG(nv >= 3 && nv <= 5, GENS_ELIMIT, "gens_blend_views_bf16x3: built for two to four source views (nv = 3..5), got nv=%d (use gens_blend_views)", nv);
+    GENS_CHECK_ARG(imgs && w2c && intr && c2w, GENS_EINVAL, "gens_blend_views_bf16x3: null camera / image pointer");
+    GENS_CHECK_ARG(((uintptr_t)wstream & 15) == 0, GENS_EINVAL, "gens_blend_views_bf16x3: the weight stream must be 16-byte aligned");
+    GENS_CHECK_ARG(n >= 0 && (n == 0 || (pts && rgb_out)), GENS_EINVAL, "gens_blend_views_bf16x3: null pts / output");
+    if (n == 0) return 0;
+    BlendBWeights W;
+    W.stream = (const u32x4*)wstream;
+    W.tab = tab;
+    W.v2_last_b = scalars[0]; W.u2_b = scalars[1]; W.r3_b = scalars[2]; W.s_abs = scalars[3];
+    hipStream_t st = (hipStream_t)stream;
+    if (nv == 3) blend_b_launch<2>(n_levels, gens_blocks(n, 32), st, W, fs, imgs, w2c, intr, c2w, pts, index, n, n_device, rgb_out, vis_out);
+    else if (nv == 4) blend_b_launch<3>(n_levels, gens_blocks(n, 16), st, W, fs, imgs, w2c, intr, c2w, pts, index, n, n_device, rgb_out, vis_out);
+    else blend_b_launch<4>(n_levels, gens_blocks(n, 16), st, W, fs, imgs, w2c, intr, c2w, pts, index, n, n_device, rgb_out, vis_out);
+    return gens_launch_status("gens_blend_views_bf16x3");
+}
diff --git a/gens_amd/csrc/k7t_blend.hip b/gens_amd/csrc/k7t_blend.hip
--- a/gens_amd/csrc/k7t_blend.hip
+++ b/gens_amd/csrc/k7t_blend.hip
@@ -1,9 +1,4 @@
-#include "k4_common.h"
-
-typedef float f32x4 __attribute__((ext_vector_type(4)));
-
-#define KT_NT 4
-#define KT_XS 29
+#include "k7t_rows.h"
 
 struct BlendTWeights {
     const float4* stream;
@@ -11,39 +6,12 @@
     float v2_last_b, u2_b, r3_b, s_abs;
     const float* sdev;
 };
-enum { KT_RD1_B = 0, KT_RD2_B, KT_B2_B, KT_V1_B, KT_V2_B, KT_U1_B, KT_R2_B, KT_V2_LAST, KT_U2, KT_R3, KT_TAB_ENTRIES };
-
-__device__ __forceinline__ float elu1t(float x) { return __builtin_amdgcn_fmed3f(x, hw_exp(x) - 1.0f, 0.0f); }
-template <int G>
-__device__ __forceinline__ float group_sum(float v) {
-    v += dpp_move<0xB1, 0xF>(v, v);
-    if (G == 4) v += dpp_move<0x4E, 0xF>(v, v);
-    return v;
-}
-template <int G>
-__device__ __forceinline__ float group_min(float v) {
-    v = fminf(v, dpp_move<0xB1, 0xF>(v, v));
-    if (G == 4) v = fminf(v, dpp_move<0x4E, 0xF>(v, v));
-    return v;
-}
-template <int G>
-__device__ __forceinline__ float group_max(float v) {
-    v = fmaxf(v, dpp_move<0xB1, 0xF>(v, v));
-    if (G == 4) v = fmaxf(v, dpp_move<0x4E, 0xF>(v, v));
-    return v;
-}
-__device__ __forceinline__ float lanes_q_sum(float v) {
-    v += __shfl_xor(v, 16, 64);
-    v += __shfl_xor(v, 32, 64);
-    return v;
-}
 
 template <int NLEV, int S>
 __global__ __launch_bounds__(64, 2) void blend_t_k(BlendTWeights W, MapSet fs, const float4* __restrict__ imgs, const float* __restrict__ w2c,
                                                    const float* __restrict__ intr, const float* __restrict__ c2w, const float* __restrict__ pts,
                                                    const int64_t* __restrict__ index, int64_t n_max, const int32_t* __restrict__ n_dev,
                                                    float* __restrict__ rgb_out, uint8_t* __restrict__ vis_out) {
-    constexpr int F = 3 + 4 * NLEV;
     constexpr int XQ = NLEV + 1;
     constexpr int XT = (XQ + 3) / 4;
     constexpr int G = S == 2 ? 2 : 4;
@@ -69,51 +37,7 @@
     wb[1] = wp[lane + 64];
     wp += 128;
 
-    {
-        const int pl = lane / G, sv = (lane % G) + 1;
-        const bool live = first + pl < n && sv <= S;
-        const int64_t src = live ? (index ? index[first + pl] : first + pl) : 0;
-        float x = 0.f, y = 0.f, z = 0.f;
-        if (live) { x = pts[3 * src]; y = pts[3 * src + 1]; z = pts[3 * src + 2]; }
-        bool inside = true;
-        float* xr = X + lane * KT_XS;
-        const int svc = sv <= S ? sv : S;
-        const SrcBase pb = project_src_base(w2c + 16 * svc, intr + 16 * svc, x, y, z);
-#pragma unroll
-        for (int l = 0; l < NLEV; ++l) {
-            const int h = fs.h[l], w = fs.w[l];
-            const SrcProj p = project_src_level(pb, exp2f(-(float)l), h, w, fs.cw[l], fs.ch[l], fs.rcw[l], fs.rch[l]);
-            inside = inside && p.inside;
-            float4 f = f4_zero(), c = f4_zero();
-            if (live) {
-                const Taps2 t = bilinear_taps(p.ix, p.iy, h, w);
-                f = sample_texel(fs.data[l] + (int64_t)svc * h * w, h, w, 1, 0, t);
-                if (l == 0) c = sample_texel(imgs + (int64_t)svc * h * w, h, w, 1, 0, t);
-            }
-            xr[3 + 4 * l] = f.x; xr[4 + 4 * l] = f.y; xr[5 + 4 * l] = f.z; xr[6 + 4 * l] = f.w;
-            if (l == 0) { xr[0] = c.x; xr[1] = c.y; xr[2] = c.z; }
-        }
-        xr[F] = 1.0f;
-        float acc_in = x + y + z;
-#pragma unroll
-        for (int k = 0; k < F; ++k) acc_in += xr[k];
-        R[lane] = ((live && inside) ? 1.0f : 0.0f) + 0.0f * acc_in;
-        if (live && vis_out) vis_out[src * S + (sv - 1)] = inside ? 1 : 0;
-        float rx = c2w[3] - x, ry = c2w[7] - y, rz = c2w[11] - z;
-        const float rn = hw_rcp(__builtin_amdgcn_sqrtf(rx * rx + ry * ry + rz * rz) + 1e-6f);
-        rx *= rn; ry *= rn; rz *= rn;
-        const float* cs = c2w + 16 * svc;
-        float sx = cs[3] - x, sy = cs[7] - y, sz = cs[11] - z;
-        const float sn = hw_rcp(__builtin_amdgcn_sqrtf(sx * sx + sy * sy + sz * sz) + 1e-6f);
-        sx *= sn; sy *= sn; sz *= sn;
-        const float dx = rx - sx, dy = ry - sy, dz = rz - sz;
-        const float dn = hw_rcp(fmaxf(__builtin_amdgcn_sqrtf(dx * dx + dy * dy + dz * dz), 1e-6f));
-        float* rd = RD + lane * 5;
-        rd[0] = live ? dx * dn : 0.0f;
-        rd[1] = live ? dy * dn : 0.0f;
-        rd[2] = live ? dz * dn : 0.0f;
-        rd[3] = live ? rx * sx + ry * sy + rz * sz : 0.0f;
-    }
+    blend_gather_row<NLEV, S>(fs, imgs, w2c, intr, c2w, pts, index, first, n, vis_out, lane, X, RD, R);
     __syncthreads();
 
     float xq[KT_NT][XQ];
diff --git a/gens_amd/csrc/k7t_rows.h b/gens_amd/csrc/k7t_rows.h
--- /dev/null
+++ b/gens_amd/csrc/k7t_rows.h
@@ -0,0 +1,86 @@
+#pragma once
+#include "k4_common.h"
+
+typedef float f32x4 __attribute__((ext_vector_type(4)));
+
+#define KT_NT 4
+#define KT_XS 29
+
+enum { KT_RD1_B = 0, KT_RD2_B, KT_B2_B, KT_V1_B, KT_V2_B, KT_U1_B, KT_R2_B, KT_V2_LAST, KT_U2, KT_R3, KT_TAB_ENTRIES };
+
+__device__ __forceinline__ float elu1t(float x) { return __builtin_amdgcn_fmed3f(x, hw_exp(x) - 1.0f, 0.0f); }
+template <int G>
+__device__ __forceinline__ float group_sum(float v) {
+    v += dpp_move<0xB1, 0xF>(v, v);
+    if (G == 4) v += dpp_move<0x4E, 0xF>(v, v);
+    return v;
+}
+template <int G>
+__device__ __forceinline__ float group_min(float v) {
+    v = fminf(v, dpp_move<0xB1, 0xF>(v, v));
+    if (G == 4) v = fminf(v, dpp_move<0x4E, 0xF>(v, v));
+    return v;
+}
+template <int G>
+__device__ __forceinline__ float group_max(float v) {
+    v = fmaxf(v, dpp_move<0xB1, 0xF>(v, v));
+    if (G == 4) v = fmaxf(v, dpp_move<0x4E, 0xF>(v, v));
+    return v;
+}
+__device__ __forceinline__ float lanes_q_sum(float v) {
+    v += __shfl_xor(v, 16, 64);
+    v += __shfl_xor(v, 32, 64);
+    return v;
+}
+
+template <int NLEV, int S>
+__device__ __forceinline__ void blend_gather_row(const MapSet& fs, const float4* __restrict__ imgs, const float* __restrict__ w2c,
+                                                 const float* __restrict__ intr, const float* __restrict__ c2w, const float* __restrict__ pts,
+                                                 const int64_t* __restrict__ index, int64_t first, int64_t n, uint8_t* __restrict__ vis_out,
+                                                 int lane, float* X, float* RD, float* R) {
+    constexpr int F = 3 + 4 * NLEV;
+    constexpr int G = S == 2 ? 2 : 4;
+    const int pl = lane / G, sv = (lane % G) + 1;
+    const bool live = first + pl < n && sv <= S;
+    const int64_t src = live ? (index ? index[first + pl] : first + pl) : 0;
+    float x = 0.f, y = 0.f, z = 0.f;
+    if (live) { x = pts[3 * src]; y = pts[3 * src + 1]; z = pts[3 * src + 2]; }
+    bool inside = true;
+    float* xr = X + lane * KT_XS;
+    const int svc = sv <= S ? sv : S;
+    const SrcBase pb = project_src_base(w2c + 16 * svc, intr + 16 * svc, x, y, z);
+#pragma unroll
+    for (int l = 0; l < NLEV; ++l) {
+        const int h = fs.h[l], w = fs.w[l];
+        const SrcProj p = project_src_level(pb, exp2f(-(float)l), h, w, fs.cw[l], fs.ch[l], fs.rcw[l], fs.rch[l]);
+        inside = inside && p.inside;
+        float4 f = f4_zero(), c = f4_zero();
+        if (live) {
+            const Taps2 t = bilinear_taps(p.ix, p.iy, h, w);
+            f = sample_texel(fs.data[l] + (int64_t)svc * h * w, h, w, 1, 0, t);
+            if (l == 0) c = sample_texel(imgs + (int64_t)svc * h * w, h, w, 1, 0, t);
+        }
+        xr[3 + 4 * l] = f.x; xr[4 + 4 * l] = f.y; xr[5 + 4 * l] = f.z; xr[6 + 4 * l] = f.w;
+        if (l == 0) { xr[0] = c.x; xr[1] = c.y; xr[2] = c.z; }
+    }
+    xr[F] = 1.0f;
+    float acc_in = x + y + z;
+#pragma unroll
+    for (int k = 0; k < F; ++k) acc_in += xr[k];
+    R[lane] = ((live && inside) ? 1.0f : 0.0f) + 0.0f * acc_in;
+    if (live && vis_out) vis_out[src * S + (sv - 1)] = inside ? 1 : 0;
+    float rx = c2w[3] - x, ry = c2w[7] - y, rz = c2w[11] - z;
+    const float rn = hw_rcp(__builtin_amdgcn_sqrtf(rx * rx + ry * ry + rz * rz) + 1e-6f);
+    rx *= rn; ry *= rn; rz *= rn;
+    const float* cs = c2w + 16 * svc;
+    float sx = cs[3] - x, sy = cs[7] - y, sz = cs[11] - z;
+    const float sn = hw_rcp(__builtin_amdgcn_sqrtf(sx * sx + sy * sy + sz * sz) + 1e-6f);
+    sx *= sn; sy *= sn; sz *= sn;
+    const float dx = rx - sx, dy = ry - sy, dz = rz - sz;
+    const float dn = hw_rcp(fmaxf(__builtin_amdgcn_sqrtf(dx * dx + dy * dy + dz * dz), 1e-6f));
+    float* rd = RD + lane * 5;
+    rd[0] = live ? dx * dn : 0.0f;
+    rd[1] = live ? dy * dn : 0.0f;
+    rd[2] = live ? dz * dn : 0.0f;
+    rd[3] = live ? rx * sx + ry * sy + rz * sz : 0.0f;
+}
diff --git a/gens_amd/csrc/split3.h b/gens_amd/csrc/split3.h
--- /dev/null
+++ b/gens_amd/csrc/split3.h
@@ -0,0 +1,40 @@
+#pragma once
+#include <stdint.h>
+
+typedef float f32x2v __attribute__((ext_vector_type(2)));
+typedef __bf16 bf16x2 __attribute__((ext_vector_type(2)));
+typedef __bf16 bf16x8 __attribute__((ext_vector_type(8)));
+typedef uint32_t u32x4 __attribute__((ext_vector_type(4)));
+
+#define SPLIT3_TERMS 3
+
+struct Split3Block {
+    u32x4 p[SPLIT3_TERMS];
+};
+
+struct Split3Word {
+    uint32_t w[SPLIT3_TERMS];
+};
+__device__ __forceinline__ uint32_t pk_bf16(float a, float b) {
+    return __builtin_bit_cast(uint32_t, __builtin_convertvector((f32x2v){a, b}, bf16x2));
+}
+template <bool PACKED = false>
+__device__ __forceinline__ Split3Word split3_pair(float a, float b) {
+    Split3Word s;
+#pragma unroll
+    for (int k = 0; k < SPLIT3_TERMS; ++k) {
+        const uint32_t w = pk_bf16(a, b);
+        s.w[k] = w;
+        if (k + 1 < SPLIT3_TERMS) {
+            if (PACKED) {
+                const f32x2v r = (f32x2v){a, b} - (f32x2v){__builtin_bit_cast(float, w << 16), __builtin_bit_cast(float, w & 0xffff0000u)};
+                a = r[0];
+                b = r[1];
+            } else {
+                a -= __builtin_bit_cast(float, w << 16);
+                b -= __builtin_bit_cast(float, w & 0xffff0000u);
+            }
+        }
+    }
+    return s;
+}
diff --git a/gens_amd/lib.py b/gens_amd/lib.py
--- a/gens_amd/lib.py
+++ b/gens_amd/lib.py
@@ -107,6 +107,8 @@
     "gens_blend_views4_groups": [_i],
     "gens_blend_views_t": [_pp, _ip, _i, _p, _p, _p, _p, _i, _p, _p, _fp, _p, _p, _l, _p, _p, _p, _p],
     "gens_blend_views_t_groups": [_i],
+    "gens_blend_views_bf16x3": [_pp, _ip, _i, _p, _p, _p, _p, _i, _p, _p, _fp, _p, _p, _l, _p, _p, _p, _p],
+    "gens_blend_bf16x3_groups": [_i],
     "gens_blend_pack_t": [_pp, _i, _p, _p, _p, _p],
     "gens_blend_views_t_dev": [_pp, _ip, _i, _p, _p, _p, _p, _i, _p, _p, _p, _p, _p, _l, _p, _p, _p, _p],
     "gens_compact_valid": [_p, _l, _p, _p, _p, _p],
diff --git a/gens_amd/ops/base.py b/gens_amd/ops/base.py
--- a/gens_amd/ops/base.py
+++ b/gens_amd/ops/base.py
@@ -16,7 +16,7 @@
         self.sdf_value = "rowmajor" if env.get("GENS_SDF_VALUE_ROWMAJOR") else f32_mfma
         self.sdf_grad = "rowmajor" if env.get("GENS_SDF_GRAD_ROWMAJOR") else f32_mfma
         self.sdf_grad_f16 = not env.get("GENS_SDF_GRAD_F32_ONLY")
-        self.blend = "rowmajor" if env.get("GENS_BLEND_ROWMAJOR") else "transposed"
+        self.blend = "rowmajor" if env.get("GENS_BLEND_ROWMAJOR") else "transposed" if env.get("GENS_BLEND_F32_MFMA") else "bf16x3"
         self.blend_train_fwd = "rowmajor" if env.get("GENS_BLEND_TRAIN_ROWMAJOR") else "transposed"
         self.blend_train_wgrad = "rows" if env.get("GENS_K18_OPERAND_ROWS") else "inside"
         self.blend_train_bwd = "rowmajor" if env.get("GENS_BLEND_TRAIN_BWD_ROWMAJOR") or env.get("GENS_K18_OPERAND_ROWS") else "transposed"
diff --git a/gens_amd/ops/blend.py b/gens_amd/ops/blend.py
--- a/gens_amd/ops/blend.py
+++ b/gens_amd/ops/blend.py
@@ -7,47 +7,57 @@
     return out
 
 
+def _blend_fragments(w, slots, m_tiles, bias=None, quads=4):
+    dev = w.device
+    lane = torch.arange(64, device=dev)
+    m, qk = lane & 15, lane >> 4
+    row_in_tile = 4 * (m & 3) + (m >> 2)
+    o = w.shape[0]
+    aug = torch.cat([w, (bias if bias is not None else torch.zeros(o, device=dev))[:, None], torch.zeros(o, 1, device=dev)], 1)
+    aug = torch.cat([aug, torch.zeros(16 * m_tiles - o, aug.shape[1], device=dev)], 0) if 16 * m_tiles > o else aug
+    cols = torch.tensor([c if c >= 0 else (w.shape[1] if c == -1 else w.shape[1] + 1) for c in slots], device=dev)
+    nq = (len(slots) + 3) // 4
+    cols = torch.cat([cols, torch.full((4 * nq - len(slots),), w.shape[1] + 1, device=dev)])
+    groups = []
+    for t in range(m_tiles):
+        rows = 16 * t + row_in_tile
+        for g in range((nq + quads - 1) // quads):
+            frag = torch.zeros(64, quads, device=dev, dtype=_f32)
+            for j in range(quads):
+                kq = quads * g + j
+                if kq < nq:
+                    frag[:, j] = aug[rows, cols[4 * kq + qk]]
+            groups.append(frag)
+    return groups
+
+
+def _blend_products(layers, n_feat):
+    f = n_feat
+    xq = (f + 1) // 4
+    xt = (xq + 3) // 4
+    pad = [-2] * (4 * xq - f)
+    b1, r1 = layers["b1"], layers["r1"]
+    return dict(rd1=(layers["rd1"][0], [0, 1, 2, 3], 1, None),
+                rd2=(layers["rd2"][0], list(range(16)), xt, None),
+                b1mv=(b1[0], list(range(f)) + pad + list(range(f, 2 * f)) + pad, 4, None),
+                b1x=(b1[0], list(range(2 * f, 3 * f)) + [-1], 4, b1[1]),
+                b2=(layers["b2"][0], list(range(64)), 2, None),
+                v1=(layers["v1"][0], list(range(32)), 2, None),
+                v2=(layers["v2"][0][:32], list(range(32)), 2, None),
+                u1=(layers["u1"][0], list(range(32)), 2, None),
+                r1=(r1[0], list(range(36)) + [36, -1, -2, -2], 1, r1[1]),
+                r2=(layers["r2"][0], list(range(16)), 1, None))
+
+
 def _pack_blend_t(layers, n_feat):
     f = n_feat
     xq = (f + 1) // 4
     dev = layers["rd1"][0].device
-    lane = torch.arange(64, device=dev)
-    m, qk = lane & 15, lane >> 4
-    row_in_tile = 4 * (m & 3) + (m >> 2)
-
-    def product(w, slots, m_tiles, bias=None):
-        o = w.shape[0]
-        aug = torch.cat([w, (bias if bias is not None else torch.zeros(o, device=dev))[:, None], torch.zeros(o, 1, device=dev)], 1)
-        aug = torch.cat([aug, torch.zeros(16 * m_tiles - o, aug.shape[1], device=dev)], 0) if 16 * m_tiles > o else aug
-        cols = torch.tensor([c if c >= 0 else (w.shape[1] if c == -1 else w.shape[1] + 1) for c in slots], device=dev)
-        nq = (len(slots) + 3) // 4
-        cols = torch.cat([cols, torch.full((4 * nq - len(slots),), w.shape[1] + 1, device=dev)])
-        groups = []
-        for t in range(m_tiles):
-            rows = 16 * t + row_in_tile
-            for g in range((nq + 3) // 4):
-                frag = torch.zeros(64, 4, device=dev, dtype=_f32)
-                for j in range(4):
-                    kq = 4 * g + j
-                    if kq < nq:
-                        frag[:, j] = aug[rows, cols[4 * kq + qk]]
-                groups.append(frag)
-        return groups
-
-    rd1, rd2, b1, b2, v1, v2, u1, u2, r1, r2, r3 = (layers[k] for k in ("rd1", "rd2", "b1", "b2", "v1", "v2", "u1", "u2", "r1", "r2", "r3"))
+    rd1, rd2, b2, v1, v2, u1, u2, r2, r3 = (layers[k] for k in ("rd1", "rd2", "b2", "v1", "v2", "u1", "u2", "r2", "r3"))
     xt = (xq + 3) // 4
     g = []
-    g += product(rd1[0], [0, 1, 2, 3], 1)
-    g += product(rd2[0], list(range(16)), xt)
-    pad = [-2] * (4 * xq - f)
-    g += product(b1[0], list(range(f)) + pad + list(range(f, 2 * f)) + pad, 4)
-    g += product(b1[0], list(range(2 * f, 3 * f)) + [-1], 4, b1[1])
-    g += product(b2[0], list(range(64)), 2)
-    g += product(v1[0], list(range(32)), 2)
-    g += product(v2[0][:32], list(range(32)), 2)
-    g += product(u1[0], list(range(32)), 2)
-    g += product(r1[0], list(range(36)) + [36, -1, -2, -2], 1, r1[1])
-    g += product(r2[0], list(range(16)), 1)
+    for w, slots, m_tiles, bias in _blend_products(layers, f).values():
+        g += _blend_fragments(w, slots, m_tiles, bias)
     stream = torch.stack(g + [torch.zeros(64, 4, device=dev, dtype=_f32)] * 2).contiguous()
 
     def acc_bias(b, m_tiles):
@@ -68,6 +78,32 @@
     tab = torch.stack([acc_bias(rd1[1], 1), acc_bias(rd2[1], xt), acc_bias(b2[1], 2), acc_bias(v1[1], 2), acc_bias(v2[1][:32], 2),
                        acc_bias(u1[1], 2), acc_bias(r2[1], 1), dot_row(v2[0][32]), dot_row(u2[0][0]), dot_row(r3[0][0])]).contiguous()
     return stream, tab
+
+
+def _split3_planes(x):
+    planes, r = [], x.to(_f32)
+    for k in range(3):
+        t = r.to(torch.bfloat16)
+        planes.append(t.contiguous().view(torch.int32))
+        if k < 2:
+            r = r - t.to(_f32)
+    return torch.stack(planes)
+
+
+def _pack_blend_b(layers, n_feat):
+    prod = _blend_products(layers, n_feat)
+    dev = layers["rd1"][0].device
+    zero = torch.zeros(64, 4, device=dev, dtype=torch.int32)
+    f32 = lambda name, first=0: [fr.contiguous().view(torch.int32) for fr in _blend_fragments(*prod[name])[first:]]
+    bf = lambda name, blocks=None: [_split3_planes(fr) for fr in _blend_fragments(*prod[name], quads=8)[:blocks]]
+    head = f32("rd1") + f32("rd2")
+    groups = [torch.stack(head + [zero] * (3 - len(head)))]
+    for name in ("b1mv", "b1x", "b2", "v1", "v2", "u1"):
+        groups += bf(name)
+    groups += bf("r1", 1)
+    tail = _blend_fragments(*prod["r1"])[2:]
+    groups.append(torch.stack([tail[0].contiguous().view(torch.int32)] + f32("r2") + [zero]))
+    return torch.stack(groups + [torch.zeros(3, 64, 4, device=dev, dtype=torch.int32)] * 2).contiguous()
 
 
 class BlendPlan:
@@ -98,9 +134,11 @@
                             N(r1[0], [(0, 4), (16, 4), (32, 2)]), _pad32(r1[1]), N(r2[0], [(0, 4)]), _pad32(r2[1]), _c(r3[0][0].clone())]
             self.scalars = (C.c_float * 4)(float(v2[1][32]), float(u2[1][0]), float(r3[1][0]), float(net.s.detach().abs()))
             self.finite = bool(torch.stack([torch.isfinite(p.detach()).all() for p in net.parameters()]).all())
-            self.t_stream, self.t_tab = _pack_blend_t(dict(rd1=rd1, rd2=rd2, b1=b1, b2=b2, v1=v1, v2=v2, u1=u1, u2=u2, r1=r1, r2=r2, r3=r3),
-                                                      self.n_feat)
+            layers = dict(rd1=rd1, rd2=rd2, b1=b1, b2=b2, v1=v1, v2=v2, u1=u1, u2=u2, r1=r1, r2=r2, r3=r3)
+            self.t_stream, self.t_tab = _pack_blend_t(layers, self.n_feat)
             assert self.t_stream.shape[0] == L.load().gens_blend_views_t_groups((self.n_feat - 3) // 4) + 2
+            self.b_stream = _pack_blend_b(layers, self.n_feat)
+            assert self.b_stream.shape[0] == L.load().gens_blend_bf16x3_groups((self.n_feat - 3) // 4) + 2
         self.table = L.ptr_table(self.tensors)
         self.key = BlendPlan.version(net)
 
@@ -121,11 +159,13 @@
     f = plan.n_feat
     flops = 2 * s * (4 * 16 + 16 * f + 3 * f * 64 + 64 * 32 + 32 * 32 + 32 * 33 + 32 * 32 + 32 + 37 * 16 + 16 * 8 + 8)
     nbytes = n * (12 + 12 + s + (8 if idx is not None else 0))
-    if 2 <= s <= 4 and kernels.blend == "transposed":
-        L.call("gens_blend_views_t", L.ptr_table(feats, align=16), L.int_table(hw), nl, L.ptr(aligned16(views.imgs_tex.detach()), align=16),
-               L.ptr(views.w2c), L.ptr(views.intr), L.ptr(views.c2w), views.nv, L.ptr(plan.t_stream), L.ptr(plan.t_tab), plan.scalars, L.ptr(pts),
+    if 2 <= s <= 4 and kernels.blend in ("bf16x3", "transposed"):
+        bf16 = kernels.blend == "bf16x3"
+        L.call("gens_blend_views_bf16x3" if bf16 else "gens_blend_views_t", L.ptr_table(feats, align=16), L.int_table(hw), nl,
+               L.ptr(aligned16(views.imgs_tex.detach()), align=16), L.ptr(views.w2c), L.ptr(views.intr), L.ptr(views.c2w), views.nv,
+               L.ptr(plan.b_stream, torch.int32, align=16) if bf16 else L.ptr(plan.t_stream), L.ptr(plan.t_tab), plan.scalars, L.ptr(pts),
                L.ptr(idx, torch.int64), n, L.ptr(count, torch.int32), L.ptr(rgb_out), L.ptr(vis_out, torch.uint8), L.stream(),
-               live=None if count is None else (count, n), nbytes=nbytes, flops=n * flops, label="gens_blend_views")
+               live=None if count is None else (count, n), nbytes=nbytes, flops=n * flops, label=None if bf16 else "gens_blend_views")
         if not plan.finite:
             _poison(idx, count, rgb_out)
         return rgb_out, vis_out
diff --git a/include/gens_hip.h b/include/gens_hip.h
--- a/include/gens_hip.h
+++ b/include/gens_hip.h
@@ -219,6 +219,11 @@
                       const float* c2w, int nv, const float* wstream, const float* tab, const float* scalars, const float* pts,
                       const int64_t* index, int64_t n, const int32_t* n_device, float* rgb_out, uint8_t* vis_out, void* stream);
 int gens_blend_views4_groups(int n_levels);
+
+int gens_blend_views_bf16x3(const float* const* feats, const int* hw, int n_levels, const float* imgs, const float* w2c, const float* intr,
+                            const float* c2w, int nv, const void* wstream, const float* tab, const float* scalars, const float* pts,
+                            const int64_t* index, int64_t n, const int32_t* n_device, float* rgb_out, uint8_t* vis_out, void* stream);
+int gens_blend_bf16x3_groups(int n_levels);
 
 int64_t gens_blend_train_rows(int64_t n, int nv);
 int gens_blend_train_fwd(const float* const* feats, const int* hw, int n_levels, const float* imgs, const float* w2c, const float* intr,
```

After: 242.3 million ray-samples/s (median of 6 runs). 1.02x the previous value.
